# Rikorose/DeepFilterNet

Hardware: AMD Instinct MI355X
Metric: 48 kHz audio frames/sec (hop=480), DeepFilterNet3 enhance() (higher is better)
Workload: dtype f32 (storage and accumulation; GRU projections / recurrences, the fused DF-encoder convolutions and the pointwise halves of the ERB separable convolutions as fp16-split MFMAs: x = hi + lo in f16, hi*hi + hi*lo + lo*hi on v_mfma_f32_16x16x32_f16, ~2^-21 relative; see exact_fp32_ms_per_step); 1 GPU; DeepFilterNet3 (recalled shipped shape, conv_ch=64) enhance(pad=True), batch=256 clips x 10 s @48 kHz per GPU, 1002 STFT frames per clip; batch_per_gpu=256, global_batch=256, parallelism=clips sharded over 1 GPU(s); no collective, inputs_resident_in_hbm=True

## Files before the change

deepfilternet_amd/csrc/dfx_gru_sync.h:

```cpp
#pragma once

#define DFX_SYNC_SPIN_LIMIT (1 << 22)

static __device__ __forceinline__ unsigned int dfx_sync_my_word(unsigned int tag) { return tag | (unsigned int)(dfx_xcc_id() + 1); }
static __device__ __forceinline__ bool dfx_sync_is_mine(const unsigned int *word, unsigned int tag) {
    return __hip_atomic_load(word, __ATOMIC_RELAXED, __HIP_MEMORY_SCOPE_AGENT) == dfx_sync_my_word(tag);
}

struct DfxWaiter {
    int spin_limit;
    unsigned int *err;
    bool dead = false;

    template <int SLEEP>
    __device__ __forceinline__ void wait_ge(const unsigned int *flag, unsigned int want) {
        int spins = 0;
        while (!dead && (int)(__hip_atomic_load(flag, __ATOMIC_RELAXED, __HIP_MEMORY_SCOPE_AGENT) - want) < 0) {
            if (++spins > spin_limit) {
                dfx_raise(err + 2);
                dead = true;
                break;
            }
            if constexpr (SLEEP > 0) __builtin_amdgcn_s_sleep(SLEEP);
        }
    }
    template <int SLEEP>
    __device__ __forceinline__ unsigned int wait_registered(const unsigned int *word, unsigned int tag) {
        unsigned int v = 0u;
        int spins = 0;
        while (!dead && (((v = __hip_atomic_load(word, __ATOMIC_RELAXED, __HIP_MEMORY_SCOPE_AGENT)) & ~15u) != tag || (v & 15u) == 0u)) {
            if (++spins > spin_limit) {
                dfx_raise(err + 2);
                dead = true;
                break;
            }
            if constexpr (SLEEP > 0) __builtin_amdgcn_s_sleep(SLEEP);
        }
        return v;
    }
};

static __device__ __forceinline__ void dfx_sync_raise(unsigned int *flag, unsigned int value, bool light) {
    if (light) __hip_atomic_store(flag, value, __ATOMIC_RELAXED, __HIP_MEMORY_SCOPE_AGENT);
    else __hip_atomic_store(flag, value, __ATOMIC_RELEASE, __HIP_MEMORY_SCOPE_AGENT);
}
static __device__ __forceinline__ void dfx_sync_acquire(bool light) {
    if (light) DFX_L1_INV();
    else __builtin_amdgcn_fence(__ATOMIC_ACQUIRE, "agent");
}

struct DfxXcd {
    unsigned int *me = nullptr;
    const unsigned int *prod = nullptr;
    const unsigned int *cons = nullptr;
    const unsigned int *cons2 = nullptr;
    unsigned int tag = 0;
    unsigned int *stat = nullptr;
};
static __device__ __forceinline__ void dfx_xcd_register(const DfxXcd &X) {
    if (X.me && threadIdx.x == 0) __hip_atomic_store(X.me, dfx_sync_my_word(X.tag), __ATOMIC_RELAXED, __HIP_MEMORY_SCOPE_AGENT);
}
static __device__ __forceinline__ bool dfx_xcd_same(const DfxXcd &X, const unsigned int *other) { return other && dfx_sync_is_mine(other, X.tag); }
static __device__ __forceinline__ void dfx_xcd_acquire(const DfxXcd &X) { dfx_sync_acquire(dfx_xcd_same(X, X.prod)); }
static __device__ __forceinline__ void dfx_xcd_release(const DfxXcd &X, unsigned int *flag, unsigned int value) {
    const bool light = dfx_xcd_same(X, X.cons) && (!X.cons2 || dfx_xcd_same(X, X.cons2));
    dfx_sync_raise(flag, value, light);
    if (light && X.stat) __hip_atomic_fetch_add(X.stat, 1u, __ATOMIC_RELAXED, __HIP_MEMORY_SCOPE_AGENT);
}
static __device__ __forceinline__ int dfx_xcd_claim(const unsigned int *rec, unsigned int tag, int groups, unsigned int *claim, int fallback, DfxWaiter &W, int *slot) {
    if (!rec || groups > 64) return fallback;
    if (threadIdx.x == 0) {
        auto xcd_of = [&](int g) { return (int)(__hip_atomic_load(rec + g, __ATOMIC_RELAXED, __HIP_MEMORY_SCOPE_AGENT) & 15u) - 1; };
        for (int g = 0; g < groups; ++g) W.wait_registered<4>(rec + g, tag);
        int got = -1;
        const int x0 = dfx_xcc_id();
        for (int d = 0; d < 8 && got < 0 && !W.dead; ++d) {
            const int x = (x0 + d) & 7;
            int cnt = 0;
            for (int g = 0; g < groups; ++g) cnt += xcd_of(g) == x;
            if (!cnt) continue;
            const unsigned int k = __hip_atomic_fetch_add(claim + x, 1u, __ATOMIC_RELAXED, __HIP_MEMORY_SCOPE_AGENT);
            if ((int)k >= cnt) continue;
            for (int g = 0, j = 0; g < groups; ++g)
                if (xcd_of(g) == x && j++ == (int)k) got = g;
        }
        *slot = got < 0 ? fallback : got;
    }
    __syncthreads();
    const int r = *slot;
    __syncthreads();
    return r;
}

struct DfxPublish {
    unsigned int *cnt = nullptr;
    unsigned int *flag = nullptr;
    unsigned int value = 0, nblocks = 0;
};
static __device__ __forceinline__ void dfx_publish(const DfxPublish &P) {
    if (!P.cnt) return;
    DFX_VMEM_DRAIN();
    __syncthreads();
    if (threadIdx.x == 0) {
        const unsigned int old = __hip_atomic_fetch_add(P.cnt, 1u, __ATOMIC_ACQ_REL, __HIP_MEMORY_SCOPE_AGENT);
        if (old + 1u == P.nblocks) {
            __hip_atomic_store(P.cnt, 0u, __ATOMIC_RELAXED, __HIP_MEMORY_SCOPE_AGENT);
            __hip_atomic_store(P.flag, P.value, __ATOMIC_RELEASE, __HIP_MEMORY_SCOPE_AGENT);
        }
    }
}

__global__ void dfx_k_flag_set(unsigned int *flag, unsigned int value) {
    if (threadIdx.x == 0) __hip_atomic_store(flag, value, __ATOMIC_RELEASE, __HIP_MEMORY_SCOPE_AGENT);
}
__global__ void dfx_k_wait_ge(const unsigned int *flags, int n, unsigned int target, unsigned int *err, int spin_limit) {
    bool ok = false;
    int spins = 0;
    while (!ok) {
        ok = true;
        for (int i = threadIdx.x; i < n; i += blockDim.x)
            ok = ok && (int)(__hip_atomic_load(flags + i, __ATOMIC_RELAXED, __HIP_MEMORY_SCOPE_AGENT) - target) >= 0;
        ok = __all(ok);
        if (!ok) {
            if (++spins > spin_limit) {
                if (threadIdx.x == 0) dfx_raise(err + 2);
                break;
            }
            __builtin_amdgcn_s_sleep(16);
        }
    }
    __builtin_amdgcn_fence(__ATOMIC_ACQUIRE, "agent");
}

__global__ void dfx_k_probe_meet(unsigned int *cnt, unsigned int n, int spin_limit, unsigned int *fail) {
    if (threadIdx.x == 0) {
        __hip_atomic_fetch_add(cnt, 1u, __ATOMIC_RELAXED, __HIP_MEMORY_SCOPE_AGENT);
        int spins = 0;
        while (__hip_atomic_load(cnt, __ATOMIC_RELAXED, __HIP_MEMORY_SCOPE_AGENT) < n) {
            if (++spins > spin_limit) {
                dfx_raise(fail);
                break;
            }
            __builtin_amdgcn_s_sleep(16);
        }
    }
}
```

deepfilternet_amd/csrc/dfx_model.hip:

```cpp
#include "dfx_manifest.h"
#include "dfx_nn_kernels.h"

#include <cmath>
#include <functional>
#include <atomic>
#include <map>
#include <mutex>
#include <type_traits>
#include <fcntl.h>
#include <sys/file.h>
#include <sys/stat.h>
#include <unistd.h>

static int check_cfg(const dfx_model_cfg *c) {
    if (!c) DFX_FAIL(DFX_ERR_INVALID_ARG, "null model cfg");
    if (c->conv_ch != 16 && c->conv_ch != 32 && c->conv_ch != 64)
        DFX_FAIL(DFX_ERR_UNSUPPORTED, "conv_ch=%d: the HIP kernels are instantiated for 16, 32, 64", c->conv_ch);
    if (c->emb_hidden_dim != 256 || c->df_hidden_dim != 256) DFX_FAIL(DFX_ERR_UNSUPPORTED, "GRU hidden size must be 256");
    if (c->nb_erb <= 0 || c->nb_erb % 8 || c->nb_erb > 64) DFX_FAIL(DFX_ERR_UNSUPPORTED, "nb_erb must be a multiple of 8, <= 64");
    static_assert(2 * DFX_DEC10_SMEM(64, 64) <= 160 * 1024, "conv_ch <= 64, nb_erb <= 64: dfx_k_erb_dec10 must fit every accepted shape");
    if (c->nb_df <= 0 || c->nb_df % 2 || c->nb_df > c->fft_size / 2 + 1) DFX_FAIL(DFX_ERR_UNSUPPORTED, "nb_df must be even and <= F");
    if (c->df_order <= 0 || c->df_order > 16 || c->df_lookahead < 0 || c->df_lookahead >= c->df_order)
        DFX_FAIL(DFX_ERR_UNSUPPORTED, "need 0 <= df_lookahead < df_order <= 16");
    if (c->conv_lookahead < 0) DFX_FAIL(DFX_ERR_INVALID_ARG, "conv_lookahead < 0");
// ... 265 lines not shown
            acc = mode == 1 ? fmaxf(acc, v) : acc + v;
        }
        if (mode == 2) acc *= inv;
        for (int c = 0; c < ch; ++c) p[(int64_t)c * T * E] = acc;
    }
}

__global__ void dfx_k_gate_stages(const unsigned char *flags, unsigned char *stages, int64_t B) {
    const int64_t b = (int64_t)blockIdx.x * blockDim.x + threadIdx.x;
    if (b >= B) return;
    const unsigned char f = flags[b];
    stages[b] = (unsigned char)((f & DFX_GATE_DF) | ((f & (DFX_GATE_GAINS | DFX_GATE_ZEROS)) ? DFX_GATE_GAINS : 0));
}

#define DFX_GATE_MAX_ENTRIES 24
struct DfxGateTable {
    float *dst[DFX_GATE_MAX_ENTRIES];
    const float *src[DFX_GATE_MAX_ENTRIES];
    int64_t row[DFX_GATE_MAX_ENTRIES];
    unsigned char mask[DFX_GATE_MAX_ENTRIES], want[DFX_GATE_MAX_ENTRIES];
    int n;
    void add(float *dst_, const float *src_, int64_t row_, unsigned char mask_, unsigned char want_) {
        dst[n] = dst_, src[n] = src_, row[n] = row_, mask[n] = mask_, want[n] = want_;
        ++n;
    }
};
__global__ void dfx_k_gate_commit(DfxGateTable G, const unsigned char *flags, int64_t B) {
    const int64_t b = blockIdx.x;
    if (b >= B) return;
    const unsigned char f = flags[b];
    for (int e = 0; e < G.n; ++e) {
        if ((f & G.mask[e]) != G.want[e]) continue;
        const float *sp = G.src[e] + b * G.row[e];
        float *dp = G.dst[e] + b * G.row[e];
        for (int64_t i = threadIdx.x; i < G.row[e]; i += blockDim.x) dp[i] = sp[i];
    }
}

__global__ void dfx_k_gate_c0_shift(const unsigned char *flags, float *c0_win, int64_t B, int64_t T, int kt, int64_t frame) {
    const int64_t b = blockIdx.x;
    if (b >= B || !(flags[b] & DFX_GATE_DF)) return;
    float *w = c0_win + (b * T + T - kt) * frame;
    for (int64_t i = (int64_t)blockIdx.y * blockDim.x + threadIdx.x; i < frame; i += (int64_t)gridDim.y * blockDim.x)
        for (int j = 0; j + 1 < kt; ++j) w[j * frame + i] = w[(j + 1) * frame + i];
}

__global__ void dfx_k_gate_hold(const unsigned char *flags, float *win, int64_t cap, int64_t row, int64_t pos, int64_t h, int64_t B) {
    const int64_t b = blockIdx.x;
    if (b >= B || !(flags[b] & DFX_GATE_FROZEN)) return;
    float *w = win + (b * cap + pos) * row;
    for (int64_t i = (int64_t)blockIdx.y * blockDim.x + threadIdx.x; i < row; i += (int64_t)gridDim.y * blockDim.x)
        for (int64_t j = h - 1; j >= 0; --j) w[(j + 1) * row + i] = w[j * row + i];
}

__global__ void dfx_k_gate_pend_commit(const unsigned char *flags, unsigned char *par, int *cnt, int64_t B) {
    const int64_t b = (int64_t)blockIdx.x * blockDim.x + threadIdx.x;
    if (b >= B || !(flags[b] & DFX_GATE_DF)) return;
    par[b] ^= 1;
    cnt[b] += 1;
}

__global__ void dfx_k_gate_finish(const unsigned char *flags, int *skip_counter, float *y, int64_t y_stride, int hop, float *lsnr_out,
                                  int64_t lsnr_stride, int64_t B, int warm) {
    const int64_t b = blockIdx.x;
    if (b >= B) return;
    const unsigned char f = flags[b];
    if (f & DFX_GATE_FROZEN) {
        for (int i = threadIdx.x; i < hop; i += blockDim.x) y[b * y_stride + i] = 0.f;
        if (threadIdx.x == 0 && lsnr_out) lsnr_out[b * lsnr_stride] = (f & DFX_GATE_PAUSED) ? __int_as_float(0x7fc00000) : -15.f;
    } else if (threadIdx.x == 0 && !warm) {
        skip_counter[b] = (f & (DFX_GATE_GAINS | DFX_GATE_ZEROS)) ? 0 : skip_counter[b] + 1;
    }
}

enum { EV_START = 0, EV_C0, EV_C1, EV_C0P, EV_EMB, EV_COEFS, EV_FRONT, EV_DONE, EV_XA, EV_MASK, EV_FIN, EV_TICKET };

struct DfxCan {
    bool fuse_c0 = false;
    bool c0_batch_unfused = false;
    bool c0_h3 = false;
    bool c0_presplit = false;
    bool pw_h3 = false;
    bool fan = false, fan_skp = false;
    bool enc_fan = false;
    bool dfenc = false;
    bool fuse_enc = false;
    bool erb_tail = false;
    bool erb_enc4 = false;
    int df_out = DFX_PLAN_DF_OUT_GGEMM;
};

struct DfxSyncLayout {
    static constexpr size_t LG = (size_t)DFX_MAX_GRU_LAYERS * DFX_SEQ_GMAX;
    static constexpr size_t ready = 0;
    static constexpr size_t emb = 8;
    static constexpr size_t probe = 13;
    static constexpr size_t poison = 14;
    static constexpr size_t done = 16;
    static constexpr size_t pcnt = done + LG;
    static constexpr size_t yprog = pcnt + 16;
    static constexpr size_t giprog = yprog + LG;
    static constexpr size_t xtab = giprog + LG;
    static constexpr size_t xstat = xtab + 3 * LG;
    static constexpr size_t total = xstat + 64;
};

struct dfx_model {
    dfx_model_cfg cfg{};
    float *d_w = nullptr;
    size_t n_w = 0;
    size_t erb0_w = 0, erb0_b = 0;
    PwW erb1, erb2, erb3, dfc0, dfc1, ct3, ct2, ct1;
    size_t co_w = 0, co_ska = 0, co_skb = 0;
    float co_bias = 0.f;
    size_t tail_w0h3 = 0, tail_woh3 = 0;
    float tail_w0_unscale = 1.f, tail_wo_unscale = 1.f;
    GlinW fc_emb, enc_in, enc_out, dec_in, dec_out, dfg_in, df_skip, df_out, enc_skip, dec_skip;
    std::vector<GruW> enc_gru, dec_gru, df_gru;
    size_t lsnr_w = 0;
    float lsnr_b = 0.f;
    size_t fan_w = 0;
    int fan_chunks = 0;
    size_t efan_w1 = 0, efan_w2 = 0;
    int efan_groups = 0;
    size_t dfenc_fc = 0, dfenc_in = 0;
    float dfenc_fc_unscale = 1.f, dfenc_in_unscale = 1.f;
    size_t dfo_h3 = 0;
    float dfo_unscale = 1.f;
    size_t cp_w1 = 0, cp_w2 = 0, cp_b = 0;
    size_t cp_weff = 0, cp_b16 = 0;
    size_t cin_weff = 0, cin_b = 0;
    size_t c0_h3 = 0, dfc1_h3 = 0, cp_h3 = 0;
    float c0_unscale = 1.f, dfc1_unscale = 1.f, cp_unscale = 1.f;
    int cp_G = 0, cp_NO = 0;
    DfxLane *lanes = nullptr;
    struct DfxLaneSet *laneset = nullptr;
    hipEvent_t ev_fork = nullptr;
    hipEvent_t ev_pass = nullptr;
    hipEvent_t ev_gate = nullptr;
    mutable bool pass_pending = false;
    bool enqueue_ahead = false;
    bool concurrent = false;
    int max_chunks = 1;
    int tchunks = 12;
    int tchunk_min = 32;
    bool run_df = true;
    bool exact_fp32 = false;
    DfxCan can;
    unsigned int *d_sync = nullptr;
    unsigned int *d_psync = nullptr;
    mutable unsigned int seq_pbase = 0;
    mutable int64_t passes_ps = 0;
    mutable int64_t passes_pair = 0;
    mutable int64_t last_plan = 0;
    mutable int64_t passes_seq = 0, passes_ev = 0;
    mutable unsigned int seq_base = 0;
    unsigned long long *d_trace = nullptr;
    mutable int trace_dims[3] = {0, 0, 0};
    bool gru_seq = true;
    struct {
        int chunks = 0;
        bool gru_pair_far = false;
        bool gru_pair = true;
        int convp_late = -1;
        int p0_ahead = 3;
        int tail_every = 1;
        int dftail_every = 0;
        bool tail_split = true;
        int64_t convp_elems = (int64_t)1 << 29;
        bool c0_presplit = true;
        bool seq_trace = false;
        char hwq_probe_mode = 0;
        bool erb_enc_split = false;
        int ws_fill = -1;
    } sw;
    unsigned int *d_err = nullptr;
    unsigned int *h_err = nullptr;
    bool check_every_pass = false;
    int spin_limit = DFX_SYNC_SPIN_LIMIT;
    bool hwq_probe_pending = false;
    int hwq_probe = -1;
    const float *p(size_t off) const { return d_w + off; }
};

namespace {
struct Prep {
    const float *blob;
    const DfxManifest &man;
    std::vector<float> out;
    std::string err;
    bool exact_fp32 = false;
    struct Packed {
        bool pw = false, tail = false, c0 = false, fan = false, fan_skp = false, encfan = false, dfenc = false;
        int dfo_tiles = 0;
    } packed;
    const float *get(const std::string &name, const DfxTensor **tt = nullptr) {
        const DfxTensor *t = man.find(name);
        if (!t) {
            err = "tensor not in manifest: " + name;
            return nullptr;
        }
        if (tt) *tt = t;
        return blob + t->offset;
    }
    size_t alloc(size_t n) {
        size_t off = (out.size() + 3) & ~(size_t)3;
        out.resize(off + n, 0.f);
        return off;
    }
    bool bn(const std::string &p, int n, std::vector<float> &scale, std::vector<float> &shift) {
        const float *g = get(p + ".weight"), *b = get(p + ".bias"), *m = get(p + ".running_mean"), *v = get(p + ".running_var");
        if (!g || !b || !m || !v) return false;
        scale.resize(n);
        shift.resize(n);
        for (int i = 0; i < n; ++i) {
            const float s = g[i] / sqrtf(v[i] + 1e-5f);
            scale[i] = s;
            shift[i] = b[i] - m[i] * s;
        }
        return true;
    }
};

bool prep_sep(Prep &P, const std::string &name, int C, PwW &w) {
    const float *dw = P.get(name + ".0.weight"), *pw = P.get(name + ".1.weight");
    std::vector<float> sc, sh;
    if (!dw || !pw || !P.bn(name + ".2", C, sc, sh)) return false;
    w.dw = P.alloc(3 * C);
    w.wt = P.alloc((size_t)C * C);
    w.bias = P.alloc(C);
    for (int c = 0; c < C; ++c)
        for (int j = 0; j < 3; ++j) P.out[w.dw + j * C + c] = dw[c * 3 + j];
    for (int n = 0; n < C; ++n)
        for (int k = 0; k < C; ++k) P.out[w.wt + (size_t)k * C + n] = pw[(size_t)n * C + k] * sc[n];
    for (int n = 0; n < C; ++n) P.out[w.bias + n] = sh[n];
    return true;
}
bool prep_path(Prep &P, const std::string &name, int C, size_t &a_off, size_t &b_off) {
    const float *w = P.get(name + ".0.weight");
    std::vector<float> sc, sh;
    if (!w || !P.bn(name + ".1", C, sc, sh)) return false;
    a_off = P.alloc(C);
    b_off = P.alloc(C);
    for (int c = 0; c < C; ++c) {
        P.out[a_off + c] = w[c] * sc[c];
        P.out[b_off + c] = sh[c];
    }
    return true;
}
template <typename F>
size_t pack_h3(Prep &P, int nfrag, F val, float *unscale) {
    std::vector<float> v((size_t)nfrag * 64 * 8);
    float mx = 0.f;
    for (int fr = 0; fr < nfrag; ++fr)
        for (int l = 0; l < 64; ++l)
            for (int i = 0; i < 8; ++i) {
                const float w = val(fr, l, i);
                v[((size_t)fr * 64 + l) * 8 + i] = w;
                mx = fmaxf(mx, fabsf(w));
            }
    int e = 0;
    if (mx > 0.f) {
        int ex;
        frexpf(mx, &ex);
        e = 14 - ex;
        if (e > 24) e = 24;
        if (e < -14) e = -14;
    }
    const float sc = ldexpf(1.f, e);
    *unscale = ldexpf(1.f, -e);
    const size_t off = P.alloc((size_t)nfrag * 2 * 64 * 8 / 2);
    uint16_t *dst = reinterpret_cast<uint16_t *>(&P.out[off]);
    for (int fr = 0; fr < nfrag; ++fr)
        for (int l = 0; l < 64; ++l)
            for (int i = 0; i < 8; ++i) {
                const float w = v[((size_t)fr * 64 + l) * 8 + i] * sc;
                const uint16_t hb = dfx_f32_to_f16_bits(w);
                const uint16_t lb = dfx_f32_to_f16_bits(w - dfx_f16_bits_to_f32(hb));
                dst[(((size_t)fr * 2 + 0) * 64 + l) * 8 + i] = hb;
                dst[(((size_t)fr * 2 + 1) * 64 + l) * 8 + i] = lb;
            }
    return off;
}
size_t pack_x32(Prep &P, const float *w) {
    const int H = 256;
    const size_t off = P.alloc((size_t)3 * H * H);
    float *dst = &P.out[off];
    for (int ut = 0; ut < 16; ++ut)
        for (int kc = 0; kc < 8; ++kc)
            for (int gate = 0; gate < 3; ++gate)
                for (int half = 0; half < 2; ++half)
                    for (int l = 0; l < 64; ++l)
                        for (int i = 0; i < 4; ++i) {
                            const int unit = 16 * ut + (l & 15), k = 32 * kc + 8 * (l >> 4) + 4 * half + i;
                            const size_t frag = (((size_t)ut * 8 + kc) * 3 + gate) * 2 + half;
                            dst[(frag * 64 + l) * 4 + i] = w[(size_t)(gate * H + unit) * H + k];
                        }
    return off;
}
void pack_pw_h3(Prep &P, dfx_model *m) {
    const int C = m->cfg.conv_ch, KC = C / 32;
    if (C % 32 != 0) return;
    for (PwW *w : {&m->erb1, &m->erb2, &m->erb3, &m->ct3, &m->ct2, &m->ct1}) {
        w->wt_h3 = pack_h3(P, (C / 16) * KC, [&](int fr, int l, int i) {
            const int nt = fr / KC, kc = fr % KC;
            return P.out[w->wt + (size_t)((C / 4) * (l >> 4) + 8 * kc + i) * C + 16 * nt + (l & 15)];
        }, &w->unscale);
        w->has_h3 = true;
    }
    P.packed.pw = true;
}
bool prep_glin(Prep &P, const std::string &name, GlinW &g) {
    const DfxTensor *t = nullptr;
    const float *w = P.get(name, &t);
    if (!w) return false;
    g.G = (int)t->shape[0];
// ... 296 lines not shown
        const int j = l & 15, e = 8 * kc + i, ch = 16 * (e >> 2) + 4 * (l >> 4) + (e & 3);
        return j < 3 ? P.out[wo + (size_t)j * C + ch] : 0.f;
    }, &m->tail_wo_unscale);
    P.packed.tail = true;
}
bool prep_df_convp(Prep &P, dfx_model *m) {
    const dfx_model_cfg &c = m->cfg;
    const int C = c.conv_ch, kt = c.df_pathway_kernel_size_t, NO = 2 * c.df_order, G = dfx_gcd(C, NO), CG = C / G, OG = NO / G;
    const int idx = kt > 1 ? 1 : 0;
    const bool has_pw = kt > 1;
    const float *w = P.get("df_dec.df_convp." + std::to_string(idx) + ".weight");
    const float *pw = has_pw ? P.get("df_dec.df_convp." + std::to_string(idx + 1) + ".weight") : nullptr;
    std::vector<float> sc, sh;
    if (!w || (has_pw && !pw) || !P.bn("df_dec.df_convp." + std::to_string(idx + (has_pw ? 2 : 1)), NO, sc, sh)) return false;
    m->cp_G = G;
    m->cp_NO = NO;
    m->cp_w1 = P.alloc((size_t)G * kt * CG * 16);
    m->cp_w2 = P.alloc((size_t)NO * NO);
    m->cp_b = P.alloc(NO);
    for (int g = 0; g < G; ++g)
        for (int k = 0; k < kt; ++k)
            for (int ci = 0; ci < CG; ++ci)
                for (int o = 0; o < OG; ++o) {
                    float v = w[(((size_t)(g * OG + o) * CG + ci) * kt + k)];
                    if (!has_pw) v *= sc[g * OG + o];
                    P.out[m->cp_w1 + ((((size_t)g * kt + k) * CG + ci) * 16 + o)] = v;
                }
    for (int n = 0; n < NO; ++n) {
        for (int o = 0; o < NO; ++o) P.out[m->cp_w2 + (size_t)n * NO + o] = has_pw ? pw[(size_t)n * NO + o] * sc[n] : (n == o ? 1.f : 0.f);
        P.out[m->cp_b + n] = sh[n];
    }
    const bool folded = NO <= 16;
    m->cp_weff = P.alloc(folded ? (size_t)kt * C * 16 : 0);
    m->cp_b16 = P.alloc(16);
    for (int k = 0; folded && k < kt; ++k)
        for (int ch = 0; ch < C; ++ch) {
            const int g = ch / CG, ci = ch - g * CG;
            for (int n = 0; n < NO; ++n) {
                double acc = 0.0;
                for (int o = g * OG; o < (g + 1) * OG; ++o) {
                    const double p2 = has_pw ? (double)pw[(size_t)n * NO + o] : (n == o ? 1.0 : 0.0);
                    acc += p2 * (double)w[((size_t)o * CG + ci) * kt + k];
                }
                P.out[m->cp_weff + ((size_t)k * C + ch) * 16 + n] = (float)(acc * (double)sc[n]);
            }
        }
    for (int n = 0; folded && n < NO; ++n) P.out[m->cp_b16 + n] = sh[n];
    return true;
}
void pack_c0_h3(Prep &P, dfx_model *m) {
    const dfx_model_cfg &c = m->cfg;
    const int C = c.conv_ch, kt = c.df_pathway_kernel_size_t;
    if (C % 32 != 0 || 2 * c.df_order > 16) return;
    const int KC = C / 32;
    auto chan = [](int kc, int l, int i) { const int e = 8 * kc + i; return 16 * (e >> 2) + 4 * (l >> 4) + (e & 3); };
    const size_t cin = m->cin_weff, wt1 = m->dfc1.wt, cpw = m->cp_weff;
    m->c0_h3 = pack_h3(P, C / 16, [&](int nt, int l, int i) {
        const int k = 8 * (l >> 4) + i;
        return k < 18 ? P.out[cin + (size_t)k * C + 16 * nt + (l & 15)] : 0.f;
    }, &m->c0_unscale);
    m->dfc1_h3 = pack_h3(P, (C / 16) * KC, [&](int fr, int l, int i) {
        const int nt = fr / KC, kc = fr % KC;
        return P.out[wt1 + (size_t)chan(kc, l, i) * C + 16 * nt + (l & 15)];
    }, &m->dfc1_unscale);
    m->cp_h3 = pack_h3(P, kt * KC, [&](int fr, int l, int i) {
        const int k = fr / KC, kc = fr % KC;
        return P.out[cpw + ((size_t)k * C + chan(kc, l, i)) * 16 + (l & 15)];
    }, &m->cp_unscale);
    P.packed.c0 = true;
}
void pack_dfo_h3(Prep &P, dfx_model *m) {
    const GlinW a = m->df_out;
    const int NO = 2 * m->cfg.df_order, Fd = m->cfg.nb_df;
    if (!(a.Kg <= 32 && a.Kg % 8 == 0 && a.Ng % 2 == 0 && NO % 2 == 0 && Fd % 2 == 0 && (int64_t)a.G * a.Ng == (int64_t)NO * Fd &&
          DFX_DFO_SMEM(NO, Fd) <= (size_t)64 * 1024))
        return;
    const int NU = (a.Ng + 15) / 16;
    m->dfo_h3 = pack_h3(P, a.G * NU, [&](int fr, int l, int i) {
        const int g = fr / NU, u = fr % NU, o = 16 * u + (l & 15), k = 8 * (l >> 4) + i;
        return o < a.Ng && k < a.Kg ? P.out[a.w + ((size_t)g * a.Kg + k) * a.Ng + o] : 0.f;
    }, &m->dfo_unscale);
    P.packed.dfo_tiles = NU;
}
void pack_dfenc_h3(Prep &P, dfx_model *m) {
    const GlinW a = m->fc_emb, b = m->enc_in;
    const int C = m->cfg.conv_ch, Fout = m->cfg.nb_df / 2, KC = C / 32;
    if (!P.packed.c0) return;
    if (!(a.Kg % 32 == 0 && a.Ng == 16 && b.Kg == 32 && b.Ng == 16 && b.G * 2 == a.G && (int64_t)a.G * a.Kg == (int64_t)Fout * C)) return;
    m->dfenc_fc = pack_h3(P, Fout * KC, [&](int ci, int l, int i) {
        const int fo = ci / KC, kc = ci % KC, ch = 16 * ((8 * kc + i) >> 2) + 4 * (l >> 4) + (i & 3);
        const int idx = fo * C + ch, g = idx / a.Kg, kin = idx % a.Kg;
        return P.out[a.w + ((size_t)g * a.Kg + kin) * 16 + (l & 15)];
    }, &m->dfenc_fc_unscale);
    m->dfenc_in = pack_h3(P, b.G, [&](int j, int l, int i) {
        return P.out[b.w + ((size_t)j * 32 + 16 * (i >> 2) + 4 * (l >> 4) + (i & 3)) * 16 + (l & 15)];
    }, &m->dfenc_in_unscale);
    P.packed.dfenc = true;
}

bool prepare_weights(Prep &P, dfx_model *m) {
    const dfx_model_cfg &c = m->cfg;
    const int C = c.conv_ch;
    const bool skip_enc = c.emb_gru_skip_enc == DFX_SKIP_GROUPEDLINEAR, skip_dec = c.emb_gru_skip == DFX_SKIP_GROUPEDLINEAR;
    if (!prep_erb_conv0(P, m)) return false;
    if (!prep_sep(P, "enc.erb_conv1", C, m->erb1) || !prep_sep(P, "enc.erb_conv2", C, m->erb2) || !prep_sep(P, "enc.erb_conv3", C, m->erb3) ||
        !prep_sep(P, "enc.df_conv1", C, m->dfc1))
        return false;
    if (!prep_df_conv0(P, m)) return false;
    if (!prep_glin(P, "enc.df_fc_emb.0.weight", m->fc_emb) || !prep_glin(P, "enc.emb_gru.linear_in.0.weight", m->enc_in) ||
        !prep_gru(P, "enc.emb_gru.gru", 1, m->enc_gru) || !prep_glin(P, "enc.emb_gru.linear_out.0.weight", m->enc_out))
        return false;
    if (skip_enc && !prep_glin(P, "enc.emb_gru.gru_skip.weight", m->enc_skip)) return false;
    if (skip_dec && !prep_glin(P, "erb_dec.emb_gru.gru_skip.weight", m->dec_skip)) return false;
    if (!prep_lsnr(P, m)) return false;
    if (!prep_glin(P, "erb_dec.emb_gru.linear_in.0.weight", m->dec_in) || !prep_gru(P, "erb_dec.emb_gru.gru", c.emb_num_layers - 1, m->dec_gru) ||
        !prep_glin(P, "erb_dec.emb_gru.linear_out.0.weight", m->dec_out))
        return false;
    if (!prep_sep(P, "erb_dec.convt3", C, m->ct3) || !prep_path(P, "erb_dec.conv3p", C, m->ct3.sk_a, m->ct3.sk_b) ||
        !prep_sep(P, "erb_dec.convt2", C, m->ct2) || !prep_path(P, "erb_dec.conv2p", C, m->ct2.sk_a, m->ct2.sk_b) ||
        !prep_sep(P, "erb_dec.convt1", C, m->ct1) || !prep_path(P, "erb_dec.conv1p", C, m->ct1.sk_a, m->ct1.sk_b) ||
        !prep_path(P, "erb_dec.conv0p", C, m->co_ska, m->co_skb))
        return false;
    m->ct3.has_skip = m->ct2.has_skip = m->ct1.has_skip = true;
    pack_pw_h3(P, m);
    if (!prep_conv0_out(P, m)) return false;
    pack_tail_h3(P, m);
    if (!prep_df_convp(P, m)) return false;
    pack_c0_h3(P, m);
    if (!prep_glin(P, "df_dec.df_gru.linear_in.0.weight", m->dfg_in) || !prep_gru(P, "df_dec.df_gru.gru", c.df_num_layers, m->df_gru)) return false;
    if (c.df_gru_skip == DFX_SKIP_GROUPEDLINEAR && !prep_glin(P, "df_dec.df_skip.weight", m->df_skip)) return false;
    if (!prep_glin(P, "df_dec.df_out.0.weight", m->df_out)) return false;
    pack_fan(P, m);
    pack_encfan(P, m);
    pack_dfo_h3(P, m);
    pack_dfenc_h3(P, m);
    return true;
}
}

static void read_switches(dfx_model *m) {
    auto is = [](const char *name, char ch) {
        const char *v = getenv(name);
        return v && v[0] == ch;
    };
    auto at_least = [](const char *name, int least, int *out) {
        const char *v = getenv(name);
        if (v && atoi(v) >= least) *out = atoi(v);
    };
    m->exact_fp32 = is("DFX_EXACT_FP32", '1');
    m->concurrent = !is("DFX_STREAMS", '0');
    m->gru_seq = !is("DFX_GRU_SEQ", '0') && !dfx_env_is_emulator();
    if (getenv("DFX_GRU_PAIR")) m->sw.gru_pair = !is("DFX_GRU_PAIR", '0');
    m->sw.gru_pair_far = is("DFX_GRU_PAIR_FAR", '1');
    m->check_every_pass = is("DFX_CHECK_EVERY_PASS", '1');
    at_least("DFX_SYNC_SPIN_LIMIT", 1, &m->spin_limit);
    if (const char *v = getenv("DFX_CONVP_ELEMS"))
        if (atoll(v) > 0) m->sw.convp_elems = atoll(v);
    m->sw.erb_enc_split = is("DFX_ERB_ENC_SPLIT", '1');
    m->sw.c0_presplit = !is("DFX_C0_PRESPLIT", '0');
    if (const char *v = getenv("DFX_WS_FILL"))
        if (v[0] >= '0' && v[0] <= '9' && atoi(v) <= 255) m->sw.ws_fill = atoi(v);
#ifdef DFX_DEV
    if (getenv("DFX_TAIL_SPLIT")) m->sw.tail_split = !is("DFX_TAIL_SPLIT", '0');
    at_least("DFX_SEQ_P0_AHEAD", 1, &m->sw.p0_ahead);
    at_least("DFX_SEQ_DFTAIL_EVERY", 1, &m->sw.dftail_every);
    at_least("DFX_SEQ_TAIL_EVERY", 1, &m->sw.tail_every);
    at_least("DFX_SEQ_CHUNKS", 1, &m->sw.chunks);
    at_least("DFX_CONVP_LATE", 0, &m->sw.convp_late);
#endif
    m->sw.seq_trace = is("DFX_SEQ_TRACE", '1');
    int tc = 0;
    at_least("DFX_TCHUNKS", 1, &tc);
    if (tc) m->tchunks = tc < DFX_MAX_TCHUNKS ? tc : DFX_MAX_TCHUNKS;
    m->enqueue_ahead = is("DFX_ENQUEUE_AHEAD", '1');
    m->sw.hwq_probe_mode = is("DFX_HWQ_PROBE", '0') ? '0' : is("DFX_HWQ_PROBE", 'f') ? 'f' : 0;
}

static void model_capabilities(dfx_model *m, const Prep::Packed &k) {
    const dfx_model_cfg &c = m->cfg;
    const int C = c.conv_ch, E = c.nb_erb, Fd = c.nb_df, NO = 2 * c.df_order, emb = C * E / 4;
    const bool split = !m->exact_fp32;
    DfxCan &can = m->can;
    can.fuse_c0 = c.df_pathway_kernel_size_t <= 5 && NO <= 16;
    can.c0_batch_unfused = m->exact_fp32 && can.fuse_c0;
    can.c0_h3 = can.fuse_c0 && split && k.c0;
    can.c0_presplit = m->sw.c0_presplit && can.c0_h3;
    can.pw_h3 = split && k.pw;
    can.fan = k.fan && !c.enc_concat && emb == 64 * m->fan_chunks;
    can.fan_skp = can.fan && c.df_gru_skip == DFX_SKIP_GROUPEDLINEAR && k.fan_skp;
    can.enc_fan = k.encfan && !c.enc_concat && emb == 16 * m->efan_groups;
    can.dfenc = can.c0_h3 && can.enc_fan && k.dfenc;
    can.fuse_enc = E % 2 == 0 && 3 * (E + 2) <= 192 && 2 * DFX_ENC_SMEM(C, E) <= (size_t)160 * 1024;
    can.erb_tail = can.pw_h3 && k.tail && dfx_tail_ok(C, E);
    can.erb_enc4 = can.fuse_enc && can.pw_h3 && dfx_enc4_ok(C, E);
    const bool resident = k.dfo_tiles == 4 && m->df_out.G <= 16 && (int64_t)(NO / 2) * 16 * (Fd / 2) <= (int64_t)DFX_DFO_NPT * DFX_DFO_THREADS;
    can.df_out = !(split && k.dfo_tiles > 0) ? DFX_PLAN_DF_OUT_GGEMM : resident ? DFX_PLAN_DF_OUT_RESIDENT : DFX_PLAN_DF_OUT_STREAMING;
}

static int create_device_objects(dfx_model *m) {
    if (m->sw.seq_trace) (void)hipMalloc(reinterpret_cast<void **>(&m->d_trace), (size_t)DFX_MAX_GRU_LAYERS * DFX_SEQ_GMAX * DFX_GS_MAX_CHUNKS * 3 * 8);
    const size_t sync_bytes = DfxSyncLayout::total * sizeof(unsigned int);
    const size_t psync_bytes = (size_t)DFX_MAX_GRU_LAYERS * (DFX_SEQ_GMAX / 2) * 48 * sizeof(unsigned int);
    if (hipMalloc(reinterpret_cast<void **>(&m->d_psync), psync_bytes) != hipSuccess || hipMemset(m->d_psync, 0, psync_bytes) != hipSuccess ||
        hipMalloc(reinterpret_cast<void **>(&m->d_sync), sync_bytes) != hipSuccess || hipMemset(m->d_sync, 0, sync_bytes) != hipSuccess ||
        dfx_env_err_words_alloc(&m->h_err, &m->d_err, 256) != hipSuccess)
        DFX_FAIL(DFX_ERR_ALLOC, "dfx_model_create: device allocation failed");
    bool good = hipEventCreateWithFlags(&m->ev_fork, hipEventDisableTiming) == hipSuccess;
    good = good && hipEventCreateWithFlags(&m->ev_pass, hipEventDisableTiming) == hipSuccess;
    good = good && hipEventCreateWithFlags(&m->ev_gate, hipEventDisableTiming) == hipSuccess;
    good = good && dfx_create_lane(m, 0);
    for (int l = 1; l < m->max_chunks && good; ++l) good = dfx_create_lane(m, l);
    if (!good) DFX_FAIL(DFX_ERR_HIP, "dfx_model_create: could not create the auxiliary streams/events");
    return DFX_OK;
}

extern "C" int dfx_model_create(const dfx_model_cfg *cfg, const float *blob, dfx_model **out) {
    if (int rc = check_cfg(cfg)) return rc;
    if (!blob || !out) DFX_FAIL(DFX_ERR_INVALID_ARG, "dfx_model_create: null");
    if (int rc = dfx_require_device()) return rc;
    dfx_model *m = new dfx_model();
    m->cfg = *cfg;
    read_switches(m);
    const DfxManifest man = dfx_build_manifest(m->cfg);
    Prep P{blob, man};
    P.exact_fp32 = m->exact_fp32;
    if (!prepare_weights(P, m)) {
        delete m;
        DFX_FAIL(DFX_ERR_INVALID_ARG, "dfx_model_create: %s", P.err.empty() ? "weight preparation failed" : P.err.c_str());
    }
    m->n_w = P.out.size();
    if (hipMalloc(reinterpret_cast<void **>(&m->d_w), m->n_w * sizeof(float)) != hipSuccess) {
        delete m;
        DFX_FAIL(DFX_ERR_ALLOC, "dfx_model_create: device allocation of %zu bytes failed", m->n_w * sizeof(float));
    }
    if (hipMemcpy(m->d_w, P.out.data(), m->n_w * sizeof(float), hipMemcpyHostToDevice) != hipSuccess) {
        dfx_model_free(m);
        DFX_FAIL(DFX_ERR_HIP, "dfx_model_create: upload failed");
    }
    model_capabilities(m, P.packed);
    if (int rc = create_device_objects(m)) {
        dfx_model_free(m);
        return rc;
    }
    if (m->gru_seq && m->concurrent && !dfx_env_is_emulator()) {
        if (m->sw.hwq_probe_mode == 'f') {
            m->hwq_probe = 0;
            hwq_probe_fallback(m);
        } else if (m->sw.hwq_probe_mode != '0') {
            m->hwq_probe_pending = true;
        }
    }
    *out = m;
    return DFX_OK;
}

static void pass_gate_forget(const dfx_model *m);
extern "C" void dfx_model_free(dfx_model *m) {
    if (!m) return;
    pass_gate_forget(m);
    if (m->ev_fork) (void)hipEventDestroy(m->ev_fork);
    if (m->ev_pass) (void)hipEventDestroy(m->ev_pass);
    if (m->ev_gate) (void)hipEventDestroy(m->ev_gate);
    dfx_env_err_words_free(m->h_err);
    if (m->d_sync && m->d_trace) {
        unsigned int n = 0;
        if (hipMemcpy(&n, m->d_sync + DfxSyncLayout::xstat, sizeof(n), hipMemcpyDeviceToHost) == hipSuccess) fprintf(stderr, "[dfx] same-XCD (light) block hand-overs over the model's life: %u\n", n);
    }
    if (m->d_sync) (void)hipFree(m->d_sync);
    if (m->d_psync) (void)hipFree(m->d_psync);
    if (m->d_trace) (void)hipFree(m->d_trace);
    if (m->d_w) (void)hipFree(m->d_w);
    delete m;
}
extern "C" int dfx_model_set_streams(dfx_model *m, int enable) {
    if (!m) DFX_FAIL(DFX_ERR_INVALID_ARG, "null");
    m->concurrent = enable != 0;
    return DFX_OK;
}
extern "C" int dfx_model_set_run_df(dfx_model *m, int enable) {
    if (!m) DFX_FAIL(DFX_ERR_INVALID_ARG, "null");
    m->run_df = enable != 0;
    return DFX_OK;
}
extern "C" int dfx_model_set_pipeline(dfx_model *m, int time_chunks, int min_chunk_frames, int batch_chunks) {
    if (!m || time_chunks < 1 || min_chunk_frames < 1 || batch_chunks < 1) DFX_FAIL(DFX_ERR_INVALID_ARG, "dfx_model_set_pipeline: bad arguments");
    m->tchunks = time_chunks < DFX_MAX_TCHUNKS ? time_chunks : DFX_MAX_TCHUNKS;
    m->tchunk_min = min_chunk_frames;
    m->max_chunks = batch_chunks < DFX_MAX_LANES ? batch_chunks : DFX_MAX_LANES;
    for (int l = 1; l < m->max_chunks; ++l)
        if (!dfx_create_lane(m, l)) DFX_FAIL(DFX_ERR_HIP, "dfx_model_set_pipeline: could not create the streams of lane %d", l);
    return DFX_OK;
}
static int model_poll(const dfx_model *m) {
    unsigned int *h = m->h_err;
    if (!h) return DFX_OK;
    if (!(((volatile unsigned int *)h)[1] | ((volatile unsigned int *)h)[2])) return DFX_OK;
    const unsigned int e1 = __atomic_exchange_n(&h[1], 0u, __ATOMIC_ACQ_REL), e2 = __atomic_exchange_n(&h[2], 0u, __ATOMIC_ACQ_REL);
    if (!(e1 | e2)) return DFX_OK;
    if (e2)
        DFX_FAIL(DFX_ERR_HIP, "dfx: a flag wait of the persistent GRU phase timed out (bounded spin: the streams of the pass did not make progress "
                              "independently — hardware queues shared with other work, or the GPU shared with another process); the results of "
                              "the previous pass on this model are invalid.  DFX_GRU_SEQ=0 selects the event-synchronised form");
    DFX_FAIL(DFX_ERR_UNSUPPORTED, "dfx: an activation of magnitude >= 6e4 reached an fp16-split matrix kernel (GRU / DF-encoder / separable-conv "
                                  "path); the results of the previous pass on this model are invalid.  DFX_EXACT_FP32=1 selects the exact fp32 kernels");
}
extern "C" int dfx_model_poll(const dfx_model *m) {
    if (!m) DFX_FAIL(DFX_ERR_INVALID_ARG, "null");
    return model_poll(m);
}
extern "C" int dfx_model_check(const dfx_model *m) {
    if (!m) DFX_FAIL(DFX_ERR_INVALID_ARG, "null");
    DFX_HIP(hipDeviceSynchronize());
    return model_poll(m);
}
extern "C" int dfx_model_query(const dfx_model *m, int what, int64_t *value) {
    if (!m || !value) DFX_FAIL(DFX_ERR_INVALID_ARG, "dfx_model_query: null");
    switch (what) {
        case DFX_Q_GRU_PERSISTENT:
        case DFX_Q_HWQ_PROBE: {
            std::lock_guard<std::mutex> lk(dfx_enqueue_mu());
            hwq_probe_run(const_cast<dfx_model *>(m));
            *value = what == DFX_Q_HWQ_PROBE ? m->hwq_probe : (m->gru_seq && m->concurrent ? 1 : 0);
            return DFX_OK;
        }
        case DFX_Q_EXACT_FP32: *value = m->exact_fp32 ? 1 : 0; return DFX_OK;
        case DFX_Q_PASSES_PERSISTENT: *value = m->passes_seq; return DFX_OK;
        case DFX_Q_PASSES_TICKET_BUSY: *value = m->passes_ev; return DFX_OK;
        case DFX_Q_SPIN_LIMIT: *value = m->spin_limit; return DFX_OK;
        case DFX_Q_PASSES_C0_PRESPLIT: *value = m->passes_ps; return DFX_OK;
        case DFX_Q_LAST_PLAN: *value = m->last_plan; return DFX_OK;
        case DFX_Q_PASSES_PAIR: *value = m->passes_pair; return DFX_OK;
    }
    DFX_FAIL(DFX_ERR_INVALID_ARG, "dfx_model_query: unknown item %d", what);
}
extern "C" int dfx_model_seq_trace(const dfx_model *m, unsigned long long *out_host, int64_t cap, int *dims) {
    if (!m || !m->d_trace || !out_host || !dims) DFX_FAIL(DFX_ERR_INVALID_ARG, "dfx_model_seq_trace: tracing is off (DFX_SEQ_TRACE=1 at model creation)");
    const int64_t n = (int64_t)m->trace_dims[0] * m->trace_dims[1] * m->trace_dims[2] * 3;
    if (n > cap) DFX_FAIL(DFX_ERR_INVALID_ARG, "dfx_model_seq_trace: buffer too small");
    DFX_HIP(hipMemcpy(out_host, m->d_trace, (size_t)n * 8, hipMemcpyDeviceToHost));
    for (int i = 0; i < 3; ++i) dims[i] = m->trace_dims[i];
    return DFX_OK;
}
extern "C" int dfx_model_cfg_get(const dfx_model *m, dfx_model_cfg *out) {
    if (!m || !out) DFX_FAIL(DFX_ERR_INVALID_ARG, "null");
    *out = m->cfg;
    return DFX_OK;
}

static inline bool dfx_dfenc_ok(const dfx_model *m, int64_t B, int64_t T, int64_t feat_T) {
    const dfx_model_cfg &c = m->cfg;
    const int64_t emb = (int64_t)c.conv_ch * c.nb_erb / 4;
    return m->can.dfenc && B * T * emb < ((int64_t)1 << 31) && B * (feat_T > 0 ? feat_T : T) * c.nb_df < ((int64_t)1 << 29);
}
static inline bool dfx_feat_spec_unread(const dfx_model *m, int64_t B, int64_t T) { return m->can.c0_presplit && dfx_dfenc_ok(m, B, T, 0); }
static inline float *dfx_ws_base(void *workspace) { return reinterpret_cast<float *>(((uintptr_t)workspace + 255) & ~(uintptr_t)255); }

namespace {
struct Ws {
    size_t e0, e1, e2, e3, c0, c1, emb_in, emb, xa, xb, gi, xa2, xb2, gi2, demb, d3, d2, mask, c0p, xdf, coefs, lsnr, skp_e, skp_d, fps, total;
    size_t pgi[DFX_MAX_GRU_LAYERS], py[DFX_MAX_GRU_LAYERS], ph[DFX_MAX_GRU_LAYERS];
};
Ws plan_ws(const dfx_model *m, int64_t R, int64_t B) {
    const dfx_model_cfg &c = m->cfg;
    const bool c0_stored = !m->can.fuse_c0 || m->can.c0_batch_unfused, presplit = m->can.c0_presplit;
    Ws w{};
    size_t off = 0;
    auto take = [&](size_t n) {
        size_t o = off;
        off += (n + 63) & ~(size_t)63;
        return o;
    };
    const size_t C = c.conv_ch, E = c.nb_erb, Fd = c.nb_df, emb = C * E / 4, NO = 2 * c.df_order;
    w.e0 = take(R * E * C);
    w.e1 = take(R * (E / 2) * C);
    w.e2 = take(R * (E / 4) * C);
    w.e3 = take(R * (E / 4) * C);
    w.c0 = c0_stored ? take(R * Fd * C) : 0;
    w.c1 = take(R * (Fd / 2) * C);
    w.emb_in = take(R * emb * (c.enc_concat ? 2 : 1));
    w.emb = take(R * emb);
    w.xa = take(R * 256);
    w.xb = take(R * 256);
    w.gi = take(R * 768);
    w.xa2 = take(R * 256);
    w.xb2 = take(R * 256);
    w.gi2 = take(R * 768);
    w.demb = take(R * emb);
    w.d3 = take(R * (E / 4) * C);
    w.d2 = take(R * (E / 2) * C);
    w.mask = take(R * E);
    w.c0p = take(R * Fd * NO);
    w.xdf = take(R * 256);
    w.coefs = take(R * Fd * NO);
    w.lsnr = take(R);
    w.skp_e = take(c.emb_gru_skip_enc == DFX_SKIP_GROUPEDLINEAR ? R * emb : 0);
    w.skp_d = take(c.emb_gru_skip == DFX_SKIP_GROUPEDLINEAR ? R * emb : 0);
    w.fps = take(presplit ? R * Fd * 2 : 0);
    const int nlayers = 1 + (c.emb_num_layers - 1) + c.df_num_layers;
    for (int l = 0; l < DFX_MAX_GRU_LAYERS; ++l) {
        const bool used = l < nlayers;
        w.pgi[l] = take(used ? R * 768 : 0);
        w.py[l] = take(used ? R * 256 : 0);
        w.ph[l] = take(used ? (B > 0 ? B : R) * 256 : 0);
    }
    w.total = off;
    return w;
}
}

extern "C" int dfx_model_workspace_bytes(const dfx_model *m, int64_t B, int64_t T, int64_t *bytes) {
    if (!m || !bytes || B < 0 || T < 0) DFX_FAIL(DFX_ERR_INVALID_ARG, "dfx_model_workspace_bytes: bad arguments");
    *bytes = (int64_t)(plan_ws(m, B * T, B).total * sizeof(float)) + 256;
    return DFX_OK;
}

#include "dfx_model_launch.h"
#include "dfx_model_forward.h"
#include "dfx_model_stream.h"
#include "dfx_stream_move.h"
#include "dfx_model_enhance.h"
```

deepfilternet_amd/csrc/dfx_model_forward.h:

```cpp
#pragma once

#ifdef DFX_DEV
static int dfx_dev_skip() {
    static const int v = [] { const char *e = getenv("DFX_DEV_SKIP"); return e ? atoi(e) : 0; }();
    return v;
}
static bool dfx_dev_stage(int n) {
    static const int lo = [] { const char *e = getenv("DFX_DEV_STAGE_LO"); return e ? atoi(e) : 0; }();
    static const int hi = [] { const char *e = getenv("DFX_DEV_STAGE_HI"); return e ? atoi(e) : 99; }();
    return n >= lo && n <= hi;
}
#else
static constexpr int dfx_dev_skip() { return 0; }
static constexpr bool dfx_dev_stage(int) { return true; }
#endif

struct TicketGuard {
    bool armed = false;
    ~TicketGuard() {
        if (armed) dfx_ticket_release_cb(nullptr);
    }
};

template <int C>
// ... 334 lines not shown
            convp_split = use_seq && late_pct > 0 ? T - (T - t_begin) * late_pct / 100 : T;
            if (convp_split > t_begin && dfx_dev_stage(1) && (rc = convp_range(t_begin, convp_split, x2))) return rc;
            if (post_behind_convp && (rc = sc->df_post(x2))) return rc;
            if (convp_split >= T && (rc = signal(EV_C0P, x2))) return rc;
        }
        if (dfx_dev_stage(2) && (rc = erb_range(t_begin, T, Rn, rmw, s))) return rc;
        if ((rc = wait(EV_C1, s))) return rc;
        if (dfenc) {
            if (dfx_dev_stage(3) && (rc = launch_df_enc<C>(m, feat_spec, e3, c.emb_gru_skip_enc != DFX_SKIP_NONE ? emb_in : nullptr, xa, B, T, Fd, s, t_begin, Lk, T, featT, fps))) return rc;
        } else if (dfx_dev_stage(3) && (rc = emb_range(Rn, rmw, s))) return rc;
        if (signal_front && (rc = signal(EV_FRONT, s))) return rc;
        return DFX_OK;
    }

    int gru_serial() {
        int rc;
        float *hs_enc = sc ? sc->h_state : nullptr, *hs_dec = sc ? sc->h_state + (int64_t)nenc * B * 256 : nullptr;
        float *hs_df = sc ? sc->h_state + (int64_t)(nenc + ndec) * B * 256 : nullptr;
        float *hn_enc = sc && sc->h_next ? sc->h_next : nullptr, *hn_dec = hn_enc ? hn_enc + (int64_t)nenc * B * 256 : nullptr;
        float *hn_df = hn_enc ? hn_enc + (int64_t)(nenc + ndec) * B * 256 : nullptr;
        const float *y = xa;
        if (dfx_dev_stage(4) && (rc = run_gru_stack(m, m->enc_gru, xa, xa, xb, gi, B, T, &y, s, hs_enc, t_begin, rmw, hn_enc))) return rc;
        float *dec_x = y == xa ? xb : xa;
        if (fan) {
            if (dfx_dev_stage(5) && (rc = emb_fan(y, dec_x, Rn, s, rmw))) return rc;
            if ((rc = signal(EV_EMB, s)) || (rc = wait(EV_EMB, x1))) return rc;
        } else {
            if ((rc = enc_out_skip(y, Rn, s, rmw))) return rc;
            if ((rc = signal(EV_EMB, s)) || (rc = wait(EV_EMB, x1))) return rc;
            if ((rc = lsnr_all(s))) return rc;
        }
        if (gate) {
            dfx_launch(dfx_k_gate_post, dim3((unsigned)dfx_ceil_div(B, 256)), dim3(256), 0, s, (const float *)lsnr, T, gate->thr[0],
                       gate->thr[1], run_df ? gate->thr[2] : -INFINITY, gate->flags, B, gate->channels, gate->thr_rows);
            DFX_LAUNCH_CHECK();
        }
        if (run_df && dfx_dev_stage(6)) {
            const float *y2 = nullptr;
            if (!fan && (rc = launch_glin(m, m->dfg_in, embv, DFX_ACT_RELU, nullptr, xa2, Rn, x1, rmw))) return rc;
            if ((rc = run_gru_stack(m, m->df_gru, xa2, xa2, xb2, gi2, B, T, &y2, x1, hs_df, t_begin, rmw, hn_df, par))) return rc;
            if ((rc = df_tail_rows(y2, Rn, rmw, x1, true))) return rc;
            if ((rc = signal(EV_COEFS, x1))) return rc;
        }
        if (!fan && (rc = launch_glin(m, m->dec_in, embv, DFX_ACT_RELU, nullptr, dec_x, Rn, s, rmw))) return rc;
        if (dfx_dev_stage(7) && (rc = run_gru_stack(m, m->dec_gru, dec_x, xa, xb, gi, B, T, &y, s, hs_dec, t_begin, rmw, hn_dec, par && run_df))) return rc;
        if (dfx_dev_stage(8) && (rc = dec_out_skip(y, Rn, s, rmw))) return rc;
        if ((!fuse_tail || dfx_dev_stage(9)) && (rc = erb_dec_convs(Rn, rmw, s))) return rc;
        return DFX_OK;
    }

    int gru_events() {
        int rc;
        auto proj_ev = [&](const GruW &g, int l, int k, const float *xin, hipStream_t st) -> int {
            if ((dfx_dev_skip() & 4) && l > 0) return DFX_OK;
            return proj_chunk(g, l, k, xin, st);
        };
        auto gru_chunk = [&](const GruW &g, int l, int k, hipStream_t st) -> int {
            float *hl = ws + w.ph[l];
            return launch_gru_h3(m, g, ws + w.pgi[l], ws + w.py[l], k == 0 ? nullptr : hl, hl, B, T, tb(k), tb(k + 1), st, l);
        };
        if ((rc = signal(EV_XA, s))) return rc;
        for (int l = 0; l < nl; ++l) {
            if (l > 0 && (rc = wait(EV_XA, ln->gs[l]))) return rc;
            if ((rc = wait(EV_XA, ln->ps[l]))) return rc;
        }
        if ((rc = wait(EV_XA, ln->ts[0])) || (rc = wait(EV_XA, ln->ts[1]))) return rc;
        for (int k = 0; k < K; ++k) {
            if ((rc = proj_ev(m->enc_gru[0], 0, k, xa, ln->ps[0])) || (rc = esig(ln->pev[0][k], ln->ps[0]))) return rc;
        }
        for (int k = 0; k < K; ++k) {
            if ((rc = ewait(ln->pev[0][k], s)) || (rc = gru_chunk(m->enc_gru[0], 0, k, s)) || (rc = esig(ln->gev[0][k], s))) return rc;
        }
        for (int j = 0; j < ndec; ++j) {
            const int l = 1 + j;
            hipStream_t pst = ln->ps[l], gst = ln->gs[l];
            for (int k = 0; k < K; ++k) {
                if ((rc = ewait(ln->gev[l - 1][k], pst))) return rc;
                const float *xin = ws + w.py[l - 1];
                if (j == 0 && fan) {
                    if ((rc = emb_fan(ws + w.py[0], xb, Mk(k), pst, rmk(k)))) return rc;
                    if ((rc = esig(ln->eev[k], pst))) return rc;
                    xin = xb;
                } else if (j == 0) {
                    if ((rc = enc_out_skip(ws + w.py[0], Mk(k), pst, rmk(k)))) return rc;
                    if ((rc = esig(ln->eev[k], pst))) return rc;
                    if ((rc = launch_glin(m, m->dec_in, embv, DFX_ACT_RELU, nullptr, xb, Mk(k), pst, rmk(k)))) return rc;
                    xin = xb;
                }
                if ((rc = proj_ev(m->dec_gru[j], l, k, xin, pst)) || (rc = esig(ln->pev[l][k], pst))) return rc;
            }
            for (int k = 0; k < K; ++k) {
                if ((rc = ewait(ln->pev[l][k], gst)) || (rc = gru_chunk(m->dec_gru[j], l, k, gst)) || (rc = esig(ln->gev[l][k], gst))) return rc;
            }
        }
        {
            hipStream_t st = ln->ts[0];
            for (int k = 0; k < K; ++k) {
                if ((rc = ewait(ln->gev[ndec][k], st))) return rc;
                if (dfx_dev_skip() & 1) continue;
                if ((rc = dec_out_skip(ws + w.py[ndec], Mk(k), st, rmk(k))) || (rc = erb_dec_convs(Mk(k), rmk(k), st))) return rc;
            }
            if ((rc = signal(EV_MASK, st))) return rc;
        }
        for (int j = 0; j < ndf; ++j) {
            const int l = 1 + ndec + j;
            hipStream_t pst = ln->ps[l], gst = ln->gs[l];
            for (int k = 0; k < K; ++k) {
                const float *xin = ws + w.py[l - 1];
                if (j == 0) {
                    if ((rc = ewait(ln->eev[k], pst))) return rc;
                    if (!fan && (rc = launch_glin(m, m->dfg_in, embv, DFX_ACT_RELU, nullptr, xa2, Mk(k), pst, rmk(k)))) return rc;
                    xin = xa2;
                } else if ((rc = ewait(ln->gev[l - 1][k], pst))) return rc;
                if ((rc = proj_ev(m->df_gru[j], l, k, xin, pst)) || (rc = esig(ln->pev[l][k], pst))) return rc;
            }
            for (int k = 0; k < K; ++k) {
                if ((rc = ewait(ln->pev[l][k], gst)) || (rc = gru_chunk(m->df_gru[j], l, k, gst)) || (rc = esig(ln->gev[l][k], gst))) return rc;
            }
        }
        if (run_df) {
            hipStream_t st = ln->ts[1];
            const int l = ndec + ndf;
            if ((rc = wait(EV_C0P, st))) return rc;
            if (c.df_gru_skip != DFX_SKIP_IDENTITY) {
                for (int k = 0; k < K; ++k) {
                    if ((rc = ewait(ln->gev[l][k], st))) return rc;
                    if (dfx_dev_skip() & 2) continue;
                    if ((rc = df_tail_rows(ws + w.py[l], Mk(k), rmk(k), st))) return rc;
                }
            } else if ((rc = ewait(ln->gev[l][K - 1], st)) || (rc = df_tail_identity(ws + w.py[l], st))) return rc;
            if ((rc = signal(EV_COEFS, st))) return rc;
        }
        if ((rc = ewait(ln->eev[K - 1], s))) return rc;
        if (!fan && (rc = lsnr_all(s))) return rc;
        return DFX_OK;
    }

    int gru_persistent() {
        int rc;
        const unsigned int base = m->seq_base;
        m->seq_base += (unsigned int)K + 1u;
        using SL = DfxSyncLayout;
        unsigned int *ready = m->d_sync + SL::ready, *embf = m->d_sync + SL::emb, *done = m->d_sync + SL::done;
        unsigned int *pcnt = m->d_sync + SL::pcnt;
        unsigned int *yprog = m->d_sync + SL::yprog, *giprog = m->d_sync + SL::giprog;
        unsigned int *embprog = yprog + (size_t)(DFX_MAX_GRU_LAYERS - 1) * DFX_SEQ_GMAX;
        unsigned int *xtab = m->d_sync + SL::xtab, *xstat = m->d_sync + SL::xstat;
        const unsigned int xtag = (m->seq_pbase & 0x0fffffffu) << 4;
        auto xword = [&](int kind, int layer) { return xtab + ((size_t)kind * DFX_MAX_GRU_LAYERS + layer) * DFX_SEQ_GMAX; };
        const unsigned int pbase = m->seq_pbase;
        bool followed[DFX_MAX_GRU_LAYERS] = {};
        int nfollow = 0;
        const int lfirst_df = 1 + ndec;
        const bool follow_emb = fan && c.emb_gru_skip_enc != DFX_SKIP_GROUPEDLINEAR && nl < DFX_MAX_GRU_LAYERS &&
                                (nl + nl) * groups <= dfx_env_num_cus() * 3 / 4 && nl - 1 <= DFX_PF_MAX;
        for (int l = 1; l < nl; ++l) {
            const bool first = l == 1 || l == lfirst_df;
            if (!first || follow_emb) followed[l] = true, ++nfollow;
        }
        if (nfollow > DFX_PF_MAX || (nl + nfollow + 1) * groups > dfx_env_num_cus() * 3 / 4) {
            nfollow = 0;
            for (int l = 0; l < nl; ++l) followed[l] = false;
        }
        const bool use_pair = m->sw.gru_pair && !m->exact_fp32 && groups >= 2 && m->d_psync;
        m->passes_pair += use_pair ? 1 : 0;
        if (nfollow || use_pair) m->seq_pbase += (unsigned int)T + 1u;
        auto proj_pub = [&](const GruW &g, int l, int k, const float *xin, hipStream_t st) -> int {
            DfxPublish pub;
            pub.cnt = pcnt + l, pub.flag = ready + l, pub.value = base + (unsigned int)k + 1u;
            return proj_chunk(g, l, k, xin, st, &pub);
        };
        auto donep = [&](int l) { return done + (size_t)l * DFX_SEQ_GMAX; };
        auto tgt = [&](int k) { return base + (unsigned int)k + 1u; };
        hipStream_t G = ln->gs[1], Eq = ln->ts[0], Dq = ln->ts[1], Pq = ln->ps[0];
        const int ev_go = EV_XA;
        if ((rc = signal(EV_XA, s))) return rc;
        if (!m->enqueue_ahead && R >= DFX_THROTTLE_MIN_FRAMES) DFX_HIP(hipEventSynchronize(ln->ev[EV_XA]));
        if ((rc = wait(ev_go, G)) || (rc = wait(ev_go, Eq)) || (rc = wait(ev_go, Dq)) || (rc = wait(ev_go, Pq))) return rc;
        if (nfollow) DFX_HIP(hipMemsetAsync(xstat + 8, 0, (size_t)(DFX_PF_MAX + 1) * 8 * sizeof(unsigned int), G));
        {
            DfxGsArgs S;
            for (int l = 0; l < DFX_GS_MAX_LAYERS; ++l) S.gi[l] = nullptr, S.y[l] = nullptr, S.whf[l] = nullptr, S.bhn[l] = nullptr, S.unscale[l] = 1.f;
            for (int l = 0; l < nl; ++l) {
                const GruW &g = l == 0 ? m->enc_gru[0] : (l <= ndec ? m->dec_gru[l - 1] : m->df_gru[l - 1 - ndec]);
                S.gi[l] = ws + w.pgi[l];
                S.y[l] = ws + w.py[l];
                S.whf[l] = reinterpret_cast<const dfx_h8 *>(m->p(m->exact_fp32 ? g.whh_x32 : g.whh_h3));
                S.bhn[l] = m->p(g.bhn);
                S.unscale[l] = m->exact_fp32 ? 1.f : g.whh_unscale;
            }
            S.B = B, S.T = T, S.nlayers = nl, S.groups = groups, S.K = K;
            for (int i = 0; i <= K; ++i) S.tb[i] = cb[i];
            S.ready = ready, S.done = done, S.done_stride = DFX_SEQ_GMAX, S.base = base, S.err = m->d_err;
            S.trace = m->d_trace;
            S.spin_limit = m->spin_limit;
            S.pbase = pbase, S.sblk = 16;
            S.xtab = xtab, S.xstride = DFX_SEQ_GMAX, S.xstat = xstat;
            S.xtag = xtag, S.psync = m->d_psync, S.pair_far = m->sw.gru_pair_far ? 1 : 0;
            for (int l = 1; l < nl; ++l) {
                if (!followed[l]) continue;
                S.giprog[l] = giprog + (size_t)l * DFX_SEQ_GMAX;
                const bool first = l == 1 || l == lfirst_df;
                const int src = first ? 0 : l - 1;
                S.yprog[src] = yprog + (size_t)src * DFX_SEQ_GMAX;
                S.yblk[src] = first ? DFX_EF_STEPS : 16;
                S.xcons_kind[src] = first ? 2 : 1, S.xcons_layer[src] = first ? 0 : l;
            }
            m->trace_dims[0] = nl, m->trace_dims[1] = groups, m->trace_dims[2] = K;
            if (use_pair) DFX_HIP(dfx_env_set_max_dyn_smem((const void *)dfx_k_gru_seq_p2, DFX_GP_SMEM));
            else DFX_HIP(dfx_env_set_max_dyn_smem(m->exact_fp32 ? (const void *)dfx_k_gru_seq_x32 : (const void *)dfx_k_gru_seq, DFX_GH_SMEM));
            DfxKScope ks(DFX_K_GRU_REC, G);
            if (use_pair) dfx_launch(dfx_k_gru_seq_p2, dim3(dfx_gp_grid(nl * (int)((groups + 1) / 2))), dim3(DFX_GP_THREADS), DFX_GP_SMEM, G, S);
            else if (m->exact_fp32) dfx_launch(dfx_k_gru_seq_x32, dim3((unsigned)(nl * groups)), dim3(DFX_GH_THREADS), DFX_GH_SMEM, G, S);
            else dfx_launch(dfx_k_gru_seq, dim3((unsigned)(nl * groups)), dim3(DFX_GH_THREADS), DFX_GH_SMEM, G, S);
            DFX_LAUNCH_CHECK();
        }
        if (nfollow) {
            DfxPfArgs F;
            int f = 0;
            for (int l = 1; l < nl; ++l) {
                if (!followed[l]) continue;
                const GruW &g = l <= ndec ? m->dec_gru[l - 1] : m->df_gru[l - 1 - ndec];
                const bool first = l == 1 || l == lfirst_df;
                F.x[f] = first ? (l == 1 ? xb : xa2) : ws + w.py[l - 1], F.gi[f] = ws + w.pgi[l];
                F.wf[f] = reinterpret_cast<const dfx_h8 *>(m->p(m->exact_fp32 ? g.wih_t : g.wih_h3)), F.bias[f] = m->p(g.bias_i), F.unscale[f] = g.wih_unscale;
                F.yprog[f] = first ? embprog : yprog + (size_t)(l - 1) * DFX_SEQ_GMAX, F.giprog[f] = giprog + (size_t)l * DFX_SEQ_GMAX;
                F.xme[f] = xword(1, l), F.xprod[f] = first ? xword(2, 0) : xword(0, l - 1), F.xcons[f] = xword(0, l);
                ++f;
            }
            for (; f < DFX_PF_MAX; ++f) F.x[f] = nullptr, F.gi[f] = nullptr, F.wf[f] = nullptr, F.bias[f] = nullptr, F.unscale[f] = 1.f, F.yprog[f] = nullptr, F.giprog[f] = nullptr;
            F.xtag = xtag, F.xstat = xstat;
            F.xrec = xword(0, 0), F.xclaim = xstat + 8;
            F.B = B, F.T = T, F.nf = nfollow, F.groups = groups, F.pbase = pbase, F.err = m->d_err, F.spin_limit = m->spin_limit;
            int lq = -1;
            for (int l = nl - 1; l >= 2 && lq < 0; --l)
                if (followed[l]) lq = l;
            hipStream_t Fq = lq > 0 ? ln->ps[lq] : Dq;
            DFX_HIP(dfx_env_set_max_dyn_smem(m->exact_fp32 ? (const void *)dfx_k_proj_follow_x32 : (const void *)dfx_k_proj_follow, DFX_PH_SMEM));
            if ((rc = wait(ev_go, Fq))) return rc;
            DfxKScope ks(DFX_K_PROJ, Fq);
            if (m->exact_fp32) dfx_launch(dfx_k_proj_follow_x32, dim3((unsigned)(nfollow * groups)), dim3(512), DFX_PH_SMEM, Fq, F);
            else dfx_launch(dfx_k_proj_follow, dim3((unsigned)(nfollow * groups)), dim3(512), DFX_PH_SMEM, Fq, F);
            DFX_LAUNCH_CHECK();
        }
        if (followed[1]) {
            const float *res = c.emb_gru_skip_enc == DFX_SKIP_IDENTITY ? emb_in : nullptr;
            const bool need_emb = c.emb_gru_skip != DFX_SKIP_NONE || (run_df && c.df_gru_skip == DFX_SKIP_IDENTITY);
            float *dfg_x = run_df ? xa2 : nullptr, *skp = fan_skp ? xdf : nullptr;
            DfxFanArgs EA = emb_fan_args(m, ws + w.py[0], res, need_emb ? embv : nullptr, xb, dfg_x, skp, lsnr);
            DfxFollowSync EY;
            EY.x.me = xword(2, 0), EY.x.prod = xword(0, 0), EY.x.cons = xword(1, 1), EY.x.cons2 = followed[lfirst_df] ? xword(1, lfirst_df) : nullptr;
            EY.x.tag = xtag, EY.x.stat = xstat;
            EY.xclaim = xstat + 8 + 8 * DFX_PF_MAX, EY.groups = groups;
            EY.src = yprog, EY.dst = embprog, EY.pbase = pbase, EY.err = m->d_err, EY.spin_limit = m->spin_limit, EY.B = B, EY.T = T;
            hipStream_t Eq2 = ln->ps[1];
            if ((rc = wait(ev_go, Eq2))) return rc;
            {
                DfxKScope ks(DFX_K_EMB_FAN, Eq2);
                if (dfg_x && skp) dfx_launch((dfx_k_emb_follow<1, 2, 1>), dim3((unsigned)groups), dim3(512), 0, Eq2, EA, EY);
                else if (dfg_x) dfx_launch((dfx_k_emb_follow<1, 2, 0>), dim3((unsigned)groups), dim3(512), 0, Eq2, EA, EY);
                else dfx_launch((dfx_k_emb_follow<1, 0, 0>), dim3((unsigned)groups), dim3(512), 0, Eq2, EA, EY);
                DFX_LAUNCH_CHECK();
            }
            if ((rc = signal(EV_EMB, Eq2))) return rc;
        }
        const bool convp_after_p0 = nfollow > 0;
        auto convp_late = [&]() -> int {
            if (!(run_df && convp_split < T)) return DFX_OK;
            int r;
            if ((r = wait(ev_go, x2)) || (r = convp_range(convp_split, T, x2)) || (r = signal(EV_C0P, x2))) return r;
            return DFX_OK;
        };
        if (!convp_after_p0 && (rc = convp_late())) return rc;
        {
            for (int k = 0; k < K; ++k) {
                const int p0_ahead = m->sw.p0_ahead;
                if (k >= p0_ahead && (rc = launch_wait_ge(m, donep(0), groups, tgt(k - p0_ahead), Pq))) return rc;
                if ((rc = proj_pub(m->enc_gru[0], 0, k, xa, Pq))) return rc;
                if (convp_after_p0 && k == (K < p0_ahead ? K : p0_ahead) - 1 && (rc = convp_late())) return rc;
            }
        }
        for (int l = 1; l < nl; ++l)
            if ((rc = wait(ev_go, ln->ps[l]))) return rc;
        const int lf = 1 + ndec;
        auto prep_dec = [&](int j, int k) -> int {
            const int l = 1 + j;
            hipStream_t st = ln->ps[l];
            int r;
            if (followed[l]) return DFX_OK;
            if ((r = launch_wait_ge(m, donep(l - 1), groups, tgt(k), st))) return r;
            const float *xin = ws + w.py[l - 1];
            if (j == 0 && fan) {
                if (!m->exact_fp32) {
                    DfxPublish pub;
                    pub.cnt = pcnt + 8, pub.flag = embf, pub.value = tgt(k);
                    if ((r = emb_fan(ws + w.py[0], xb, Mk(k), st, rmk(k), &pub))) return r;
                } else if ((r = emb_fan(ws + w.py[0], xb, Mk(k), st, rmk(k))) || (r = launch_flag_set(embf, tgt(k), st))) return r;
                if (k == K - 1 && (r = signal(EV_EMB, st))) return r;
                xin = xb;
            } else if (j == 0) {
                if ((r = enc_out_skip(ws + w.py[0], Mk(k), st, rmk(k))) || (r = launch_flag_set(embf, tgt(k), st))) return r;
                if (k == K - 1 && (r = signal(EV_EMB, st))) return r;
                if ((r = launch_glin(m, m->dec_in, embv, DFX_ACT_RELU, nullptr, xb, Mk(k), st, rmk(k)))) return r;
                xin = xb;
            }
            if ((r = proj_pub(m->dec_gru[j], l, k, xin, st))) return r;
            return DFX_OK;
        };
        auto erb_tail = [&](int k0, int k) -> int {
            const int64_t Rk = Mk(k0, k);
            const DfxRowMap rm = rmk(k0, k);
            int r;
            hipStream_t Gq = (m->sw.tail_split && ndec >= 2 && followed[2]) ? ln->ps[2] : Eq;
            if ((r = launch_wait_ge(m, donep(ndec), groups, tgt(k), Gq))) return r;
            if (dfx_dev_skip() & 1) return DFX_OK;
            if ((r = dec_out_skip(ws + w.py[ndec], Rk, Gq, rm))) return r;
            if (Gq != Eq && ((r = esig(ln->pev[2][k], Gq)) || (r = ewait(ln->pev[2][k], Eq)))) return r;
            return erb_dec_convs(Rk, rm, Eq);
        };
        auto prep_df = [&](int j, int k) -> int {
            const int l = lf + j;
            hipStream_t st = ln->ps[l];
            int r;
            if (followed[l]) return DFX_OK;
            const float *xin = ws + w.py[l - 1];
            if (j == 0) {
                if ((r = launch_wait_ge(m, embf, 1, tgt(k), st))) return r;
                if (!fan && (r = launch_glin(m, m->dfg_in, embv, DFX_ACT_RELU, nullptr, xa2, Mk(k), st, rmk(k)))) return r;
                xin = xa2;
            } else if ((r = launch_wait_ge(m, donep(l - 1), groups, tgt(k), st))) return r;
            if ((r = proj_pub(m->df_gru[j], l, k, xin, st))) return r;
            return DFX_OK;
        };
        auto df_tail = [&](int k0, int k) -> int {
            const int l = ndec + ndf;
            const int64_t Rk = Mk(k0, k);
            const DfxRowMap rm = rmk(k0, k);
            if (int r = launch_wait_ge(m, donep(l), groups, tgt(k), Dq)) return r;
            if (dfx_dev_skip() & 2) return DFX_OK;
            if (c.df_gru_skip == DFX_SKIP_IDENTITY) {
                if (k < K - 1) return DFX_OK;
                return df_tail_identity(ws + w.py[l], Dq);
            }
            return df_tail_rows(ws + w.py[l], Rk, rm, Dq);
        };
        if (run_df && (rc = wait(EV_C0P, Dq))) return rc;
        for (int k = 0; k < K; ++k) {
            for (int j = 0; j < (ndec > ndf ? ndec : ndf); ++j) {
                if (j < ndec && (rc = prep_dec(j, k))) return rc;
                if (j < ndf && (rc = prep_df(j, k))) return rc;
            }
            const int tail_every = m->sw.tail_every;
            if ((k + 1) % tail_every == 0 || k == K - 1) {
                const int k0 = k - (k % tail_every);
                if ((rc = erb_tail(k0, k))) return rc;
            }
            const int dft_env = m->sw.dftail_every;
            const int dft_every = dft_env > 0 ? dft_env : (nfollow > 0 && convp_split < T && tail_every < 4 ? 4 : tail_every);
            if (run_df && ((k + 1) % dft_every == 0 || k == K - 1)) {
                const int k0 = k - (k % dft_every);
                if ((rc = df_tail(k0, k))) return rc;
            }
        }
        if ((rc = signal(EV_MASK, Eq))) return rc;
        if ((rc = wait(EV_EMB, s))) return rc;
        if (!fan && (rc = lsnr_all(s))) return rc;
        DFX_HIP(hipEventRecord(ln->gev[0][0], G));
        DFX_HIP(hipStreamWaitEvent(s, ln->gev[0][0], 0));
        for (int l = 0; l < nl; ++l) {
            DFX_HIP(hipEventRecord(ln->pev[l][0], ln->ps[l]));
            DFX_HIP(hipStreamWaitEvent(s, ln->pev[l][0], 0));
        }
        return DFX_OK;
    }

    int finish(float *coefs_out) {
        int rc;
        if (pipe) {
            fin_s = ln->ts[1];
            if ((rc = wait(EV_MASK, fin_s))) return rc;
        }
        if (run_df && fin_s == s && (rc = wait(EV_COEFS, s))) return rc;
        if (!run_df && coefs_out) DFX_HIP(hipMemsetAsync(coefs_out, 0, (size_t)R * Fd * NO * sizeof(float), fin_s));
        if (sc) {
            const float beta = sc->pf_beta >= 0.f ? sc->pf_beta : (c.mask_pf ? c.pf_beta : 0.f);
            if (sc->channels > 1 && sc->reduce_mask != 0) {
                dfx_launch(dfx_k_mask_reduce, dim3((unsigned)nn_grid(dfx_ceil_div(Rn * E / sc->channels, 256), 8)), dim3(256), 0, s, mask, B, T, t_begin,
                           E, sc->channels, sc->reduce_mask);
                DFX_LAUNCH_CHECK();
            }
            if (gate) {
                dfx_launch(dfx_k_gate_edit, dim3((unsigned)B), dim3(128), 0, s, (const unsigned char *)gate->flags, mask, coefs,
                           (const unsigned char *)bands->d_bin2band, B, T, E, Fd, run_df ? O : 0, O - 1 - c.df_lookahead);
                DFX_LAUNCH_CHECK();
            }
            return dfx_launch_df_apply(spec, coefs, DFX_COEF_BOTF, mask, bands, B, sc->spec_T, c.fft_size / 2 + 1, run_df ? Fd : 0, O, c.df_lookahead, beta,
                                       atten_lim, sc->out, s, t_begin, T, T, sc->out_T, sc->out_toff, sc->spec_stride, sc->spec_stride,
                                       sc->channels > 0 ? sc->channels : 1, sc->lim_rows, sc->beta_rows);
        }
        if (fin && dfx_synthesis_rows_ok(fin->st, true, O, run_df ? Fd : 0, E) && bands == fin->st->bands && sstride % 2 == 0 && sstride > 0) {
            m->last_plan |= DFX_PLAN_ROWS_FINISH;
            if ((rc = dfx_launch_synthesis_rows(fin->st, spec, sstride, run_df ? coefs : nullptr, run_df ? Fd : 0, O, c.df_lookahead, mask,
                                                c.mask_pf ? c.pf_beta : 0.f, atten_lim, B, T, fin->y, fin->out_stride, fin->out_skip, fin->out_len, fin_s, fin->out_i16, m->d_err, m->d_sync ? m->d_sync + DfxSyncLayout::poison : nullptr)))
                return rc;
        } else {
            if (dfx_dev_stage(10) && (rc = dfx_launch_df_apply(spec, coefs, DFX_COEF_BOTF, mask, bands, B, T, c.fft_size / 2 + 1, run_df ? Fd : 0, O, c.df_lookahead,
                                          c.mask_pf ? c.pf_beta : 0.f, atten_lim, spec_e, fin_s, 0, -1, -1, -1, 0, sstride, sstride)))
                return rc;
            if (fin && (rc = dfx_launch_synthesis(fin->st, spec_e, B, T, nullptr, nullptr, fin->y, fin->out_stride, fin->out_skip, fin->out_len,
                                                  fin_s, 0, -1, sstride, fin->out_i16)))
                return rc;
        }
        if (fin_s != s && ((rc = signal(EV_FIN, fin_s)) || (rc = wait(EV_FIN, s)))) return rc;
        if (use_seq && dfx_ticket().fd >= 0) {
// ... 131 lines not shown
```

deepfilternet_amd/csrc/dfx_nn_kernels.h:

```cpp
#pragma once

#include "dfx_common.h"

#include <type_traits>

#define DFX_ACT_NONE 0
#define DFX_ACT_RELU 1
#define DFX_ACT_TANH 2
#define DFX_ACT_SIGMOID 3

static __device__ __forceinline__ float dfx_sigmoid(float x) { return 1.f / (1.f + expf(-x)); }
static __device__ __forceinline__ float dfx_act(float v, int act) {
    if (act == DFX_ACT_RELU) return fmaxf(v, 0.f);
    if (act == DFX_ACT_TANH) return tanhf(v);
    if (act == DFX_ACT_SIGMOID) return dfx_sigmoid(v);
    return v;
}

static __device__ __forceinline__ float dfx_row256_scale_split(const float4 (&raw)[16], dfx_h8 (&xh)[8], dfx_h8 (&xl)[8]) {
    float mx = 0.f;
#pragma unroll
    for (int i = 0; i < 16; ++i) mx = fmaxf(mx, fmaxf(fmaxf(fabsf(raw[i].x), fabsf(raw[i].y)), fmaxf(fabsf(raw[i].z), fabsf(raw[i].w))));
    mx = fmaxf(mx, __shfl_xor(mx, 16));
    mx = fmaxf(mx, __shfl_xor(mx, 32));
// ... 2917 lines not shown
            }
        }
        __syncthreads();
        int prow = row0, pcol = col0;
        DFX_OPAQUE(prow);
        DFX_OPAQUE(pcol);
#pragma unroll
        for (int h = 0; h < 2; ++h) {
            float4 cv[DFX_DFO_NPT / 2];
            unsigned off[DFX_DFO_NPT / 2];
            int lrow[DFX_DFO_NPT / 2];
#pragma unroll
            for (int k = 0; k < DFX_DFO_NPT / 2; ++k) {
                off[k] = piece_off(prow, pcol);
                lrow[k] = (prow << 8) | pcol;
                piece_next(prow, pcol);
                cv[k] = *reinterpret_cast<const float4 *>(A.c0p + (off[k] != 0xffffffffu ? off[k] : 0u));
            }
#pragma unroll
            for (int k = 0; k < DFX_DFO_NPT / 2; ++k) {
                if (off[k] != 0xffffffffu) {
                    const float4 v = *reinterpret_cast<const float4 *>(img + (size_t)(lrow[k] >> 8) * RS + 4 * (lrow[k] & 255));
                    *reinterpret_cast<float4 *>(A.out + off[k]) = make_float4(v.x + cv[k].x, v.y + cv[k].y, v.z + cv[k].z, v.w + cv[k].w);
                }
            }
        }
        __syncthreads();
    }
    if (amax >= DFX_H3_LIMIT && A.err) dfx_raise(A.err + 1);
}

#define DFX_PJ_K 256
#define DFX_PJ_BN 128
#define DFX_PJ_LDW (DFX_PJ_BN + 16)
#define DFX_PJ_SMEM ((size_t)DFX_PJ_K * DFX_PJ_LDW * 4)
struct DfxPjArgs {
    const float *a;
    const float *w;
    const float *bias;
    float *out;
    int64_t M;
    int N, ncol, rgroups;
    DfxRowMap rm = DfxRowMap{0, 0, 0};
};

#define DFX_PJ_THREADS 512
template <int MODE>
__global__ void __launch_bounds__(DFX_PJ_THREADS, 2) dfx_k_proj256(DfxPjArgs A) {
    constexpr int K = DFX_PJ_K, BN = DFX_PJ_BN, LDW = DFX_PJ_LDW, NT = BN / 16;
    DFX_DYN_SMEM(float, wl);
    const int tid = threadIdx.x, lane = tid & 63, wave = tid >> 6, q = lane >> 4, jl = lane & 15;
    const int64_t jj = (int64_t)blockIdx.x >> 3;
    const int64_t rg = (jj / A.ncol) * 8 + (blockIdx.x & 7);
    const int ct = (int)(jj % A.ncol);
    if (rg >= A.rgroups) return;
    const int n0 = ct * BN;
    for (int i = tid; i < K * (BN / 4); i += DFX_PJ_THREADS) {
        const int k = i / (BN / 4), n4 = i - k * (BN / 4);
        const float4 v = *reinterpret_cast<const float4 *>(A.w + (size_t)k * A.N + n0 + 4 * n4);
        *reinterpret_cast<float4 *>(wl + ((k & 63) * 4 + (k >> 6)) * LDW + 4 * n4) = v;
    }
    __syncthreads();
    constexpr int NW = DFX_PJ_THREADS / 64;
    const int64_t ntiles = (A.M + 15) / 16;
    const int64_t tstride = (int64_t)A.rgroups * NW;
    const float *wfrag = wl + q * LDW + jl;
    const float4 *bias4 = reinterpret_cast<const float4 *>(A.bias + n0) + q;
    auto load_half = [&](float4 *dst, int64_t tl, int h) {
        const int64_t m = tl * 16 + jl;
        if (MODE != 1 && tl < ntiles && m < A.M) {
            const float4 *p = reinterpret_cast<const float4 *>(A.a + dfx_row(A.rm, m) * K + 64 * q) + 8 * h;
#pragma unroll
            for (int v = 0; v < 8; ++v) dst[8 * h + v] = p[v];
        } else {
#pragma unroll
            for (int v = 0; v < 8; ++v) dst[8 * h + v] = make_float4(0.f, 0.f, 0.f, 0.f);
        }
    };
    float4 xv[16];
    int64_t tile = rg * NW + wave;
    load_half(xv, tile, 0);
    load_half(xv, tile, 1);
    while (tile < ntiles) {
        const int64_t next = tile + tstride;
        f32x4 acc[NT];
#pragma unroll
        for (int nt = 0; nt < NT; ++nt) acc[nt] = f32x4{0.f, 0.f, 0.f, 0.f};
        float fa[2][NT];
#pragma unroll
        for (int nt = 0; nt < NT; ++nt) fa[0][nt] = wfrag[16 * nt];
        dfx_static_for<0, 64>([&](auto kc) {
            constexpr int ks = decltype(kc)::value;
            if constexpr (ks + 1 < 64 && MODE != 2) {
#pragma unroll
                for (int nt = 0; nt < NT; ++nt) fa[(ks + 1) & 1][nt] = wfrag[(ks + 1) * 4 * LDW + 16 * nt];
            }
            const float4 x4 = xv[ks >> 2];
            const float xk = (ks & 3) == 0 ? x4.x : (ks & 3) == 1 ? x4.y : (ks & 3) == 2 ? x4.z : x4.w;
#pragma unroll
            for (int nt = 0; nt < NT; ++nt) acc[nt] = __builtin_amdgcn_mfma_f32_16x16x4f32(fa[MODE == 2 ? 0 : (ks & 1)][nt], xk, acc[nt], 0, 0, 0);
            DFX_SCHED_BARRIER();
            if constexpr (ks == 31) load_half(xv, next, 0);
        });
        load_half(xv, next, 1);
        const int64_t m = tile * 16 + jl;
        if (m < A.M) {
            float4 *op = reinterpret_cast<float4 *>(A.out + dfx_row(A.rm, m) * A.N + n0 + 4 * q);
#pragma unroll
            for (int nt = 0; nt < NT; ++nt) {
                const float4 bz = bias4[4 * nt];
                op[4 * nt] = make_float4(acc[nt][0] + bz.x, acc[nt][1] + bz.y, acc[nt][2] + bz.z, acc[nt][3] + bz.w);
            }
        }
        tile = next;
    }
}

#define DFX_PH_THREADS 512
#define DFX_PH_BM 128
#define DFX_PH_NC 64
#define DFX_PH_CHUNK_H8 (8 * 4 * 2 * 64)
#define DFX_PH_SMEM ((size_t)2 * DFX_PH_CHUNK_H8 * 16)
#include "dfx_gru_sync.h"
struct DfxPhArgs {
    const float *a;
    const dfx_h8 *wf;
    const float *bias;
    float *out;
    int64_t M;
    int N;
    float unscale;
    DfxRowMap rm;
    int parts = 1;
    DfxPublish pub;
};

__global__ void __launch_bounds__(DFX_PH_THREADS, 2) dfx_k_proj256_h3(DfxPhArgs A) {
    DFX_DYN_SMEM(dfx_h8, ws);
    const int tid = threadIdx.x, lane = tid & 63, wave = tid >> 6, q = lane >> 4, jl = lane & 15;
    const int nparts = A.parts > 0 ? A.parts : 1;
    const int cper = A.N / DFX_PH_NC / nparts;
    const int cfirst = (int)(blockIdx.x % nparts) * cper, nchunks = cfirst + cper;
    const int64_t ml = (int64_t)(blockIdx.x / nparts) * DFX_PH_BM + 16 * wave + jl;
    const bool ok = ml < A.M;
    const int64_t m = ok ? dfx_row(A.rm, ml) : 0;
    constexpr int PER_T = DFX_PH_CHUNK_H8 / DFX_PH_THREADS;
#pragma unroll
    for (int i = 0; i < PER_T; ++i) ws[(size_t)(cfirst & 1) * DFX_PH_CHUNK_H8 + i * DFX_PH_THREADS + tid] = A.wf[(size_t)cfirst * DFX_PH_CHUNK_H8 + i * DFX_PH_THREADS + tid];
    dfx_h8 xh[8], xl[8];
    const float unscale = A.unscale * dfx_row256_split(A.a + m * 256 + 8 * q, ok, xh, xl);
    __syncthreads();
    for (int c = cfirst; c < nchunks; ++c) {
        const dfx_h8 *wc = ws + (size_t)(c & 1) * DFX_PH_CHUNK_H8;
        dfx_h8 pre[PER_T];
        if (c + 1 < nchunks) {
            const dfx_h8 *src = A.wf + (size_t)(c + 1) * DFX_PH_CHUNK_H8;
#pragma unroll
            for (int i = 0; i < PER_T; ++i) pre[i] = src[i * DFX_PH_THREADS + tid];
        }
        f32x4 acc[4];
#pragma unroll
        for (int ct = 0; ct < 4; ++ct) acc[ct] = f32x4{0.f, 0.f, 0.f, 0.f};
#pragma unroll
        for (int kc = 0; kc < 8; ++kc) {
            dfx_h8 whi[4], wlo[4];
#pragma unroll
            for (int ct = 0; ct < 4; ++ct) {
                whi[ct] = wc[((kc * 4 + ct) * 2 + 0) * 64 + lane];
                wlo[ct] = wc[((kc * 4 + ct) * 2 + 1) * 64 + lane];
            }
#pragma unroll
            for (int ct = 0; ct < 4; ++ct) acc[ct] = dfx_mfma_16x16x32_f16(wlo[ct], xh[kc], acc[ct]);
#pragma unroll
            for (int ct = 0; ct < 4; ++ct) acc[ct] = dfx_mfma_16x16x32_f16(whi[ct], xl[kc], acc[ct]);
#pragma unroll
            for (int ct = 0; ct < 4; ++ct) acc[ct] = dfx_mfma_16x16x32_f16(whi[ct], xh[kc], acc[ct]);
        }
        if (ok) {
#pragma unroll
            for (int ct = 0; ct < 4; ++ct) {
                const int n = c * DFX_PH_NC + 16 * ct + 4 * q;
                const float4 bz = *reinterpret_cast<const float4 *>(A.bias + n);
                *reinterpret_cast<float4 *>(A.out + m * A.N + n) =
                    make_float4(acc[ct][0] * unscale + bz.x, acc[ct][1] * unscale + bz.y, acc[ct][2] * unscale + bz.z, acc[ct][3] * unscale + bz.w);
            }
        }
        if (c + 1 < nchunks) {
            dfx_h8 *dst = ws + (size_t)((c + 1) & 1) * DFX_PH_CHUNK_H8;
#pragma unroll
            for (int i = 0; i < PER_T; ++i) dst[i * DFX_PH_THREADS + tid] = pre[i];
        }
        __syncthreads();
    }
    dfx_publish(A.pub);
}

struct DfxGstArgs {
    const float *x;
    const float *h_in;
    float *h_out;
    float *y;
    const dfx_h8 *wif, *whf;
    const float *bias_i;
    const float *bhn;
    float unscale_i, unscale_h;
    int64_t B;
    DfxRowMap xrm, yrm;
};
#ifndef DFX_GST_ABLATE
#define DFX_GST_ABLATE 0
#endif
template <int CT>
static __device__ __forceinline__ bool dfx_gru_step_place(int64_t B, int wave, int jl, int &u, int64_t &b) {
    constexpr int NU = 16 / CT;
    const int xcd = (int)(blockIdx.x & 7), kk = (int)(blockIdx.x >> 3);
    u = kk % NU;
    const int64_t rb = xcd + 8 * (int64_t)(kk / NU);
    b = rb * DFX_PH_BM + 16 * wave + jl;
    return rb * DFX_PH_BM < B;
}
template <int CT>
static __device__ __forceinline__ void dfx_gru_step_gates(const DfxGstArgs &A, const f32x4 (&g)[6][CT], int64_t b, int u, int q) {
    const int64_t yr = A.y ? dfx_row(A.yrm, b) : 0;
#pragma unroll
    for (int ct = 0; ct < CT; ++ct) {
        const int n0 = 16 * CT * u + 16 * ct + 4 * q;
        const float4 br = *reinterpret_cast<const float4 *>(A.bias_i + n0), bz = *reinterpret_cast<const float4 *>(A.bias_i + 256 + n0),
                     bn = *reinterpret_cast<const float4 *>(A.bias_i + 512 + n0), bh = *reinterpret_cast<const float4 *>(A.bhn + n0),
                     hp = *reinterpret_cast<const float4 *>(A.h_in + b * 256 + n0);
        const float brr[4] = {br.x, br.y, br.z, br.w}, bzz[4] = {bz.x, bz.y, bz.z, bz.w}, bnn[4] = {bn.x, bn.y, bn.z, bn.w},
                    bhh[4] = {bh.x, bh.y, bh.z, bh.w}, hpp[4] = {hp.x, hp.y, hp.z, hp.w};
        float o[4];
#pragma unroll
        for (int r = 0; r < 4; ++r) {
            if (DFX_GST_ABLATE & 8) {
                o[r] = g[0][ct][r] + g[1][ct][r] + g[2][ct][r] + g[3][ct][r] + g[4][ct][r] + g[5][ct][r] + brr[r] + bzz[r] + bnn[r] + bhh[r] + hpp[r];
                continue;
            }
            const float rg = dfx_fast_rcp(1.f + dfx_fast_exp(-((g[0][ct][r] + brr[r]) + g[3][ct][r])));
            const float zg = dfx_fast_rcp(1.f + dfx_fast_exp(-((g[1][ct][r] + bzz[r]) + g[4][ct][r])));
            const float pre = (g[2][ct][r] + bnn[r]) + rg * (g[5][ct][r] + bhh[r]);
            const float ng = 2.f * dfx_fast_rcp(1.f + dfx_fast_exp(-2.f * pre)) - 1.f;
            o[r] = (1.f - zg) * ng + zg * hpp[r];
        }
        const float4 ov = make_float4(o[0], o[1], o[2], o[3]);
        *reinterpret_cast<float4 *>(A.h_out + b * 256 + n0) = ov;
        if (A.y) *reinterpret_cast<float4 *>(A.y + yr * 256 + n0) = ov;
    }
}
template <int CT>
__global__ void __launch_bounds__(DFX_PH_THREADS, 2) dfx_k_gru_step_h3(DfxGstArgs A) {
    static_assert(CT == 2 || CT == 4, "32 or 64 hidden units per workgroup");
    constexpr int CHUNK = 8 * CT * 2 * 64;
    constexpr int PER_T = CHUNK / DFX_PH_THREADS;
    DFX_DYN_SMEM(dfx_h8, ws);
    const int tid = threadIdx.x, lane = tid & 63, wave = tid >> 6, q = lane >> 4, jl = lane & 15;
    int u;
    int64_t b;
    if (!dfx_gru_step_place<CT>(A.B, wave, jl, u, b)) return;
    const bool ok = b < A.B;
    const int ct0 = (CT * u) & 3;
    auto chunk_src = [&](int i) { return (i < 3 ? A.wif : A.whf) + (size_t)(4 * (i % 3) + (CT * u) / 4) * DFX_PH_CHUNK_H8; };
    auto src_index = [&](int e) {
        const int kc = e / (CT * 128), rem = e - kc * (CT * 128);
        return (kc * 4 + ct0) * 128 + rem;
    };
    float4 xraw[16], hraw[16];
    const int64_t bl = ok ? b : A.B - 1;
    const int64_t xr = dfx_row(A.xrm, bl);
    auto fetch_row = [&](const float *row, float4 (&raw)[16]) {
        const float4 *p = reinterpret_cast<const float4 *>(row + 8 * q);
#pragma unroll
        for (int kc = 0; kc < 8; ++kc) {
            raw[2 * kc] = !(DFX_GST_ABLATE & 4) ? p[8 * kc] : make_float4(0.f, 0.f, 0.f, 0.f);
            raw[2 * kc + 1] = !(DFX_GST_ABLATE & 4) ? p[8 * kc + 1] : make_float4(0.f, 0.f, 0.f, 0.f);
        }
    };
    fetch_row(A.x + xr * 256, xraw);
    fetch_row(A.h_in + bl * 256, hraw);
    {
        const dfx_h8 *src = chunk_src(0);
#pragma unroll
        for (int i = 0; i < PER_T; ++i) ws[i * DFX_PH_THREADS + tid] = src[src_index(i * DFX_PH_THREADS + tid)];
    }
    dfx_h8 xh[8], xl[8], hh[8], hl[8];
    const float us_x = A.unscale_i * dfx_row256_scale_split(xraw, xh, xl);
    float us_h = 0.f;
    f32x4 g[6][CT];
    __syncthreads();
    dfx_static_for<0, 6>([&](auto cc) {
        constexpr int c = decltype(cc)::value;
        const dfx_h8 *wc = ws + (size_t)(c & 1) * CHUNK;
        dfx_h8 pre[PER_T];
        if constexpr (c + 1 < 6 && !(DFX_GST_ABLATE & 2)) {
            const dfx_h8 *src = chunk_src(c + 1);
#pragma unroll
            for (int i = 0; i < PER_T; ++i) pre[i] = src[src_index(i * DFX_PH_THREADS + tid)];
            DFX_SCHED_BARRIER();
        }
        f32x4 acc[CT];
#pragma unroll
        for (int ct = 0; ct < CT; ++ct) acc[ct] = f32x4{0.f, 0.f, 0.f, 0.f};
        if constexpr (c == 1) us_h = A.unscale_h * dfx_row256_scale_split(hraw, hh, hl);
#pragma unroll
        for (int kc = 0; kc < 8; ++kc) {
            dfx_h8 whi[CT], wlo[CT];
#pragma unroll
            for (int ct = 0; ct < CT; ++ct) {
                whi[ct] = wc[((kc * CT + ct) * 2 + 0) * 64 + lane];
                wlo[ct] = wc[((kc * CT + ct) * 2 + 1) * 64 + lane];
            }
            const dfx_h8 vh = c < 3 ? xh[kc] : hh[kc], vl = c < 3 ? xl[kc] : hl[kc];
#pragma unroll
            for (int ct = 0; ct < CT; ++ct) acc[ct] = dfx_mfma_16x16x32_f16(wlo[ct], vh, acc[ct]);
            if (DFX_GST_ABLATE & 1) continue;
#pragma unroll
            for (int ct = 0; ct < CT; ++ct) acc[ct] = dfx_mfma_16x16x32_f16(whi[ct], vl, acc[ct]);
#pragma unroll
            for (int ct = 0; ct < CT; ++ct) acc[ct] = dfx_mfma_16x16x32_f16(whi[ct], vh, acc[ct]);
        }
#pragma unroll
        for (int ct = 0; ct < CT; ++ct) g[c][ct] = acc[ct] * (c < 3 ? us_x : us_h);
        if constexpr (c + 1 < 6) {
            dfx_h8 *dst = ws + (size_t)((c + 1) & 1) * CHUNK;
#pragma unroll
            for (int i = 0; i < PER_T; ++i) dst[i * DFX_PH_THREADS + tid] = pre[i];
            __syncthreads();
        }
    });
    if (ok) dfx_gru_step_gates<CT>(A, g, b, u, q);
}

template <int CT>
__global__ void __launch_bounds__(DFX_PH_THREADS, 2) dfx_k_gru_step_x32(DfxGstArgs A) {
    static_assert(CT == 2 || CT == 4, "32 or 64 hidden units per workgroup");
    constexpr int CHUNK = 8 * CT * 2 * 64;
    constexpr int PER_T = CHUNK / DFX_PH_THREADS;
    static_assert((size_t)2 * CHUNK * 16 <= DFX_PH_SMEM, "two chunks fit the projection kernel's LDS");
    DFX_DYN_SMEM(dfx_h8, ws);
    const int tid = threadIdx.x, lane = tid & 63, wave = tid >> 6, q = lane >> 4, jl = lane & 15;
    int u;
    int64_t b;
    if (!dfx_gru_step_place<CT>(A.B, wave, jl, u, b)) return;
    const bool ok = b < A.B;
    auto src_of = [&](int i, int e) -> const dfx_h8 * {
        const int kc = e / (CT * 128), rem = e - kc * (CT * 128), ct = rem >> 7;
        return (i < 3 ? A.wif : A.whf) + ((((size_t)(CT * u + ct) * 8 + kc) * 3 + (i % 3)) * 128 + (rem & 127));
    };
    f32x4 xv[16], hv[16];
    const int64_t bl = ok ? b : A.B - 1;
    const int64_t xr = dfx_row(A.xrm, bl);
    auto fetch_row = [&](const float *row, f32x4 (&v)[16]) {
        const float4 *p = reinterpret_cast<const float4 *>(row + 8 * q);
#pragma unroll
        for (int i = 0; i < 16; ++i) {
            const float4 t = !(DFX_GST_ABLATE & 4) ? p[8 * (i >> 1) + (i & 1)] : make_float4(0.f, 0.f, 0.f, 0.f);
            v[i] = f32x4{t.x, t.y, t.z, t.w};
        }
    };
    fetch_row(A.x + xr * 256, xv);
    fetch_row(A.h_in + bl * 256, hv);
#pragma unroll
    for (int i = 0; i < PER_T; ++i) ws[i * DFX_PH_THREADS + tid] = *src_of(0, i * DFX_PH_THREADS + tid);
    f32x4 g[6][CT];
    __syncthreads();
    dfx_static_for<0, 6>([&](auto cc) {
        constexpr int c = decltype(cc)::value;
        const dfx_h8 *wc = ws + (size_t)(c & 1) * CHUNK;
        dfx_h8 pre[PER_T];
        if constexpr (c + 1 < 6 && !(DFX_GST_ABLATE & 2)) {
#pragma unroll
            for (int i = 0; i < PER_T; ++i) pre[i] = *src_of(c + 1, i * DFX_PH_THREADS + tid);
            DFX_SCHED_BARRIER();
        }
        f32x4 acc[CT];
#pragma unroll
        for (int ct = 0; ct < CT; ++ct) acc[ct] = f32x4{0.f, 0.f, 0.f, 0.f};
#pragma unroll
        for (int kc = 0; kc < 8; ++kc) {
#pragma unroll
            for (int hf = 0; hf < 2; ++hf) {
                f32x4 w[CT];
#pragma unroll
                for (int ct = 0; ct < CT; ++ct) w[ct] = __builtin_bit_cast(f32x4, wc[((kc * CT + ct) * 2 + hf) * 64 + lane]);
                const f32x4 v = c < 3 ? xv[2 * kc + hf] : hv[2 * kc + hf];
#pragma unroll
                for (int j = 0; j < 4; ++j)
#pragma unroll
                    for (int ct = 0; ct < CT; ++ct) acc[ct] = __builtin_amdgcn_mfma_f32_16x16x4f32(w[ct][j], v[j], acc[ct], 0, 0, 0);
            }
        }
#pragma unroll
        for (int ct = 0; ct < CT; ++ct) g[c][ct] = acc[ct];
        if constexpr (c + 1 < 6) {
            dfx_h8 *dst = ws + (size_t)((c + 1) & 1) * CHUNK;
            if constexpr (!(DFX_GST_ABLATE & 2)) {
#pragma unroll
                for (int i = 0; i < PER_T; ++i) dst[i * DFX_PH_THREADS + tid] = pre[i];
            }
            __syncthreads();
        }
    });
    if (ok) dfx_gru_step_gates<CT>(A, g, b, u, q);
}

#ifndef DFX_PH_ABLATE
#define DFX_PH_ABLATE 0
#endif
template <int NW, int CT>
__global__ void __launch_bounds__(64 * NW, CT == 2 ? 2 : 1) dfx_k_proj256_h3x2(DfxPhArgs A) {
    constexpr int DFX_PH2_THREADS = 64 * NW, BM2 = 32 * NW;
    constexpr int CH8 = 8 * CT * 2 * 64;
    DFX_DYN_SMEM(dfx_h8, ws);
    const int tid = threadIdx.x, lane = tid & 63, wave = tid >> 6, q = lane >> 4, jl = lane & 15;
    const int nchunks = A.N / (16 * CT);
    constexpr int PER_T = CH8 / DFX_PH2_THREADS;
    auto src_of = [&](int c, int i) -> const dfx_h8 * {
        const int e = i * DFX_PH2_THREADS + tid;
        const int kc = e / (CT * 128), r = e - kc * (CT * 128);
        const int blk = (c * CT) / 4, ct0 = (c * CT) % 4;
        return A.wf + (size_t)blk * DFX_PH_CHUNK_H8 + (size_t)(kc * 4 + ct0) * 128 + r;
    };
#pragma unroll
    for (int i = 0; i < PER_T; ++i) ws[i * DFX_PH2_THREADS + tid] = *src_of(0, i);
    dfx_h8 xh[2][8], xl[2][8];
    float unscale[2];
    int64_t mrow[2];
    bool okr[2];
#pragma unroll
    for (int t = 0; t < 2; ++t) {
        const int64_t ml = (int64_t)blockIdx.x * BM2 + 32 * wave + 16 * t + jl;
        okr[t] = ml < A.M;
        mrow[t] = okr[t] ? dfx_row(A.rm, ml) : 0;
        unscale[t] = A.unscale * dfx_row256_split(A.a + mrow[t] * 256 + 8 * q, okr[t], xh[t], xl[t]);
    }
    __syncthreads();
    for (int c = 0; c < nchunks; ++c) {
        const dfx_h8 *wc = ws + (size_t)(c & 1) * CH8;
        dfx_h8 pre[PER_T];
        if (c + 1 < nchunks && !(DFX_PH_ABLATE & 8)) {
#pragma unroll
            for (int i = 0; i < PER_T; ++i) pre[i] = *src_of(c + 1, i);
        }
        f32x4 acc[2][CT];
#pragma unroll
        for (int t = 0; t < 2; ++t)
#pragma unroll
            for (int ct = 0; ct < CT; ++ct) acc[t][ct] = f32x4{0.f, 0.f, 0.f, 0.f};
#pragma unroll
        for (int kc = 0; kc < 8; ++kc) {
            dfx_h8 whi[CT], wlo[CT];
#pragma unroll
            for (int ct = 0; ct < CT; ++ct) {
                whi[ct] = wc[((kc * CT + ct) * 2 + 0) * 64 + lane];
                wlo[ct] = wc[((kc * CT + ct) * 2 + 1) * 64 + lane];
            }
#pragma unroll
            for (int ct = 0; ct < CT; ++ct)
#pragma unroll
                for (int t = 0; t < 2; ++t) acc[t][ct] = (DFX_PH_ABLATE & 4) ? acc[t][ct] + f32x4{(float)wlo[ct][0], 0.f, 0.f, (float)xh[t][kc][0]} : dfx_mfma_16x16x32_f16(wlo[ct], xh[t][kc], acc[t][ct]);
#pragma unroll
            for (int ct = 0; ct < CT; ++ct)
#pragma unroll
                for (int t = 0; t < 2; ++t) acc[t][ct] = (DFX_PH_ABLATE & 4) ? acc[t][ct] : dfx_mfma_16x16x32_f16(whi[ct], xl[t][kc], acc[t][ct]);
#pragma unroll
            for (int ct = 0; ct < CT; ++ct)
#pragma unroll
                for (int t = 0; t < 2; ++t) acc[t][ct] = (DFX_PH_ABLATE & 4) ? acc[t][ct] : dfx_mfma_16x16x32_f16(whi[ct], xh[t][kc], acc[t][ct]);
        }
#pragma unroll
        for (int ct = 0; ct < CT; ++ct) {
            const int n = c * (16 * CT) + 16 * ct + 4 * q;
            const float4 bz = *reinterpret_cast<const float4 *>(A.bias + n);
#pragma unroll
            for (int t = 0; t < 2; ++t)
                if (okr[t] && (!(DFX_PH_ABLATE & 1) || acc[t][ct][0] == 1.2345e-30f))
                    *reinterpret_cast<float4 *>(A.out + mrow[t] * A.N + n) =
                        make_float4(acc[t][ct][0] * unscale[t] + bz.x, acc[t][ct][1] * unscale[t] + bz.y, acc[t][ct][2] * unscale[t] + bz.z,
                                    acc[t][ct][3] * unscale[t] + bz.w);
        }
        if (c + 1 < nchunks && !(DFX_PH_ABLATE & 2)) {
            dfx_h8 *dst = ws + (size_t)((c + 1) & 1) * CH8;
#pragma unroll
            for (int i = 0; i < PER_T; ++i) dst[i * DFX_PH2_THREADS + tid] = pre[i];
        }
        __syncthreads();
    }
    dfx_publish(A.pub);
}

#define DFX_FAN_NC 3
#define DFX_FAN_WPJ 28
struct DfxFanArgs {
    const float *y;
    const float4 *wfrag;
    const float *res;
    float *emb_out;
    float *out[DFX_FAN_NC];
    int act[DFX_FAN_NC];
    const float *lsnr_w;
    float lsnr_b, lsnr_scale, lsnr_off;
    float *lsnr;
    int64_t R;
    int nj;
    int parts;
    DfxRowMap rm;
    DfxPublish pub;
};
template <int RT, int K0, int K1, int K2>
static __device__ __forceinline__ void dfx_emb_fan_item(const DfxFanArgs &A, int64_t tile, int J0, int J1) {
    const int lane = threadIdx.x & 63, n = lane & 15, q = lane >> 4;
    const int H = 32 * A.nj, EMB = 64 * A.nj;
    int64_t prow[RT];
    bool ok[RT];
    float ls[RT];
#pragma unroll
    for (int rt = 0; rt < RT; ++rt) {
        const int64_t lr = tile * (16 * RT) + 16 * rt + n;
        ok[rt] = lr < A.R;
        prow[rt] = ok[rt] ? dfx_row(A.rm, lr) : 0;
        ls[rt] = 0.f;
    }
    float4 w1n[4], yn[RT][2];
    auto request = [&](int J) {
#pragma unroll
        for (int i = 0; i < 4; ++i) w1n[i] = A.wfrag[((size_t)J * DFX_FAN_WPJ + i) * 64 + lane];
#pragma unroll
        for (int rt = 0; rt < RT; ++rt)
#pragma unroll
            for (int ch = 0; ch < 2; ++ch)
                yn[rt][ch] = ok[rt] ? *reinterpret_cast<const float4 *>(A.y + prow[rt] * H + 32 * J + 16 * ch + 4 * q) : make_float4(0.f, 0.f, 0.f, 0.f);
    };
    request(J0);
    for (int J = J0; J < J1; ++J) {
        float4 w1[4], yc[RT][2], wc[DFX_FAN_NC][8];
#pragma unroll
        for (int i = 0; i < 4; ++i) w1[i] = w1n[i];
#pragma unroll
        for (int rt = 0; rt < RT; ++rt) yc[rt][0] = yn[rt][0], yc[rt][1] = yn[rt][1];
        dfx_static_for<0, DFX_FAN_NC>([&](auto CI) {
            constexpr int c = decltype(CI)::value;
            constexpr int kind = c == 0 ? K0 : (c == 1 ? K1 : K2);
#pragma unroll
            for (int i = 0; i < (kind == 2 ? 8 : (kind == 1 ? 4 : 0)); ++i) wc[c][i] = A.wfrag[((size_t)J * DFX_FAN_WPJ + 4 + 8 * c + i) * 64 + lane];
        });
        if (J + 1 < J1) request(J + 1);
        float4 lw[4];
#pragma unroll
        for (int tt = 0; tt < 4; ++tt)
            lw[tt] = A.lsnr_w ? *reinterpret_cast<const float4 *>(A.lsnr_w + 64 * J + 16 * tt + 4 * q) : make_float4(0.f, 0.f, 0.f, 0.f);
#pragma unroll
        for (int rt = 0; rt < RT; ++rt) {
            float e[4][4];
#pragma unroll
            for (int ch = 0; ch < 2; ++ch) {
                const float ys[4] = {yc[rt][ch].x, yc[rt][ch].y, yc[rt][ch].z, yc[rt][ch].w};
#pragma unroll
                for (int t = 0; t < 2; ++t) {
                    const int tt = 2 * ch + t;
                    const float ws[4] = {w1[tt].x, w1[tt].y, w1[tt].z, w1[tt].w};
                    f32x4 d = f32x4{0.f, 0.f, 0.f, 0.f};
#pragma unroll
                    for (int k = 0; k < 4; ++k) d = __builtin_amdgcn_mfma_f32_16x16x4f32(ws[k], ys[k], d, 0, 0, 0);
#pragma unroll
                    for (int r = 0; r < 4; ++r) e[tt][r] = fmaxf(d[r], 0.f);
                    const int64_t eoff = prow[rt] * EMB + 64 * J + 16 * tt + 4 * q;
                    if (A.res && ok[rt]) {
                        const float4 rv = *reinterpret_cast<const float4 *>(A.res + eoff);
                        e[tt][0] += rv.x, e[tt][1] += rv.y, e[tt][2] += rv.z, e[tt][3] += rv.w;
                    }
                    if (A.emb_out && ok[rt]) *reinterpret_cast<float4 *>(A.emb_out + eoff) = make_float4(e[tt][0], e[tt][1], e[tt][2], e[tt][3]);
                    ls[rt] += e[tt][0] * lw[tt].x;
                    ls[rt] += e[tt][1] * lw[tt].y;
                    ls[rt] += e[tt][2] * lw[tt].z;
                    ls[rt] += e[tt][3] * lw[tt].w;
                }
            }
            dfx_static_for<0, DFX_FAN_NC>([&](auto CI) {
                constexpr int c = decltype(CI)::value;
                constexpr int kind = c == 0 ? K0 : (c == 1 ? K1 : K2);
                if constexpr (kind != 0) {
                    constexpr int NTT = kind == 2 ? 4 : 2;
#pragma unroll
                    for (int u = 0; u < 2; ++u) {
                        f32x4 d = f32x4{0.f, 0.f, 0.f, 0.f};
#pragma unroll
                        for (int i = 0; i < NTT; ++i) {
                            const int tt = kind == 2 ? i : 2 * u + i;
                            const float4 wv = wc[c][NTT * u + i];
                            const float ws[4] = {wv.x, wv.y, wv.z, wv.w};
#pragma unroll
                            for (int r = 0; r < 4; ++r) d = __builtin_amdgcn_mfma_f32_16x16x4f32(ws[r], e[tt][r], d, 0, 0, 0);
                        }
                        if (ok[rt])
                            *reinterpret_cast<float4 *>(A.out[c] + prow[rt] * H + 32 * J + 16 * u + 4 * q) =
                                make_float4(dfx_act(d[0], A.act[c]), dfx_act(d[1], A.act[c]), dfx_act(d[2], A.act[c]), dfx_act(d[3], A.act[c]));
                    }
                }
            });
        }
    }
    if (A.lsnr) {
#pragma unroll
        for (int rt = 0; rt < RT; ++rt) {
            float v = ls[rt];
            v += __shfl_xor(v, 16);
            v += __shfl_xor(v, 32);
            if (q == 0 && ok[rt]) A.lsnr[prow[rt]] = dfx_sigmoid(v + A.lsnr_b) * A.lsnr_scale + A.lsnr_off;
        }
    }
}
template <int RT, int K0, int K1, int K2>
__global__ void __launch_bounds__(256, 2) dfx_k_emb_fan(DfxFanArgs A) {
    const int64_t ntile = (A.R + 16 * RT - 1) / (16 * RT);
    const int jper = A.nj / A.parts;
    for (int64_t item = (int64_t)blockIdx.x * 4 + (threadIdx.x >> 6); item < ntile * A.parts; item += (int64_t)gridDim.x * 4) {
        const int64_t tile = item / A.parts;
        const int J0 = (int)(item - tile * A.parts) * jper;
        dfx_emb_fan_item<RT, K0, K1, K2>(A, tile, J0, J0 + jper);
    }
    dfx_publish(A.pub);
}
#define DFX_EF_STEPS 8
struct DfxFollowSync {
    const unsigned int *src;
    unsigned int *dst;
    unsigned int pbase;
    unsigned int *err;
    int spin_limit;
    int64_t B, T;
    DfxXcd x;
    unsigned int *xclaim = nullptr;
    int groups = 0;
};
template <int K0, int K1, int K2>
__global__ void __launch_bounds__(512, 1) dfx_k_emb_follow(DfxFanArgs A, DfxFollowSync Y) {
    __shared__ int gslot;
    DfxWaiter W{Y.spin_limit, Y.err};
    const int g = dfx_xcd_claim(Y.xclaim ? Y.x.prod : nullptr, Y.x.tag, Y.groups, Y.xclaim, (int)blockIdx.x, W, &gslot);
    const int tid = threadIdx.x, wave = tid >> 6;
    const int64_t b0 = (int64_t)g * 16;
    const int nclip = (int)(Y.B - b0 < 16 ? Y.B - b0 : 16);
    if (nclip <= 0) return;
    const int H = 32 * A.nj, EMB = 64 * A.nj;
    A.y += b0 * Y.T * H;
    if (A.res) A.res += b0 * Y.T * EMB;
    if (A.emb_out) A.emb_out += b0 * Y.T * EMB;
#pragma unroll
    for (int c = 0; c < DFX_FAN_NC; ++c)
        if (A.out[c]) A.out[c] += b0 * Y.T * H;
    if (A.lsnr) A.lsnr += b0 * Y.T;
    A.parts = 1;
    DfxXcd X = Y.x;
    if (X.me) X.me += g, X.prod = X.prod ? X.prod + g : nullptr, X.cons = X.cons ? X.cons + g : nullptr, X.cons2 = X.cons2 ? X.cons2 + g : nullptr;
    dfx_xcd_register(X);
    for (int64_t t0 = 0; t0 < Y.T; t0 += DFX_EF_STEPS) {
        const int64_t t1 = t0 + DFX_EF_STEPS < Y.T ? t0 + DFX_EF_STEPS : Y.T;
        if (tid == 0) W.wait_ge<4>(Y.src + g, Y.pbase + (unsigned int)t1);
        __syncthreads();
        dfx_xcd_acquire(X);
        A.rm = DfxRowMap{Y.T, t1 - t0, t0};
        A.R = (int64_t)nclip * (t1 - t0);
        const int ntile = (int)((A.R + 15) / 16);
        for (int tile = wave; tile < ntile; tile += 8) dfx_emb_fan_item<1, K0, K1, K2>(A, tile, 0, A.nj);
        DFX_VMEM_DRAIN();
        __syncthreads();
        if (tid == 0) dfx_sync_raise(Y.dst + g, Y.pbase + (unsigned int)t1, false);
    }
}

struct DfxEncFanArgs {
    const float *c1;
    const float4 *w1;
    const float4 *w2;
    const float *e3;
    float *emb_out;
    float *out;
    int64_t R;
    int ng;
    int parts;
    DfxRowMap rm;
};
template <int RT>
__global__ void __launch_bounds__(256, 2) dfx_k_enc_fan(DfxEncFanArgs A) {
    const int lane = threadIdx.x & 63, n = lane & 15, q = lane >> 4;
    const int K = 96 * A.ng, EMB = 16 * A.ng, H = 8 * A.ng;
    const int64_t ntile = (A.R + 16 * RT - 1) / (16 * RT);
    const int gper = A.ng / A.parts;
    for (int64_t item = (int64_t)blockIdx.x * 4 + (threadIdx.x >> 6); item < ntile * A.parts; item += (int64_t)gridDim.x * 4) {
        const int64_t tile = item / A.parts;
        const int g0 = (int)(item - tile * A.parts) * gper, g1 = g0 + gper;
        int64_t prow[RT];
        bool ok[RT];
#pragma unroll
        for (int rt = 0; rt < RT; ++rt) {
            const int64_t lr = tile * (16 * RT) + 16 * rt + n;
            ok[rt] = lr < A.R;
            prow[rt] = ok[rt] ? dfx_row(A.rm, lr) : 0;
        }
        float4 wn[6], yn[RT][6];
        auto request = [&](int g) {
#pragma unroll
            for (int i = 0; i < 6; ++i) wn[i] = A.w1[((size_t)g * 6 + i) * 64 + lane];
#pragma unroll
            for (int rt = 0; rt < RT; ++rt)
#pragma unroll
                for (int i = 0; i < 6; ++i)
                    yn[rt][i] = ok[rt] ? *reinterpret_cast<const float4 *>(A.c1 + prow[rt] * K + 96 * g + 16 * i + 4 * q) : make_float4(0.f, 0.f, 0.f, 0.f);
        };
        request(g0);
        float e[RT][2][4];
        for (int g = g0; g < g1; ++g) {
            float4 w[6], y[RT][6];
#pragma unroll
            for (int i = 0; i < 6; ++i) w[i] = wn[i];
#pragma unroll
            for (int rt = 0; rt < RT; ++rt)
#pragma unroll
                for (int i = 0; i < 6; ++i) y[rt][i] = yn[rt][i];
            const int t = g & 1;
            float4 w2[2];
            if (t) {
                w2[0] = A.w2[((size_t)(g >> 1) * 2 + 0) * 64 + lane];
                w2[1] = A.w2[((size_t)(g >> 1) * 2 + 1) * 64 + lane];
            }
            if (g + 1 < g1) request(g + 1);
#pragma unroll
            for (int rt = 0; rt < RT; ++rt) {
                f32x4 d = f32x4{0.f, 0.f, 0.f, 0.f};
#pragma unroll
                for (int i = 0; i < 6; ++i) {
                    const float ws[4] = {w[i].x, w[i].y, w[i].z, w[i].w}, ys[4] = {y[rt][i].x, y[rt][i].y, y[rt][i].z, y[rt][i].w};
#pragma unroll
                    for (int k = 0; k < 4; ++k) d = __builtin_amdgcn_mfma_f32_16x16x4f32(ws[k], ys[k], d, 0, 0, 0);
                }
                const int64_t eoff = prow[rt] * EMB + 16 * g + 4 * q;
                float4 rv = make_float4(0.f, 0.f, 0.f, 0.f);
                if (ok[rt]) rv = *reinterpret_cast<const float4 *>(A.e3 + eoff);
                float ev[4] = {fmaxf(d[0], 0.f) + rv.x, fmaxf(d[1], 0.f) + rv.y, fmaxf(d[2], 0.f) + rv.z, fmaxf(d[3], 0.f) + rv.w};
                if (A.emb_out && ok[rt]) *reinterpret_cast<float4 *>(A.emb_out + eoff) = make_float4(ev[0], ev[1], ev[2], ev[3]);
                if (t == 0) {
#pragma unroll
                    for (int r = 0; r < 4; ++r) e[rt][0][r] = ev[r];
                } else {
#pragma unroll
                    for (int r = 0; r < 4; ++r) e[rt][1][r] = ev[r];
                    f32x4 o = f32x4{0.f, 0.f, 0.f, 0.f};
#pragma unroll
                    for (int tt = 0; tt < 2; ++tt) {
                        const float ws[4] = {w2[tt].x, w2[tt].y, w2[tt].z, w2[tt].w};
#pragma unroll
                        for (int r = 0; r < 4; ++r) o = __builtin_amdgcn_mfma_f32_16x16x4f32(ws[r], e[rt][tt][r], o, 0, 0, 0);
                    }
                    if (ok[rt])
                        *reinterpret_cast<float4 *>(A.out + prow[rt] * H + 16 * (g >> 1) + 4 * q) =
                            make_float4(fmaxf(o[0], 0.f), fmaxf(o[1], 0.f), fmaxf(o[2], 0.f), fmaxf(o[3], 0.f));
                }
            }
        }
    }
}

__global__ void dfx_k_lsnr(const float *emb, const float *w, float bias, float scale, float offset, float *out, int64_t R,
                           int D) {
    const int lane = threadIdx.x & 63;
    const int64_t row = ((int64_t)blockIdx.x * blockDim.x + threadIdx.x) >> 6;
    if (row >= R) return;
    float acc = 0.f;
    const float *e = emb + row * D;
    if ((D & 255) == 0 && ((reinterpret_cast<uintptr_t>(e) | reinterpret_cast<uintptr_t>(w)) & 15) == 0) {
        for (int i = 4 * lane; i < D; i += 256) {
            const float4 ev = *reinterpret_cast<const float4 *>(e + i), wv = *reinterpret_cast<const float4 *>(w + i);
            acc += ev.x * wv.x;
            acc += ev.y * wv.y;
            acc += ev.z * wv.z;
            acc += ev.w * wv.w;
        }
    } else {
        for (int i = lane; i < D; i += 64) acc += e[i] * w[i];
    }
    for (int off = 32; off > 0; off >>= 1) acc += __shfl_xor(acc, off);
    if (lane == 0) out[row] = dfx_sigmoid(acc + bias) * scale + offset;
}

__global__ void dfx_k_lsnr_rows(const float *emb, const float *w, float bias, float scale, float offset, float *out, int64_t R, int D, DfxRowMap rm) {
    const int lane = threadIdx.x & 63;
    const int64_t lrow = ((int64_t)blockIdx.x * blockDim.x + threadIdx.x) >> 6;
    if (lrow >= R) return;
    const int64_t row = dfx_row(rm, lrow);
    float acc = 0.f;
    const float *e = emb + row * D;
    for (int i = 4 * lane; i < D; i += 256) {
        const float4 ev = *reinterpret_cast<const float4 *>(e + i), wv = *reinterpret_cast<const float4 *>(w + i);
        acc += ev.x * wv.x;
        acc += ev.y * wv.y;
        acc += ev.z * wv.z;
        acc += ev.w * wv.w;
    }
    for (int off = 32; off > 0; off >>= 1) acc += __shfl_xor(acc, off);
    if (lane == 0) out[row] = dfx_sigmoid(acc + bias) * scale + offset;
}

__global__ void dfx_k_add(const float *a, const float *b, float *out, int64_t n) {
    for (int64_t i = (int64_t)blockIdx.x * blockDim.x + threadIdx.x; i < n; i += (int64_t)gridDim.x * blockDim.x)
        out[i] = a[i] + b[i];
}

#define DFX_GRU_H 256
#define DFX_GRU_ROWS 2
#define DFX_GRU_THREADS 512
#define DFX_GRU_KR 14
#define DFX_GRU_KL 6
#define DFX_GRU_KS (32 - DFX_GRU_KR - DFX_GRU_KL)
#define DFX_GRU_SMEM ((size_t)DFX_GRU_KL * 3 * DFX_GRU_THREADS * 16 + (size_t)2 * DFX_GRU_ROWS * DFX_GRU_H * 4)

__global__ void __launch_bounds__(DFX_GRU_THREADS, 2) dfx_k_gru_rec(const float *gi, const float4 *__restrict__ whh4,
                                                                    const float *bhn, const float *h_in, float *h_out,
                                                                    float *y, int64_t B, int64_t T) {
    constexpr int H = DFX_GRU_H, MR = DFX_GRU_ROWS, KR = DFX_GRU_KR, KL = DFX_GRU_KL, KS = DFX_GRU_KS, NT = DFX_GRU_THREADS;
    static_assert(KS >= 2 && KS % 2 == 0 && MR == 2, "ring of two single-block buffers, lane pair = row pair");
// ... 353 lines not shown
                    wlo[i] = ring[SC.idx[f] % D][1];
                }
            });
            constexpr int ta = DFX_GH_POS_TILE(f0), tb_ = DFX_GH_POS_TILE(f0 + 1), tc = DFX_GH_POS_TILE(f0 + 2);
            if constexpr (X32) {
                const f32x4 b0 = __builtin_bit_cast(f32x4, bh[kc & 1]), b1 = __builtin_bit_cast(f32x4, bl[kc & 1]);
                const f32x4 a0[3] = {__builtin_bit_cast(f32x4, whi[0]), __builtin_bit_cast(f32x4, whi[1]), __builtin_bit_cast(f32x4, whi[2])};
                const f32x4 a1[3] = {__builtin_bit_cast(f32x4, wlo[0]), __builtin_bit_cast(f32x4, wlo[1]), __builtin_bit_cast(f32x4, wlo[2])};
#pragma unroll
                for (int j = 0; j < 4; ++j) {
                    acc[ta] = __builtin_amdgcn_mfma_f32_16x16x4f32(a0[0][j], b0[j], acc[ta], 0, 0, 0);
                    acc[tb_] = __builtin_amdgcn_mfma_f32_16x16x4f32(a0[1][j], b0[j], acc[tb_], 0, 0, 0);
                    acc[tc] = __builtin_amdgcn_mfma_f32_16x16x4f32(a0[2][j], b0[j], acc[tc], 0, 0, 0);
                }
#pragma unroll
                for (int j = 0; j < 4; ++j) {
                    acc[ta] = __builtin_amdgcn_mfma_f32_16x16x4f32(a1[0][j], b1[j], acc[ta], 0, 0, 0);
                    acc[tb_] = __builtin_amdgcn_mfma_f32_16x16x4f32(a1[1][j], b1[j], acc[tb_], 0, 0, 0);
                    acc[tc] = __builtin_amdgcn_mfma_f32_16x16x4f32(a1[2][j], b1[j], acc[tc], 0, 0, 0);
                }
            } else if (!(DFX_GH_ABLATE & 4)) {
                acc[ta] = dfx_mfma_16x16x32_f16(wlo[0], bh[kc & 1], acc[ta]);
                acc[tb_] = dfx_mfma_16x16x32_f16(wlo[1], bh[kc & 1], acc[tb_]);
                acc[tc] = dfx_mfma_16x16x32_f16(wlo[2], bh[kc & 1], acc[tc]);
                acc[ta] = dfx_mfma_16x16x32_f16(whi[0], bl[kc & 1], acc[ta]);
                acc[tb_] = dfx_mfma_16x16x32_f16(whi[1], bl[kc & 1], acc[tb_]);
                acc[tc] = dfx_mfma_16x16x32_f16(whi[2], bl[kc & 1], acc[tc]);
                acc[ta] = dfx_mfma_16x16x32_f16(whi[0], bh[kc & 1], acc[ta]);
                acc[tb_] = dfx_mfma_16x16x32_f16(whi[1], bh[kc & 1], acc[tb_]);
                acc[tc] = dfx_mfma_16x16x32_f16(whi[2], bh[kc & 1], acc[tc]);
            } else {
                acc[ta][0] += (float)whi[0][0] + (float)wlo[0][1] + (float)bh[kc & 1][0] + (float)bl[kc & 1][0];
                acc[tb_][0] += (float)whi[1][0] + (float)wlo[1][1] + (float)bh[kc & 1][0] + (float)bl[kc & 1][0];
                acc[tc][0] += (float)whi[2][0] + (float)wlo[2][1] + (float)bh[kc & 1][0] + (float)bl[kc & 1][0];
            }
            DFX_SCHED_BARRIER();
            dfx_static_for<0, 3>([&](auto ic) {
                constexpr int f = f0 + decltype(ic)::value;
                if constexpr (SC.cls[f] == 2 && !(DFX_GH_ABLATE & 1)) {
                    constexpr int nxt = SC.spos[(SC.idx[f] + D) % FS];
                    ring[SC.idx[f] % D][0] = wst[DFX_GH_GIDX(nxt)];
                    ring[SC.idx[f] % D][1] = wst[DFX_GH_GIDX(nxt) + 64];
                }
            });
            DFX_SCHED_BARRIER();
        });
#pragma unroll
        for (int s = 0; s < NS; ++s) {
#pragma unroll
            for (int r = 0; r < 4; ++r) gate_unit(s, r);
            gate_finish(s);
        }
        const bool ypub = SEQ && Y.yprog && (((t + 1) & (Y.yblk - 1)) == 0 || t + 1 == A.T);
        if (ypub) DFX_VMEM_DRAIN();
        __syncthreads();
        cur ^= 1;
        if (ypub && tid == 0) dfx_xcd_release(Y.x, Y.yprog, Y.pbase + (unsigned int)(t + 1));
    }
    if (SEQ) {
        __builtin_amdgcn_fence(__ATOMIC_RELEASE, "agent");
        __syncthreads();
        if (tid == 0) dfx_sync_raise(Y.done + grp, Y.base + (unsigned int)ck + 1u, false);
        if (tid == 0 && Y.trace) Y.trace[ck * 3 + 2] = wall_clock64();
    }
    }
    if (A.h_out && valid) {
#pragma unroll
        for (int s = 0; s < NS; ++s)
            *reinterpret_cast<float4 *>(A.h_out + brow * H + UW * wave + 16 * s + 4 * q) = make_float4(hp[s][0], hp[s][1], hp[s][2], hp[s][3]);
    }
}
#undef DFX_GH_GIDX

template <bool X32>
static __device__ __forceinline__ void dfx_gru_rec_body(const DfxGhArgs &A) {
    int64_t grp = blockIdx.x;
    if (A.xcd_mask) {
        const int x = dfx_xcc_id();
        if (!((A.xcd_mask >> x) & 1)) return;
        grp = (int64_t)(blockIdx.x >> 3) * __builtin_popcount(A.xcd_mask) + __builtin_popcount(A.xcd_mask & ((1 << x) - 1));
        if (grp * DFX_GH_ROWS >= A.B) return;
    }
    dfx_gru_h3_run<false, X32>(A, grp, DfxGhSync{nullptr, nullptr, 0u, 1, nullptr, nullptr, nullptr, 0});
}
__global__ void __launch_bounds__(DFX_GH_THREADS, DFX_GH_NW / 4) dfx_k_gru_rec_h3(DfxGhArgs A) { dfx_gru_rec_body<false>(A); }
__global__ void __launch_bounds__(DFX_GH_THREADS, DFX_GH_NW / 4) dfx_k_gru_rec_x32(DfxGhArgs A) { dfx_gru_rec_body<true>(A); }

struct DfxGsArgs {
    const float *gi[DFX_GS_MAX_LAYERS];
    float *y[DFX_GS_MAX_LAYERS];
    const dfx_h8 *whf[DFX_GS_MAX_LAYERS];
    const float *bhn[DFX_GS_MAX_LAYERS];
    float unscale[DFX_GS_MAX_LAYERS];
    int64_t B, T;
    int nlayers, groups, K;
    int tb[DFX_GS_MAX_CHUNKS + 1];
    unsigned int *ready;
    unsigned int *done;
    int done_stride;
    unsigned int base;
    unsigned int *err;
    unsigned long long *trace;
    int spin_limit;
    unsigned int *yprog[DFX_GS_MAX_LAYERS] = {};
    unsigned int *giprog[DFX_GS_MAX_LAYERS] = {};
    unsigned int pbase = 0;
    int sblk = 16;
    int yblk[DFX_GS_MAX_LAYERS] = {};
    unsigned int *xtab = nullptr;
    int xstride = 0;
    int xcons_kind[DFX_GS_MAX_LAYERS] = {}, xcons_layer[DFX_GS_MAX_LAYERS] = {};
    unsigned int xtag = 0;
    unsigned int *xstat = nullptr;
    int pair_far = 0;
    unsigned int *psync = nullptr;
};
template <bool X32>
static __device__ __forceinline__ void dfx_gru_seq_body(const DfxGsArgs &S) {
    const int l = (int)(blockIdx.x / (unsigned)S.groups), g = (int)(blockIdx.x % (unsigned)S.groups);
    if (l >= S.nlayers) return;
    DfxGhArgs A;
    A.gi = S.gi[l];
    A.whf = S.whf[l];
    A.bhn = S.bhn[l];
    A.h_in = nullptr;
    A.h_out = nullptr;
    A.y = S.y[l];
    A.B = S.B;
    A.T = S.T;
    A.t0 = 0;
    A.t1 = S.T;
    A.unscale = S.unscale[l];
    A.xcd_mask = 0;
    DfxGhSync Y{S.ready + l, S.done + (size_t)l * S.done_stride, S.base, S.K, S.tb, S.err,
                S.trace ? S.trace + ((size_t)l * S.groups + g) * S.K * 3 : nullptr, S.spin_limit};
    Y.yprog = S.yprog[l] ? S.yprog[l] + g : nullptr;
    Y.giprog = S.giprog[l] ? S.giprog[l] + g : nullptr;
    Y.pbase = S.pbase, Y.sblk = S.sblk, Y.yblk = S.yblk[l] > 0 ? S.yblk[l] : 16;
    if (S.xtab) {
        auto word = [&](int kind, int layer) { return S.xtab + ((size_t)kind * DFX_GS_MAX_LAYERS + layer) * S.xstride + g; };
        Y.x.me = word(0, l);
        Y.x.prod = Y.giprog ? word(1, l) : nullptr;
        Y.x.cons = Y.yprog ? word(S.xcons_kind[l], S.xcons_layer[l]) : nullptr;
        Y.x.tag = S.xtag, Y.x.stat = S.xstat;
    }
    dfx_gru_h3_run<true, X32>(A, g, Y);
}
__global__ void __launch_bounds__(DFX_GH_THREADS, DFX_GH_NW / 4) dfx_k_gru_seq(DfxGsArgs S) { dfx_gru_seq_body<false>(S); }
__global__ void __launch_bounds__(DFX_GH_THREADS, DFX_GH_NW / 4) dfx_k_gru_seq_x32(DfxGsArgs S) { dfx_gru_seq_body<true>(S); }

#include "dfx_gru_pair.h"

#define DFX_PF_MAX 4
struct DfxPfArgs {
    const float *x[DFX_PF_MAX];
    float *gi[DFX_PF_MAX];
    const dfx_h8 *wf[DFX_PF_MAX];
    const float *bias[DFX_PF_MAX];
    float unscale[DFX_PF_MAX];
    const unsigned int *yprog[DFX_PF_MAX];
    unsigned int *giprog[DFX_PF_MAX];
    int64_t B, T;
    int nf, groups;
    unsigned int pbase;
    unsigned int *err;
    int spin_limit;
    const unsigned int *xprod[DFX_PF_MAX] = {};
    unsigned int *xme[DFX_PF_MAX] = {};
    const unsigned int *xcons[DFX_PF_MAX] = {};
    unsigned int xtag = 0;
    unsigned int *xstat = nullptr;
    const unsigned int *xrec = nullptr;
    unsigned int *xclaim = nullptr;
};
static __device__ __forceinline__ DfxXcd dfx_pf_xcd(const DfxPfArgs &A, int f, int g) {
    DfxXcd X;
    if (A.xme[f]) X.me = A.xme[f] + g, X.prod = A.xprod[f] ? A.xprod[f] + g : nullptr, X.cons = A.xcons[f] ? A.xcons[f] + g : nullptr, X.tag = A.xtag, X.stat = A.xstat;
    return X;
}
static __device__ __forceinline__ bool dfx_pf_begin(const DfxPfArgs &A, DfxWaiter &W, int *slot, int &f, int &g) {
    f = (int)(blockIdx.x / (unsigned)A.groups);
    if (f >= A.nf) return false;
    g = dfx_xcd_claim(A.xrec ? (A.xcons[f] ? A.xcons[f] : A.xrec) : nullptr, A.xtag, A.groups,
                      A.xclaim ? A.xclaim + 8 * f : nullptr, (int)(blockIdx.x % (unsigned)A.groups), W, slot);
    dfx_xcd_register(dfx_pf_xcd(A, f, g));
    return true;
}
static __device__ __forceinline__ void dfx_pf_wait_block(const DfxPfArgs &A, DfxWaiter &W, int f, int g, int t1) {
    if (threadIdx.x == 0) W.wait_ge<4>(A.yprog[f] + g, A.pbase + (unsigned int)t1);
    __syncthreads();
    dfx_xcd_acquire(dfx_pf_xcd(A, f, g));
}
static __device__ __forceinline__ void dfx_pf_raise_block(const DfxPfArgs &A, int f, int g, int t1) {
    if (threadIdx.x == 0) dfx_xcd_release(dfx_pf_xcd(A, f, g), A.giprog[f] + g, A.pbase + (unsigned int)t1);
}
__global__ void __launch_bounds__(512, 1) dfx_k_proj_follow(DfxPfArgs A) {
    constexpr int NW = 8, CT = 4, NTH = 64 * NW, SB = 2 * NW, N = 768;
    constexpr int CH8 = 8 * CT * 2 * 64;
    constexpr int PER_T = CH8 / NTH;
    DFX_DYN_SMEM(dfx_h8, ws);
    DfxWaiter W{A.spin_limit, A.err};
    int f, g;
    if (!dfx_pf_begin(A, W, reinterpret_cast<int *>(ws), f, g)) return;
    const int tid = threadIdx.x, lane = tid & 63, wave = tid >> 6, q = lane >> 4, jl = lane & 15;
    constexpr int nchunks = N / (16 * CT);
    const int T = (int)A.T;
    for (int t0 = 0; t0 < T; t0 += SB) {
        const int t1 = t0 + SB < T ? t0 + SB : T;
        int zoff = 0, jz = jl;
        DFX_OPAQUE(zoff);
        DFX_OPAQUE(jz);
        const dfx_h8 *wf = A.wf[f] + zoff;
        const float *bias = A.bias[f] + zoff;
        const int64_t clip = (int64_t)g * 16 + jz;
        const bool okc = clip < A.B;
        const float *xrow = A.x[f] + (okc ? clip : 0) * A.T * 256 + 8 * q;
        float *orow = A.gi[f] + (okc ? clip : 0) * A.T * N;
#pragma unroll
        for (int i = 0; i < PER_T; ++i) ws[i * NTH + tid] = wf[i * NTH + tid];
        dfx_pf_wait_block(A, W, f, g, t1);
        dfx_h8 xh[2][8], xl[2][8];
        float unscale[2];
        int trow[2];
        bool okr[2];
#pragma unroll
        for (int t = 0; t < 2; ++t) {
            trow[t] = t0 + 2 * wave + t;
            okr[t] = okc && trow[t] < t1;
            if (!okr[t]) trow[t] = t0;
            unscale[t] = A.unscale[f] * dfx_row256_split(xrow + trow[t] * 256, okr[t], xh[t], xl[t]);
        }
        for (int c = 0; c < nchunks; ++c) {
            const dfx_h8 *wc = ws + (size_t)(c & 1) * CH8;
            constexpr int HP = PER_T / 2;
            dfx_h8 pre[HP];
            const dfx_h8 *src = wf + (size_t)(c + 1) * CH8;
            dfx_h8 *dst = ws + (size_t)((c + 1) & 1) * CH8;
            if (c + 1 < nchunks) {
#pragma unroll
                for (int i = 0; i < HP; ++i) pre[i] = src[i * NTH + tid];
            }
            f32x4 acc[2][CT];
#pragma unroll
            for (int t = 0; t < 2; ++t)
#pragma unroll
                for (int ct = 0; ct < CT; ++ct) acc[t][ct] = f32x4{0.f, 0.f, 0.f, 0.f};
#pragma unroll
            for (int kc = 0; kc < 8; ++kc) {
                dfx_h8 whi[CT], wlo[CT];
#pragma unroll
                for (int ct = 0; ct < CT; ++ct) {
                    whi[ct] = wc[((kc * CT + ct) * 2 + 0) * 64 + lane];
                    wlo[ct] = wc[((kc * CT + ct) * 2 + 1) * 64 + lane];
                }
#pragma unroll
                for (int ct = 0; ct < CT; ++ct)
#pragma unroll
                    for (int t = 0; t < 2; ++t) acc[t][ct] = dfx_mfma_16x16x32_f16(wlo[ct], xh[t][kc], acc[t][ct]);
#pragma unroll
                for (int ct = 0; ct < CT; ++ct)
#pragma unroll
                    for (int t = 0; t < 2; ++t) acc[t][ct] = dfx_mfma_16x16x32_f16(whi[ct], xl[t][kc], acc[t][ct]);
#pragma unroll
                for (int ct = 0; ct < CT; ++ct)
#pragma unroll
                    for (int t = 0; t < 2; ++t) acc[t][ct] = dfx_mfma_16x16x32_f16(whi[ct], xh[t][kc], acc[t][ct]);
                if (kc == 3 && c + 1 < nchunks) {
#pragma unroll
                    for (int i = 0; i < HP; ++i) dst[i * NTH + tid] = pre[i];
#pragma unroll
                    for (int i = 0; i < HP; ++i) pre[i] = src[(HP + i) * NTH + tid];
                }
            }
#pragma unroll
            for (int ct = 0; ct < CT; ++ct) {
                const int n = c * (16 * CT) + 16 * ct + 4 * q;
                const float4 bz = *reinterpret_cast<const float4 *>(bias + n);
#pragma unroll
                for (int t = 0; t < 2; ++t)
                    if (okr[t])
                        *reinterpret_cast<float4 *>(orow + trow[t] * N + n) =
                            make_float4(acc[t][ct][0] * unscale[t] + bz.x, acc[t][ct][1] * unscale[t] + bz.y, acc[t][ct][2] * unscale[t] + bz.z,
                                        acc[t][ct][3] * unscale[t] + bz.w);
            }
            if (c + 1 < nchunks) {
#pragma unroll
                for (int i = 0; i < HP; ++i) dst[(HP + i) * NTH + tid] = pre[i];
            } else {
                DFX_VMEM_DRAIN();
            }
            __syncthreads();
        }
        dfx_pf_raise_block(A, f, g, t1);
    }
}

__global__ void __launch_bounds__(512, 1) dfx_k_proj_follow_x32(DfxPfArgs A) {
    constexpr int NW = 8, CT = 4, NTH = 64 * NW, SB = 2 * NW, N = 768, K = 256;
    constexpr int CHF = K * 16 * CT;
    constexpr int PER_T = CHF / 4 / NTH;
    constexpr int HP = PER_T / 2;
    DFX_DYN_SMEM(float, wsf);
    DfxWaiter W{A.spin_limit, A.err};
    int f, g;
    if (!dfx_pf_begin(A, W, reinterpret_cast<int *>(wsf), f, g)) return;
    const int tid = threadIdx.x, lane = tid & 63, wave = tid >> 6, q = lane >> 4, jl = lane & 15;
    constexpr int nchunks = N / (16 * CT);
    const int T = (int)A.T;
    const int kt = tid >> 4, n4 = tid & 15;
    const int src_off = kt * N + 4 * n4;
    const int dst_off0 = 4 * kt * 64 + 4 * n4, dst_off1 = 4 * kt * 64 + ((4 * n4) ^ 16);
    auto piece_src = [&](const float *w, int c, int i) -> const f32x4 * {
        return reinterpret_cast<const f32x4 *>(w + src_off + 32 * i * N + 64 * c);
    };
    auto piece_dst = [&](float *buf, int i) -> f32x4 * {
        return reinterpret_cast<f32x4 *>(buf + (((i >> 1) & 1) ? dst_off1 : dst_off0) + (128 * (i & 1) + (i >> 1)) * 64);
    };
    for (int t0 = 0; t0 < T; t0 += SB) {
        const int t1 = t0 + SB < T ? t0 + SB : T;
        int zoff = 0, jz = jl;
        DFX_OPAQUE(zoff);
        DFX_OPAQUE(jz);
        const float *w = reinterpret_cast<const float *>(A.wf[f]) + zoff;
        const float *bias = A.bias[f] + zoff;
        const int64_t clip = (int64_t)g * 16 + jz;
        const bool okc = clip < A.B;
        const float *xrow = A.x[f] + (okc ? clip : 0) * A.T * K + 64 * q;
        float *orow = A.gi[f] + (okc ? clip : 0) * A.T * N;
#pragma unroll
        for (int i = 0; i < PER_T; ++i) *piece_dst(wsf, i) = *piece_src(w, 0, i);
        dfx_pf_wait_block(A, W, f, g, t1);
        float4 xv[2][16];
        int trow[2];
        bool okr[2];
#pragma unroll
        for (int t = 0; t < 2; ++t) {
            trow[t] = t0 + 2 * wave + t;
            okr[t] = okc && trow[t] < t1;
            if (!okr[t]) trow[t] = t0;
            const float4 *p = reinterpret_cast<const float4 *>(xrow + trow[t] * K);
#pragma unroll
            for (int v = 0; v < 16; ++v) xv[t][v] = okr[t] ? p[v] : make_float4(0.f, 0.f, 0.f, 0.f);
        }
        for (int c = 0; c < nchunks; ++c) {
            const float *wc = wsf + (size_t)(c & 1) * CHF + q * 64 + jl;
            float *dstb = wsf + (size_t)((c + 1) & 1) * CHF;
            f32x4 pre[HP];
            if (c + 1 < nchunks) {
#pragma unroll
                for (int i = 0; i < HP; ++i) pre[i] = *piece_src(w, c + 1, i);
            }
            f32x4 acc[2][CT];
#pragma unroll
            for (int t = 0; t < 2; ++t)
#pragma unroll
                for (int ct = 0; ct < CT; ++ct) acc[t][ct] = f32x4{0.f, 0.f, 0.f, 0.f};
            float fa[2][CT];
#pragma unroll
            for (int ct = 0; ct < CT; ++ct) fa[0][ct] = wc[16 * (ct ^ (q & 1))];
            auto ksteps = [&](auto kc) {
                constexpr int ks = decltype(kc)::value;
                if constexpr (ks + 1 < 64) {
#pragma unroll
                    for (int ct = 0; ct < CT; ++ct) fa[(ks + 1) & 1][ct] = wc[(ks + 1) * 256 + 16 * (ct ^ (q & 1))];
                }
#pragma unroll
                for (int t = 0; t < 2; ++t) {
                    const float4 x4 = xv[t][ks >> 2];
                    const float xk = (ks & 3) == 0 ? x4.x : (ks & 3) == 1 ? x4.y : (ks & 3) == 2 ? x4.z : x4.w;
#pragma unroll
                    for (int ct = 0; ct < CT; ++ct) acc[t][ct] = __builtin_amdgcn_mfma_f32_16x16x4f32(fa[ks & 1][ct], xk, acc[t][ct], 0, 0, 0);
                }
                DFX_SCHED_BARRIER();
            };
            dfx_static_for<0, 32>(ksteps);
            if (c + 1 < nchunks) {
#pragma unroll
                for (int i = 0; i < HP; ++i) *piece_dst(dstb, i) = pre[i];
#pragma unroll
                for (int i = 0; i < HP; ++i) pre[i] = *piece_src(w, c + 1, HP + i);
            }
            dfx_static_for<32, 64>(ksteps);
            DFX_MFMA_GUARD();
#pragma unroll
            for (int ct = 0; ct < CT; ++ct) {
                const int n = c * (16 * CT) + 16 * ct + 4 * q;
                const float4 bz = *reinterpret_cast<const float4 *>(bias + n);
#pragma unroll
                for (int t = 0; t < 2; ++t)
                    if (okr[t])
                        *reinterpret_cast<float4 *>(orow + trow[t] * N + n) =
                            make_float4(acc[t][ct][0] + bz.x, acc[t][ct][1] + bz.y, acc[t][ct][2] + bz.z, acc[t][ct][3] + bz.w);
            }
            if (c + 1 < nchunks) {
#pragma unroll
                for (int i = 0; i < HP; ++i) *piece_dst(dstb, HP + i) = pre[i];
            } else {
                DFX_VMEM_DRAIN();
            }
            __syncthreads();
        }
        dfx_pf_raise_block(A, f, g, t1);
    }
}
```

deepfilternet_amd/model.py:

```python
from __future__ import annotations

import ctypes as C
import glob
import os
import re
from typing import Dict, Optional, Tuple

import numpy as np
import torch

from . import _lib
from .config import ModelParams
from .libdf import DF

def make_cfg(p: ModelParams) -> _lib.ModelCfg:
    p.check_supported()
    return p.to_cfg()


def tensor_manifest(cfg: _lib.ModelCfg):
    L = _lib.lib()
    n = C.c_int()
    _lib.check(L.dfx_model_tensor_count(C.byref(cfg), C.byref(n)))
    out = []
    name = C.create_string_buffer(256)
    shape = (C.c_int64 * 4)()
    nd, off = C.c_int(), C.c_int64()
    for i in range(n.value):
        _lib.check(L.dfx_model_tensor_info(C.byref(cfg), i, name, 256, shape, C.byref(nd), C.byref(off)))
        out.append((name.value.decode(), tuple(int(shape[k]) for k in range(nd.value)), int(off.value)))
    return out


def pack_state_dict(cfg: _lib.ModelCfg, sd: Dict[str, "np.ndarray | torch.Tensor"], strict: bool = True,
                    warn=None) -> np.ndarray:
    import warnings

    warn = warn or (lambda msg: warnings.warn(msg, stacklevel=3))
    total = C.c_int64()
    _lib.check(_lib.lib().dfx_model_blob_floats(C.byref(cfg), C.byref(total)))
    blob = np.zeros(total.value, dtype=np.float32)
    for name, shape, off in tensor_manifest(cfg):
        v = sd.get(name)
        if v is not None:
            v = v.detach().cpu().numpy() if isinstance(v, torch.Tensor) else np.asarray(v)
            if tuple(v.shape) != shape:
                if strict:
                    raise ValueError(f"size mismatch for {name}: checkpoint {tuple(v.shape)}, model {shape}")
                warn(f"size mismatch for {name}: copying a param with shape {tuple(v.shape)} from checkpoint, the shape in current "
                     f"model is {shape}. (dropped)")
                v = None
        elif strict:
            raise KeyError(f"state dict is missing '{name}'")
        else:
            warn(f"Missing key: '{name}'")
        n = int(np.prod(shape)) if shape else 1
        if v is None:
            leaf = name.rsplit(".", 1)[-1]
            is_bn = len(shape) == 1 and ".gru." not in name and "lsnr_fc" not in name
            fill = 1.0 if is_bn and leaf in ("weight", "running_var") else 0.0
            blob[off:off + n] = fill
        else:
            blob[off:off + n] = v.astype(np.float32, copy=False).ravel()
    return blob


class DfNet:

    def __init__(self, p: ModelParams, state_dict: Dict[str, "np.ndarray | torch.Tensor"], df_state: Optional[DF] = None,
                 run_df: bool = True, strict: bool = True):
        self.p = p
        self.cfg = make_cfg(p)
        blob = pack_state_dict(self.cfg, state_dict, strict=strict)
        h = C.c_void_p()
        _lib.check(_lib.lib().dfx_model_create(C.byref(self.cfg), blob.ctypes.data_as(C.POINTER(C.c_float)), C.byref(h)))
        self._h = h
        self.run_df = bool(run_df)
        if not self.run_df:
            _lib.check(_lib.lib().dfx_model_set_run_df(self._h, 0))
        self.df_state = df_state or DF(p.sr, p.fft_size, p.hop_size, p.nb_erb, p.min_nb_freqs)
        self.nb_df = p.nb_df
        self.df_order = p.df_order
        self.df_lookahead = p.df_lookahead
        self.freq_bins = p.freq_bins
        self.erb_bins = p.nb_erb
        self.post_filter = p.mask_pf
        self._ws: Optional[torch.Tensor] = None

    def __del__(self):
        h, self._h = getattr(self, "_h", None), None
        try:
            if h:
                _lib.lib().dfx_model_free(h)
        except Exception:
            pass

    @property
    def handle(self) -> C.c_void_p:
        return self._h

    def set_streams(self, enable: bool) -> None:
        _lib.check(_lib.lib().dfx_model_set_streams(self._h, int(bool(enable))))

    def set_pipeline(self, time_chunks: int = 6, min_chunk_frames: int = 32, batch_chunks: int = 1) -> None:
        _lib.check(_lib.lib().dfx_model_set_pipeline(self._h, int(time_chunks), int(min_chunk_frames), int(batch_chunks)))

    def check(self) -> None:
        _lib.check(_lib.lib().dfx_model_check(self._h))

    def poll(self) -> None:
        _lib.check(_lib.lib().dfx_model_poll(self._h))

    Q_GRU_PERSISTENT, Q_HWQ_PROBE, Q_EXACT_FP32, Q_SPIN_LIMIT, Q_PASSES_PERSISTENT, Q_PASSES_TICKET_BUSY = 1, 2, 3, 4, 5, 6
    Q_PASSES_C0_PRESPLIT = 7
    Q_LAST_PLAN = 8
    Q_PASSES_PAIR = 9
    PLAN_BITS = {"fan": 1 << 0, "fan_skp": 1 << 1, "fuse_h3": 1 << 2, "presplit": 1 << 3, "fuse_tail": 1 << 4, "fuse_enc": 1 << 5,
                 "fuse_enc4": 1 << 6, "enc_fan": 1 << 7, "dfenc": 1 << 8, "c0_fused": 1 << 9, "pipe": 1 << 10, "use_seq": 1 << 11,
                 "rows_finish": 1 << 14, "fuse_dec": 1 << 15}
    PLAN_DF_OUT_SHIFT, PLAN_DF_OUT_FORMS = 12, {0: "none", 1: "resident", 2: "streaming", 3: "ggemm"}

    def last_plan(self) -> Dict[str, object]:
        v = self.query(self.Q_LAST_PLAN)
        d: Dict[str, object] = {k: bool(v & b) for k, b in self.PLAN_BITS.items()}
        d["df_out"] = self.PLAN_DF_OUT_FORMS[(v >> self.PLAN_DF_OUT_SHIFT) & 3]
        return d

    def query(self, what: int) -> int:
        v = C.c_int64()
        _lib.check(_lib.lib().dfx_model_query(self._h, int(what), C.byref(v)))
        return int(v.value)

    def eval(self):
        return self

    def to(self, *a, **k):
        return self

    def workspace(self, nbytes: int) -> torch.Tensor:
        if self._ws is None or self._ws.numel() < nbytes or not _lib.on_device(self._ws):
            self._ws = None
            self._ws = torch.empty(int(nbytes), dtype=torch.uint8, device=_lib.device())
        return self._ws

    @torch.no_grad()
    def __call__(self, spec: torch.Tensor, feat_erb: torch.Tensor, feat_spec: torch.Tensor, atten_lim: float = 0.0
                 ) -> Tuple[torch.Tensor, torch.Tensor, torch.Tensor, torch.Tensor]:
        p = self.p
        dev = _lib.device()
        B, _, T, F, _ = spec.shape
        spec_d = spec.to(dev, torch.float32).contiguous()
        fe = feat_erb.to(dev, torch.float32).contiguous()
        fs = feat_spec.to(dev, torch.float32).contiguous()
        assert F == p.freq_bins and fe.shape == (B, 1, T, p.nb_erb) and fs.shape == (B, 1, T, p.nb_df, 2)
        spec_e = torch.empty_like(spec_d)
        m = torch.empty((B, 1, T, p.nb_erb), dtype=torch.float32, device=dev)
        lsnr = torch.empty((B, T, 1), dtype=torch.float32, device=dev)
        coefs = torch.empty((B, p.df_order, T, p.nb_df, 2), dtype=torch.float32, device=dev)
        nbytes = C.c_int64()
        L = _lib.lib()
        _lib.check(L.dfx_model_workspace_bytes(self._h, B, T, C.byref(nbytes)))
        ws = self.workspace(nbytes.value)
        _lib.check(L.dfx_model_forward(self._h, self.df_state.bands_handle, _lib.ptr(spec_d), _lib.ptr(fe), _lib.ptr(fs),
                                       B, T, float(atten_lim), _lib.ptr(spec_e), _lib.ptr(m), _lib.ptr(lsnr),
                                       _lib.ptr(coefs), _lib.ptr(ws), ws.numel(), _lib.stream()))
        if not self.run_df:
            coefs = torch.zeros((), device=dev)
        self.poll()
        return spec_e, m, lsnr, coefs

    forward = __call__


def _find_checkpoint(dirname: str, epoch) -> Tuple[Optional[str], int]:
    if not dirname or not os.path.isdir(dirname):
        return None, 0
    cps = glob.glob(os.path.join(dirname, "model_*.ckpt*"))
    if not cps:
        return None, 0

    def ep(path):
        mm = re.search(r"model_(\d+)\.ckpt", os.path.basename(path))
        return int(mm.group(1)) if mm else -1

    if isinstance(epoch, int) or (isinstance(epoch, str) and epoch.isdigit()):
        want = int(epoch)
        for c in cps:
            if ep(c) == want:
                return c, want
        return None, 0
    if epoch == "best":
        best = [c for c in cps if c.endswith(".best")]
        if best:
            c = max(best, key=ep)
            return c, ep(c)
    c = max(cps, key=ep)
    return c, ep(c)


def read_cp(dirname: str, epoch="best") -> Tuple[Optional[Dict[str, torch.Tensor]], int]:
    path, ep = _find_checkpoint(dirname, epoch)
    if path is None:
        return None, 0
    sd = torch.load(path, map_location="cpu")
    if isinstance(sd, dict) and "model" in sd and isinstance(sd["model"], dict):
        sd = sd["model"]
    out = {}
    for k, v in sd.items():
        out[k.replace("clc", "df")] = v
    return out, ep


def read_onnx_targz(path: str) -> Tuple[ModelParams, Dict[str, np.ndarray]]:
    L = _lib.lib()
    cfg = _lib.ModelCfg()
    n = C.c_int64()
    _lib.check(L.dfx_onnx_targz_read(os.fsencode(path), C.byref(cfg), None, 0, C.byref(n)))
    blob = np.empty(n.value, dtype=np.float32)
    _lib.check(L.dfx_onnx_targz_read(os.fsencode(path), C.byref(cfg), blob.ctypes.data_as(C.POINTER(C.c_float)), n.value, C.byref(n)))
    return _from_cfg_blob(cfg, blob)


def read_dfx(path: str) -> Tuple[ModelParams, Dict[str, np.ndarray]]:
    import struct

    with open(path, "rb") as f:
        data = f.read()
    if data[:4] != b"DFXM" or len(data) < 12:
        raise ValueError(f"{path}: not a .dfx model file")
    ver, csz = struct.unpack_from("<II", data, 4)
    if ver not in (1, 2) or csz > C.sizeof(_lib.ModelCfg) or len(data) < 20 + csz:
        raise ValueError(f"{path}: .dfx model file of version {ver} / configuration size {csz}: re-export it with export_dfx")
    cfg = _lib.ModelCfg()
    C.memmove(C.addressof(cfg), data[12:12 + csz], csz)
    (n,) = struct.unpack_from("<q", data, 12 + csz)
    if n < 0 or len(data) < 20 + csz + 4 * n:
        raise ValueError(f"{path}: truncated .dfx model file")
    return _from_cfg_blob(cfg, np.frombuffer(data, dtype="<f4", count=n, offset=20 + csz))


def _from_cfg_blob(cfg: _lib.ModelCfg, blob: np.ndarray) -> Tuple[ModelParams, Dict[str, np.ndarray]]:
    skip = {0: "none", 1: "identity", 2: "groupedlinear"}
    p = ModelParams(sr=cfg.sr, fft_size=cfg.fft_size, hop_size=cfg.hop_size, nb_erb=cfg.nb_erb, nb_df=cfg.nb_df,
                    min_nb_freqs=cfg.min_nb_freqs, df_order=cfg.df_order, df_lookahead=cfg.df_lookahead, lsnr_min=cfg.lsnr_min,
                    lsnr_max=cfg.lsnr_max, conv_lookahead=cfg.conv_lookahead, conv_ch=cfg.conv_ch, emb_hidden_dim=cfg.emb_hidden_dim,
                    emb_num_layers=cfg.emb_num_layers, df_hidden_dim=cfg.df_hidden_dim, df_num_layers=cfg.df_num_layers,
                    df_gru_skip=skip[cfg.df_gru_skip], df_pathway_kernel_size_t=cfg.df_pathway_kernel_size_t, lin_groups=cfg.lin_groups,
                    enc_lin_groups=cfg.enc_lin_groups, mask_pf=bool(cfg.mask_pf), pf_beta=cfg.pf_beta,
                    emb_gru_skip_enc=skip[cfg.emb_gru_skip_enc], emb_gru_skip=skip[cfg.emb_gru_skip], enc_concat=bool(cfg.enc_concat),
                    norm_alpha_value=float(cfg.norm_alpha))
    sd = {}
    for name, shape, off in tensor_manifest(cfg):
        k = int(np.prod(shape)) if shape else 1
        sd[name] = blob[off:off + k].reshape(shape).copy()
    return p, sd


def export_dfx(path: str, model_base_dir: Optional[str] = None, epoch="best", *, params: Optional[ModelParams] = None,
               state_dict: Optional[Dict[str, "np.ndarray | torch.Tensor"]] = None) -> str:
    if params is None:
        if model_base_dir is None:
            raise ValueError("export_dfx needs a model directory or params= + state_dict=")
        params = ModelParams.from_ini(os.path.join(model_base_dir, "config.ini"), must_exist=True)
    if state_dict is None:
        if model_base_dir is None:
            raise ValueError("export_dfx needs a model directory or params= + state_dict=")
        state_dict, _ = read_cp(os.path.join(model_base_dir, "checkpoints"), epoch)
        if state_dict is None:
            raise FileNotFoundError("Could not find a checkpoint")
# ... 5 lines not shown
```

include/dfx.h:

```cpp
#ifndef DFX_H
#define DFX_H

#include <stddef.h>
#include <stdint.h>

#ifdef __cplusplus
extern "C" {
#endif

#define DFX_OK 0
#define DFX_ERR_INVALID_ARG 1
#define DFX_ERR_UNSUPPORTED 2
#define DFX_ERR_HIP 3
#define DFX_ERR_NO_DEVICE 4
#define DFX_ERR_ALLOC 5

#define DFX_VERSION 200

#define DFX_G711_ULAW 1
#define DFX_G711_ALAW 2
#define DFX_FMT_F32 0
#define DFX_FMT_PCM16 1
#define DFX_FMT_ULAW 2
#define DFX_FMT_ALAW 3

int dfx_version(void);
const char *dfx_status_string(int status);
const char *dfx_last_error(void);
int dfx_device_count(void);
int dfx_is_emulator(void);

typedef struct dfx_bands dfx_bands;
int dfx_bands_create(const uint64_t *widths_host, int nb_bands, dfx_bands **out);
void dfx_bands_free(dfx_bands *b);
int dfx_bands_nb(const dfx_bands *b);
int dfx_bands_nfreqs(const dfx_bands *b);

typedef struct dfx_state dfx_state;
int dfx_state_create(int sr, int fft_size, int hop_size, int nb_bands, int min_nb_erb_freqs, dfx_state **out);
void dfx_state_free(dfx_state *st);
int dfx_state_sr(const dfx_state *st);
int dfx_state_fft_size(const dfx_state *st);
int dfx_state_hop_size(const dfx_state *st);
int dfx_state_nb_erb(const dfx_state *st);
float dfx_state_wnorm(const dfx_state *st);
const dfx_bands *dfx_state_bands(const dfx_state *st);
int dfx_state_erb_widths(const dfx_state *st, uint64_t *out_host );
int dfx_state_fft_window(const dfx_state *st, float *out_host );
int dfx_erb_fb(int sr, int fft_size, int nb_bands, int min_nb_freqs, uint64_t *out_host);

int dfx_analysis(const dfx_state *st, const float *x, int64_t B, int64_t T, int64_t x_stride, const float *mem_in,
                 float *mem_out, float *spec, void *stream);

int dfx_synthesis(const dfx_state *st, const float *spec, int64_t B, int64_t Tf, const float *mem_in, float *mem_out,
                  float *out, int64_t out_stride, void *stream);

int dfx_erb(const dfx_bands *bands, const float *spec, int64_t rows, int db, float *out, void *stream);
int dfx_erb_inv(const dfx_bands *bands, const float *gains, int64_t rows, float *out, void *stream);
int dfx_erb_norm(float *x, int64_t C, int64_t T, int E, float alpha, float *state, void *stream);
int dfx_unit_norm(const float *x, int64_t x_frame_stride, float *out, int64_t C, int64_t T, int F, float alpha,
                  float *state, void *stream);
int dfx_unit_norm_init(int n, float *out_host);

int dfx_features(const dfx_state *st, const float *x, int64_t B, int64_t T, int64_t x_stride, int nb_df, float alpha,
                 float *spec, float *erb_feat, float *spec_feat, void *stream);

#define DFX_COEF_BOTF 0
#define DFX_COEF_BTFO 1
#define DFX_COEF_BTOF 2
int dfx_df_apply(const float *spec, const float *coefs, int coef_layout, const float *gains, const dfx_bands *bands,
                 int64_t B, int64_t T, int F, int nb_df, int order, int lookahead, float pf_beta, float atten_lim,
                 float *out, void *stream);
int dfx_df_apply_strided(const float *spec, int64_t spec_stride, const float *coefs, int coef_layout, const float *gains,
                         const dfx_bands *bands, int64_t B, int64_t T, int F, int nb_df, int order, int lookahead, float pf_beta,
                         float atten_lim, float *out, int64_t out_stride, void *stream);

#define DFX_SKIP_NONE 0
#define DFX_SKIP_IDENTITY 1
#define DFX_SKIP_GROUPEDLINEAR 2

typedef struct dfx_model_cfg {
    int32_t sr, fft_size, hop_size, nb_erb, nb_df, min_nb_freqs, df_order, df_lookahead;
    int32_t lsnr_min, lsnr_max;
    int32_t conv_lookahead, conv_ch, emb_hidden_dim, emb_num_layers, df_hidden_dim, df_num_layers;
    int32_t df_gru_skip;
    int32_t df_pathway_kernel_size_t, lin_groups, enc_lin_groups;
    int32_t mask_pf;
    float pf_beta;
    float norm_alpha;
    int32_t emb_gru_skip_enc, emb_gru_skip, enc_concat;
} dfx_model_cfg;

int dfx_model_tensor_count(const dfx_model_cfg *cfg, int *count);
int dfx_model_tensor_info(const dfx_model_cfg *cfg, int index, char *name_out, int name_cap, int64_t shape_out[4],
                          int *ndim_out, int64_t *offset_out );
int dfx_model_blob_floats(const dfx_model_cfg *cfg, int64_t *n);

typedef struct dfx_model dfx_model;
int dfx_model_create(const dfx_model_cfg *cfg, const float *blob_host, dfx_model **out);
void dfx_model_free(dfx_model *m);
int dfx_model_save_file(const dfx_model_cfg *cfg, const float *blob_host, const char *path);
int dfx_model_load_file(const char *path, dfx_model **out);
int dfx_onnx_targz_read(const char *path, dfx_model_cfg *cfg_out, float *blob_out, int64_t blob_cap, int64_t *blob_floats);
int dfx_model_cfg_get(const dfx_model *m, dfx_model_cfg *out);
int dfx_model_set_streams(dfx_model *m, int enable);
int dfx_model_set_run_df(dfx_model *m, int enable);
int dfx_model_set_pipeline(dfx_model *m, int time_chunks, int min_chunk_frames, int batch_chunks);
int dfx_model_poll(const dfx_model *m);
int dfx_model_check(const dfx_model *m);
#define DFX_Q_GRU_PERSISTENT 1
#define DFX_Q_HWQ_PROBE 2
#define DFX_Q_EXACT_FP32 3
#define DFX_Q_SPIN_LIMIT 4
#define DFX_Q_PASSES_PERSISTENT 5
#define DFX_Q_PASSES_TICKET_BUSY 6
#define DFX_Q_PASSES_C0_PRESPLIT 7
#define DFX_Q_PASSES_PAIR 9
#define DFX_Q_LAST_PLAN 8
#define DFX_PLAN_FAN (1 << 0)
#define DFX_PLAN_FAN_SKP (1 << 1)
#define DFX_PLAN_FUSE_H3 (1 << 2)
#define DFX_PLAN_PRESPLIT (1 << 3)
#define DFX_PLAN_FUSE_TAIL (1 << 4)
#define DFX_PLAN_FUSE_ENC (1 << 5)
#define DFX_PLAN_FUSE_ENC4 (1 << 6)
#define DFX_PLAN_ENC_FAN (1 << 7)
#define DFX_PLAN_DFENC (1 << 8)
#define DFX_PLAN_C0_FUSED (1 << 9)
#define DFX_PLAN_PIPE (1 << 10)
#define DFX_PLAN_USE_SEQ (1 << 11)
#define DFX_PLAN_DF_OUT_SHIFT 12
#define DFX_PLAN_DF_OUT_MASK (3 << DFX_PLAN_DF_OUT_SHIFT)
#define DFX_PLAN_DF_OUT_RESIDENT 1
#define DFX_PLAN_DF_OUT_STREAMING 2
#define DFX_PLAN_DF_OUT_GGEMM 3
#define DFX_PLAN_ROWS_FINISH (1 << 14)
#define DFX_PLAN_FUSE_DEC (1 << 15)
int dfx_model_query(const dfx_model *m, int what, int64_t *value);

int dfx_model_workspace_bytes(const dfx_model *m, int64_t B, int64_t T, int64_t *bytes);

int dfx_model_forward(const dfx_model *m, const dfx_bands *bands, const float *spec, const float *feat_erb,
                      const float *feat_spec, int64_t B, int64_t T, float atten_lim, float *spec_e, float *mask,
                      float *lsnr, float *df_coefs, void *workspace, int64_t workspace_bytes, void *stream);

int dfx_enhance_workspace_bytes(const dfx_model *m, const dfx_state *st, int64_t B, int64_t T, int pad, int64_t *bytes);
int dfx_enhance(const dfx_model *m, const dfx_state *st, const float *x, int64_t B, int64_t T, int pad,
                float atten_lim_db, float *y, void *workspace, int64_t workspace_bytes, void *stream);
int dfx_enhance_pcm16(const dfx_model *m, const dfx_state *st, const int16_t *x, int64_t B, int64_t T, int pad,
                      float atten_lim_db, int16_t *y, void *workspace, int64_t workspace_bytes, void *stream);
int dfx_enhance_varlen_workspace_bytes(const dfx_model *m, const dfx_state *st, int64_t B, const int64_t *lengths, int pad, int64_t *bytes);
int dfx_enhance_varlen(const dfx_model *m, const dfx_state *st, const float *x, int64_t B, int64_t x_stride, const int64_t *lengths,
                       int pad, float atten_lim_db, float *y, int64_t y_stride, void *workspace, int64_t workspace_bytes, void *stream);
int dfx_enhance_varlen_pcm16(const dfx_model *m, const dfx_state *st, const int16_t *x, int64_t B, int64_t x_stride, const int64_t *lengths,
                             int pad, float atten_lim_db, int16_t *y, int64_t y_stride, void *workspace, int64_t workspace_bytes, void *stream);

typedef struct dfx_stream_state dfx_stream_state;
int dfx_stream_create(const dfx_model *m, const dfx_state *st, int64_t streams, int max_frames, dfx_stream_state **out);
void dfx_stream_free(dfx_stream_state *s);
int dfx_stream_reset(dfx_stream_state *s, void *stream);
int dfx_stream_reset_streams(dfx_stream_state *s, const int64_t *ids, int64_t count, void *stream);
int dfx_stream_frames(const dfx_stream_state *s, int64_t *frames_out);
int dfx_stream_frame_length(const dfx_stream_state *s);
int dfx_stream_delay_frames(const dfx_stream_state *s);
int dfx_stream_set_atten_lim(dfx_stream_state *s, float lim_db);
int dfx_stream_set_atten_lim_enhance(dfx_stream_state *s, float atten_lim_db);
int dfx_stream_set_post_filter_beta(dfx_stream_state *s, float beta);
int dfx_stream_set_channels(dfx_stream_state *s, int channels, int reduce_mask);
int dfx_stream_set_gating(dfx_stream_state *s, int enable);
int dfx_stream_set_thresholds(dfx_stream_state *s, float min_db_thresh, float max_db_erb_thresh,
                              float max_db_df_thresh);
int dfx_stream_set_atten_lim_streams(dfx_stream_state *s, const int64_t *ids, int64_t count, const float *lim_db ,
                                     void *stream);
int dfx_stream_set_post_filter_beta_streams(dfx_stream_state *s, const int64_t *ids, int64_t count, const float *beta ,
                                            void *stream);
int dfx_stream_set_thresholds_streams(dfx_stream_state *s, const int64_t *ids, int64_t count, const float *thr ,
                                      void *stream);
int dfx_stream_get_settings(const dfx_stream_state *s, float *out_host);
int dfx_stream_process(dfx_stream_state *s, const float *x, int64_t n_frames, float *y, float *lsnr, void *stream);
int dfx_stream_set_pausable(dfx_stream_state *s, int enable);
int dfx_stream_process_active(dfx_stream_state *s, const float *x, int64_t n_frames, float *y, float *lsnr,
                              const unsigned char *active, void *stream);
int dfx_stream_process_raw(dfx_stream_state *s, const float *spec, float *gains, float *coefs, unsigned char *stages, float *lsnr,
                           void *stream);
int dfx_stream_set_sample_rate(dfx_stream_state *s, int sr, int lowpass_filter_width, double rolloff, int method, double beta);
int dfx_stream_sample_rate(const dfx_stream_state *s);
int64_t dfx_stream_resample_delay(const dfx_stream_state *s);
int dfx_stream_process_pcm16(dfx_stream_state *s, const int16_t *x, int64_t n_frames, int16_t *y, float *lsnr, const unsigned char *active,
                             void *stream);
int dfx_stream_process_g711(dfx_stream_state *s, const uint8_t *x, int law, int64_t n_frames, uint8_t *y, float *lsnr,
                            const unsigned char *active, void *stream);
int dfx_stream_process_ends(dfx_stream_state *s, const void *x, int x_format, int64_t n_frames, void *y, float *lsnr,
                            const int64_t *valid_hops, void *stream);
int dfx_stream_memory_bytes(const dfx_model *m, const dfx_state *st, int64_t streams, int max_frames, int64_t *bytes);
#define DFX_STREAM_META_MAGIC 0x53584644u
#define DFX_STREAM_META_VERSION 1u
typedef struct dfx_stream_meta {
    uint32_t magic, version;
    uint64_t fingerprint;
    int64_t age;
    float settings[5];
    int32_t pending_current;
} dfx_stream_meta;
int dfx_stream_snapshot_bytes(const dfx_stream_state *s, int64_t *bytes_per_stream);
int dfx_stream_export_streams(dfx_stream_state *s, const int64_t *ids, int64_t count, void *payload_dev ,
                              dfx_stream_meta *meta_host , void *stream);
int dfx_stream_import_streams(dfx_stream_state *s, const int64_t *ids, int64_t count, const void *payload_dev,
                              const dfx_stream_meta *meta_host, int with_settings, void *stream);

int dfx_mf_filter(const float *spec, const float *ifc, const float *mat, int op, int frame_size, int lookahead, int cholesky_decomp,
                  int inverse, int enforce_constraints, float eps, float dload, int64_t B, int64_t T, int F, int nb, float *out,
                  void *stream);

int dfx_pcm16_to_f32(const int16_t *pcm, int64_t n, float *out, void *stream);
int dfx_f32_to_pcm16(const float *x, int64_t n, int16_t *out, void *stream);
int dfx_g711_decode(const uint8_t *codes, int law, int64_t n, void *out, int out_is_pcm16, void *stream);
int dfx_g711_encode(const void *x, int x_is_pcm16, int law, int64_t n, uint8_t *out, void *stream);
typedef struct dfx_flac_info {
    int32_t sample_rate, channels, bits_per_sample, min_block, max_block;
    int32_t first_frame;
    int64_t total_samples;
    uint8_t md5[16];
} dfx_flac_info;
int dfx_flac_probe(const uint8_t *head, int64_t n, dfx_flac_info *out);
int dfx_flac_workspace_bytes(int64_t n_streams, const int64_t *lengths, const dfx_flac_info *infos, int64_t *bytes);
int dfx_flac_decode(const uint8_t *blob, int64_t blob_bytes, int64_t n_streams, const int64_t *offsets, const int64_t *lengths,
                    const dfx_flac_info *infos, const int64_t *out_offsets, void *out, int64_t out_bytes, int64_t *status, void *workspace,
                    int64_t workspace_bytes, void *stream);
typedef struct dfx_resampler dfx_resampler;
int dfx_resampler_create(int orig_sr, int new_sr, int lowpass_filter_width, double rolloff, int method, double beta,
                         dfx_resampler **out);
void dfx_resampler_free(dfx_resampler *r);
int64_t dfx_resampler_out_len(const dfx_resampler *r, int64_t in_len);
int dfx_resampler_kernel(int orig_sr, int new_sr, int lowpass_filter_width, double rolloff, int method, double beta, int *phases,
                         int *taps, int *width, float *w_host , int64_t cap_floats);
int dfx_resample(const dfx_resampler *r, const float *x, int64_t B, int64_t T, int64_t x_stride, float *y, int64_t y_stride,
                 void *stream);
typedef struct dfx_stream_resampler dfx_stream_resampler;
int dfx_stream_resampler_create(const dfx_resampler *r, int64_t rows, int64_t max_in_samples, dfx_stream_resampler **out);
void dfx_stream_resampler_free(dfx_stream_resampler *h);
int dfx_stream_resampler_reset(dfx_stream_resampler *h, const int64_t *rows , int64_t count, void *stream);
int dfx_stream_resampler_delay(const dfx_stream_resampler *h, int64_t *in_samples, int64_t *out_samples);
int dfx_stream_resampler_process(dfx_stream_resampler *h, const void *x, int x_format, int64_t in_len, int64_t x_stride, void *y,
                                 int y_format, int64_t y_stride, const unsigned char *active_host , void *stream);

int dfx_si_sdr_workspace_bytes(int64_t B, const int64_t *lengths_host, int64_t *bytes);
int dfx_si_sdr(const float *ref, const float *est, int64_t B, int64_t stride, const int64_t *lengths_host, float *out, void *workspace,
               int64_t workspace_bytes, void *stream);
int dfx_stoi_workspace_bytes(int fs_source, int64_t B, const int64_t *lengths_host, int64_t *bytes);
int dfx_stoi(const dfx_resampler *r, const float *clean, const float *degraded, int64_t B, int64_t stride, const int64_t *lengths_host,
             float *out, int32_t *info, void *workspace, int64_t workspace_bytes, void *stream);

int dfx_sepm_workspace_bytes(int fs_source, int64_t B, const int64_t *lengths_host, int64_t *bytes);
int dfx_sepm(const dfx_resampler *r, const float *clean, const float *processed, int64_t B, int64_t stride, const int64_t *lengths_host,
             double *out , int32_t *info , void *workspace, int64_t workspace_bytes,
             void *stream);

int dfx_prof_kernel_count(void);
const char *dfx_prof_kernel_name(int kernel_id);
int dfx_prof_enable(uint32_t kernel_mask);
int dfx_prof_reset(void);
int dfx_prof_read(int kernel_id, double *total_ms, int64_t *launches);

#ifdef __cplusplus
}
#endif
#endif
```

Baseline: 24.52 million frames/s.

## Let follow kernels serve two clip groups per workgroup; hoist bias loads

Adds an opt-in mode (DFX_FOLLOW_PAIRS, default off) where the projection-follow and embedding-follow kernels each handle two 16-clip groups per workgroup. This cuts their workgroup count so the follow chain fits the CU budget alongside paired GRU recurrences. The CU-budget check now counts recurrence, projection and embedding workgroups separately. Separately, the GRU projection kernels load bias before the MFMA loop, or stage it once in shared memory, and write the next weight chunk to shared memory before the output stores. This shortens the store epilogue but increases follow-kernel shared memory.

```diff
diff --git a/deepfilternet_amd/csrc/dfx_gru_sync.h b/deepfilternet_amd/csrc/dfx_gru_sync.h
--- a/deepfilternet_amd/csrc/dfx_gru_sync.h
+++ b/deepfilternet_amd/csrc/dfx_gru_sync.h
@@ -67,11 +67,12 @@
     dfx_sync_raise(flag, value, light);
     if (light && X.stat) __hip_atomic_fetch_add(X.stat, 1u, __ATOMIC_RELAXED, __HIP_MEMORY_SCOPE_AGENT);
 }
-static __device__ __forceinline__ int dfx_xcd_claim(const unsigned int *rec, unsigned int tag, int groups, unsigned int *claim, int fallback, DfxWaiter &W, int *slot) {
+static __device__ __forceinline__ int dfx_xcd_claim(const unsigned int *rec, unsigned int tag, int groups, unsigned int *claim, int fallback, DfxWaiter &W, int *slot,
+                                                    int stride = 1) {
     if (!rec || groups > 64) return fallback;
     if (threadIdx.x == 0) {
-        auto xcd_of = [&](int g) { return (int)(__hip_atomic_load(rec + g, __ATOMIC_RELAXED, __HIP_MEMORY_SCOPE_AGENT) & 15u) - 1; };
-        for (int g = 0; g < groups; ++g) W.wait_registered<4>(rec + g, tag);
+        auto xcd_of = [&](int g) { return (int)(__hip_atomic_load(rec + g * stride, __ATOMIC_RELAXED, __HIP_MEMORY_SCOPE_AGENT) & 15u) - 1; };
+        for (int g = 0; g < groups; ++g) W.wait_registered<4>(rec + g * stride, tag);
         int got = -1;
         const int x0 = dfx_xcc_id();
         for (int d = 0; d < 8 && got < 0 && !W.dead; ++d) {
diff --git a/deepfilternet_amd/csrc/dfx_model.hip b/deepfilternet_amd/csrc/dfx_model.hip
--- a/deepfilternet_amd/csrc/dfx_model.hip
+++ b/deepfilternet_amd/csrc/dfx_model.hip
@@ -441,6 +441,7 @@
     mutable unsigned int seq_pbase = 0;
     mutable int64_t passes_ps = 0;
     mutable int64_t passes_pair = 0;
+    mutable int64_t passes_follow_pairs = 0;
     mutable int64_t last_plan = 0;
     mutable int64_t passes_seq = 0, passes_ev = 0;
     mutable unsigned int seq_base = 0;
@@ -451,6 +452,7 @@
         int chunks = 0;
         bool gru_pair_far = false;
         bool gru_pair = true;
+        int follow_pairs = 0;
         int convp_late = -1;
         int p0_ahead = 3;
         int tail_every = 1;
@@ -1053,6 +1055,8 @@
     m->gru_seq = !is("DFX_GRU_SEQ", '0') && !dfx_env_is_emulator();
     if (getenv("DFX_GRU_PAIR")) m->sw.gru_pair = !is("DFX_GRU_PAIR", '0');
     m->sw.gru_pair_far = is("DFX_GRU_PAIR_FAR", '1');
+    if (const char *v = getenv("DFX_FOLLOW_PAIRS"))
+        if (v[0] >= '0' && v[0] <= '3' && !v[1]) m->sw.follow_pairs = v[0] - '0';
     m->check_every_pass = is("DFX_CHECK_EVERY_PASS", '1');
     at_least("DFX_SYNC_SPIN_LIMIT", 1, &m->spin_limit);
     if (const char *v = getenv("DFX_CONVP_ELEMS"))
@@ -1231,6 +1235,7 @@
         case DFX_Q_PASSES_C0_PRESPLIT: *value = m->passes_ps; return DFX_OK;
         case DFX_Q_LAST_PLAN: *value = m->last_plan; return DFX_OK;
         case DFX_Q_PASSES_PAIR: *value = m->passes_pair; return DFX_OK;
+        case DFX_Q_PASSES_FOLLOW_PAIRS: *value = m->passes_follow_pairs; return DFX_OK;
     }
     DFX_FAIL(DFX_ERR_INVALID_ARG, "dfx_model_query: unknown item %d", what);
 }
diff --git a/deepfilternet_amd/csrc/dfx_model_forward.h b/deepfilternet_amd/csrc/dfx_model_forward.h
--- a/deepfilternet_amd/csrc/dfx_model_forward.h
+++ b/deepfilternet_amd/csrc/dfx_model_forward.h
@@ -510,18 +510,24 @@
         bool followed[DFX_MAX_GRU_LAYERS] = {};
         int nfollow = 0;
         const int lfirst_df = 1 + ndec;
+        const bool use_pair = m->sw.gru_pair && !m->exact_fp32 && groups >= 2 && m->d_psync;
+        int follow_pairs = use_pair ? m->sw.follow_pairs : 0;
+        const int64_t npairs = (groups + 1) / 2;
+        const int64_t wg_rec = use_pair ? 2 * npairs : groups, wg_proj = (follow_pairs & 1) ? npairs : groups, wg_emb = (follow_pairs & 2) ? npairs : groups;
         const bool follow_emb = fan && c.emb_gru_skip_enc != DFX_SKIP_GROUPEDLINEAR && nl < DFX_MAX_GRU_LAYERS &&
-                                (nl + nl) * groups <= dfx_env_num_cus() * 3 / 4 && nl - 1 <= DFX_PF_MAX;
+                                nl * wg_rec + (nl - 1) * wg_proj + wg_emb <= dfx_env_num_cus() * 3 / 4 && nl - 1 <= DFX_PF_MAX;
         for (int l = 1; l < nl; ++l) {
             const bool first = l == 1 || l == lfirst_df;
             if (!first || follow_emb) followed[l] = true, ++nfollow;
         }
-        if (nfollow > DFX_PF_MAX || (nl + nfollow + 1) * groups > dfx_env_num_cus() * 3 / 4) {
+        if (nfollow > DFX_PF_MAX || nl * wg_rec + nfollow * wg_proj + wg_emb > dfx_env_num_cus() * 3 / 4) {
             nfollow = 0;
             for (int l = 0; l < nl; ++l) followed[l] = false;
         }
-        const bool use_pair = m->sw.gru_pair && !m->exact_fp32 && groups >= 2 && m->d_psync;
+        if (!followed[1]) follow_pairs &= ~2;
+        if (!nfollow) follow_pairs = 0;
         m->passes_pair += use_pair ? 1 : 0;
+        m->passes_follow_pairs += follow_pairs ? 1 : 0;
         if (nfollow || use_pair) m->seq_pbase += (unsigned int)T + 1u;
         auto proj_pub = [&](const GruW &g, int l, int k, const float *xin, hipStream_t st) -> int {
             DfxPublish pub;
@@ -590,15 +596,16 @@
             F.xtag = xtag, F.xstat = xstat;
             F.xrec = xword(0, 0), F.xclaim = xstat + 8;
             F.B = B, F.T = T, F.nf = nfollow, F.groups = groups, F.pbase = pbase, F.err = m->d_err, F.spin_limit = m->spin_limit;
+            F.per_pair = follow_pairs & 1;
             int lq = -1;
             for (int l = nl - 1; l >= 2 && lq < 0; --l)
                 if (followed[l]) lq = l;
             hipStream_t Fq = lq > 0 ? ln->ps[lq] : Dq;
-            DFX_HIP(dfx_env_set_max_dyn_smem(m->exact_fp32 ? (const void *)dfx_k_proj_follow_x32 : (const void *)dfx_k_proj_follow, DFX_PH_SMEM));
+            DFX_HIP(dfx_env_set_max_dyn_smem(m->exact_fp32 ? (const void *)dfx_k_proj_follow_x32 : (const void *)dfx_k_proj_follow, DFX_PF_SMEM));
             if ((rc = wait(ev_go, Fq))) return rc;
             DfxKScope ks(DFX_K_PROJ, Fq);
-            if (m->exact_fp32) dfx_launch(dfx_k_proj_follow_x32, dim3((unsigned)(nfollow * groups)), dim3(512), DFX_PH_SMEM, Fq, F);
-            else dfx_launch(dfx_k_proj_follow, dim3((unsigned)(nfollow * groups)), dim3(512), DFX_PH_SMEM, Fq, F);
+            if (m->exact_fp32) dfx_launch(dfx_k_proj_follow_x32, dim3((unsigned)(nfollow * wg_proj)), dim3(512), DFX_PF_SMEM, Fq, F);
+            else dfx_launch(dfx_k_proj_follow, dim3((unsigned)(nfollow * wg_proj)), dim3(512), DFX_PF_SMEM, Fq, F);
             DFX_LAUNCH_CHECK();
         }
         if (followed[1]) {
@@ -609,15 +616,16 @@
             DfxFollowSync EY;
             EY.x.me = xword(2, 0), EY.x.prod = xword(0, 0), EY.x.cons = xword(1, 1), EY.x.cons2 = followed[lfirst_df] ? xword(1, lfirst_df) : nullptr;
             EY.x.tag = xtag, EY.x.stat = xstat;
-            EY.xclaim = xstat + 8 + 8 * DFX_PF_MAX, EY.groups = groups;
+            EY.xclaim = xstat + 8 + 8 * DFX_PF_MAX, EY.groups = groups, EY.per_pair = (follow_pairs & 2) ? 1 : 0;
+            const unsigned int egrid = (unsigned int)((follow_pairs & 2) ? npairs : groups);
             EY.src = yprog, EY.dst = embprog, EY.pbase = pbase, EY.err = m->d_err, EY.spin_limit = m->spin_limit, EY.B = B, EY.T = T;
             hipStream_t Eq2 = ln->ps[1];
             if ((rc = wait(ev_go, Eq2))) return rc;
             {
                 DfxKScope ks(DFX_K_EMB_FAN, Eq2);
-                if (dfg_x && skp) dfx_launch((dfx_k_emb_follow<1, 2, 1>), dim3((unsigned)groups), dim3(512), 0, Eq2, EA, EY);
-                else if (dfg_x) dfx_launch((dfx_k_emb_follow<1, 2, 0>), dim3((unsigned)groups), dim3(512), 0, Eq2, EA, EY);
-                else dfx_launch((dfx_k_emb_follow<1, 0, 0>), dim3((unsigned)groups), dim3(512), 0, Eq2, EA, EY);
+                if (dfg_x && skp) dfx_launch((dfx_k_emb_follow<1, 2, 1>), dim3(egrid), dim3(512), 0, Eq2, EA, EY);
+                else if (dfg_x) dfx_launch((dfx_k_emb_follow<1, 2, 0>), dim3(egrid), dim3(512), 0, Eq2, EA, EY);
+                else dfx_launch((dfx_k_emb_follow<1, 0, 0>), dim3(egrid), dim3(512), 0, Eq2, EA, EY);
                 DFX_LAUNCH_CHECK();
             }
             if ((rc = signal(EV_EMB, Eq2))) return rc;
diff --git a/deepfilternet_amd/csrc/dfx_nn_kernels.h b/deepfilternet_amd/csrc/dfx_nn_kernels.h
--- a/deepfilternet_amd/csrc/dfx_nn_kernels.h
+++ b/deepfilternet_amd/csrc/dfx_nn_kernels.h
@@ -3093,6 +3093,9 @@
     __syncthreads();
     for (int c = cfirst; c < nchunks; ++c) {
         const dfx_h8 *wc = ws + (size_t)(c & 1) * DFX_PH_CHUNK_H8;
+        float4 bz[4];
+#pragma unroll
+        for (int ct = 0; ct < 4; ++ct) bz[ct] = *reinterpret_cast<const float4 *>(A.bias + c * DFX_PH_NC + 16 * ct + 4 * q);
         dfx_h8 pre[PER_T];
         if (c + 1 < nchunks) {
             const dfx_h8 *src = A.wf + (size_t)(c + 1) * DFX_PH_CHUNK_H8;
@@ -3117,19 +3120,18 @@
 #pragma unroll
             for (int ct = 0; ct < 4; ++ct) acc[ct] = dfx_mfma_16x16x32_f16(whi[ct], xh[kc], acc[ct]);
         }
+        if (c + 1 < nchunks) {
+            dfx_h8 *dst = ws + (size_t)((c + 1) & 1) * DFX_PH_CHUNK_H8;
+#pragma unroll
+            for (int i = 0; i < PER_T; ++i) dst[i * DFX_PH_THREADS + tid] = pre[i];
+        }
         if (ok) {
 #pragma unroll
             for (int ct = 0; ct < 4; ++ct) {
                 const int n = c * DFX_PH_NC + 16 * ct + 4 * q;
-                const float4 bz = *reinterpret_cast<const float4 *>(A.bias + n);
-                *reinterpret_cast<float4 *>(A.out + m * A.N + n) =
-                    make_float4(acc[ct][0] * unscale + bz.x, acc[ct][1] * unscale + bz.y, acc[ct][2] * unscale + bz.z, acc[ct][3] * unscale + bz.w);
-            }
-        }
-        if (c + 1 < nchunks) {
-            dfx_h8 *dst = ws + (size_t)((c + 1) & 1) * DFX_PH_CHUNK_H8;
-#pragma unroll
-            for (int i = 0; i < PER_T; ++i) dst[i * DFX_PH_THREADS + tid] = pre[i];
+                *reinterpret_cast<float4 *>(A.out + m * A.N + n) = make_float4(acc[ct][0] * unscale + bz[ct].x, acc[ct][1] * unscale + bz[ct].y,
+                                                                               acc[ct][2] * unscale + bz[ct].z, acc[ct][3] * unscale + bz[ct].w);
+            }
         }
         __syncthreads();
     }
@@ -3378,6 +3380,9 @@
     __syncthreads();
     for (int c = 0; c < nchunks; ++c) {
         const dfx_h8 *wc = ws + (size_t)(c & 1) * CH8;
+        float4 bz[CT];
+#pragma unroll
+        for (int ct = 0; ct < CT; ++ct) bz[ct] = *reinterpret_cast<const float4 *>(A.bias + c * (16 * CT) + 16 * ct + 4 * q);
         dfx_h8 pre[PER_T];
         if (c + 1 < nchunks && !(DFX_PH_ABLATE & 8)) {
 #pragma unroll
@@ -3409,21 +3414,27 @@
 #pragma unroll
                 for (int t = 0; t < 2; ++t) acc[t][ct] = (DFX_PH_ABLATE & 4) ? acc[t][ct] : dfx_mfma_16x16x32_f16(whi[ct], xh[t][kc], acc[t][ct]);
         }
+        if (c + 1 < nchunks && !(DFX_PH_ABLATE & 2)) {
+            dfx_h8 *dst = ws + (size_t)((c + 1) & 1) * CH8;
+#pragma unroll
+            for (int i = 0; i < PER_T; ++i) dst[i * DFX_PH2_THREADS + tid] = pre[i];
+        }
+#pragma unroll
+        for (int ct = 0; ct < CT; ++ct) {
+            DFX_OPAQUE(bz[ct].x);
+            DFX_OPAQUE(bz[ct].y);
+            DFX_OPAQUE(bz[ct].z);
+            DFX_OPAQUE(bz[ct].w);
+        }
 #pragma unroll
         for (int ct = 0; ct < CT; ++ct) {
             const int n = c * (16 * CT) + 16 * ct + 4 * q;
-            const float4 bz = *reinterpret_cast<const float4 *>(A.bias + n);
 #pragma unroll
             for (int t = 0; t < 2; ++t)
                 if (okr[t] && (!(DFX_PH_ABLATE & 1) || acc[t][ct][0] == 1.2345e-30f))
                     *reinterpret_cast<float4 *>(A.out + mrow[t] * A.N + n) =
-                        make_float4(acc[t][ct][0] * unscale[t] + bz.x, acc[t][ct][1] * unscale[t] + bz.y, acc[t][ct][2] * unscale[t] + bz.z,
-                                    acc[t][ct][3] * unscale[t] + bz.w);
-        }
-        if (c + 1 < nchunks && !(DFX_PH_ABLATE & 2)) {
-            dfx_h8 *dst = ws + (size_t)((c + 1) & 1) * CH8;
-#pragma unroll
-            for (int i = 0; i < PER_T; ++i) dst[i * DFX_PH2_THREADS + tid] = pre[i];
+                        make_float4(acc[t][ct][0] * unscale[t] + bz[ct].x, acc[t][ct][1] * unscale[t] + bz[ct].y, acc[t][ct][2] * unscale[t] + bz[ct].z,
+                                    acc[t][ct][3] * unscale[t] + bz[ct].w);
         }
         __syncthreads();
     }
@@ -3573,15 +3584,18 @@
     DfxXcd x;
     unsigned int *xclaim = nullptr;
     int groups = 0;
+    int per_pair = 0;
 };
 template <int K0, int K1, int K2>
 __global__ void __launch_bounds__(512, 1) dfx_k_emb_follow(DfxFanArgs A, DfxFollowSync Y) {
     __shared__ int gslot;
     DfxWaiter W{Y.spin_limit, Y.err};
-    const int g = dfx_xcd_claim(Y.xclaim ? Y.x.prod : nullptr, Y.x.tag, Y.groups, Y.xclaim, (int)blockIdx.x, W, &gslot);
+    const int gper = Y.per_pair ? 2 : 1, units = (Y.groups + gper - 1) / gper;
+    const int g = gper * dfx_xcd_claim(Y.xclaim ? Y.x.prod : nullptr, Y.x.tag, units, Y.xclaim, (int)blockIdx.x, W, &gslot, gper);
+    const int ng = g + gper <= Y.groups ? gper : 1;
     const int tid = threadIdx.x, wave = tid >> 6;
     const int64_t b0 = (int64_t)g * 16;
-    const int nclip = (int)(Y.B - b0 < 16 ? Y.B - b0 : 16);
+    const int nclip = (int)(Y.B - b0 < 16 * ng ? Y.B - b0 : 16 * ng);
     if (nclip <= 0) return;
     const int H = 32 * A.nj, EMB = 64 * A.nj;
     A.y += b0 * Y.T * H;
@@ -3592,21 +3606,27 @@
         if (A.out[c]) A.out[c] += b0 * Y.T * H;
     if (A.lsnr) A.lsnr += b0 * Y.T;
     A.parts = 1;
-    DfxXcd X = Y.x;
+    DfxXcd X = Y.x, X1 = Y.x;
     if (X.me) X.me += g, X.prod = X.prod ? X.prod + g : nullptr, X.cons = X.cons ? X.cons + g : nullptr, X.cons2 = X.cons2 ? X.cons2 + g : nullptr;
     dfx_xcd_register(X);
+    if (ng == 2) {
+        if (X1.me) X1.me += g + 1, X1.prod = X1.prod ? X1.prod + g + 1 : nullptr;
+        dfx_xcd_register(X1);
+    }
     for (int64_t t0 = 0; t0 < Y.T; t0 += DFX_EF_STEPS) {
         const int64_t t1 = t0 + DFX_EF_STEPS < Y.T ? t0 + DFX_EF_STEPS : Y.T;
-        if (tid == 0) W.wait_ge<4>(Y.src + g, Y.pbase + (unsigned int)t1);
+        if (tid == 0)
+            for (int i = 0; i < ng; ++i) W.wait_ge<4>(Y.src + g + i, Y.pbase + (unsigned int)t1);
         __syncthreads();
-        dfx_xcd_acquire(X);
+        dfx_sync_acquire(dfx_xcd_same(X, X.prod) && (ng == 1 || dfx_xcd_same(X1, X1.prod)));
         A.rm = DfxRowMap{Y.T, t1 - t0, t0};
         A.R = (int64_t)nclip * (t1 - t0);
         const int ntile = (int)((A.R + 15) / 16);
         for (int tile = wave; tile < ntile; tile += 8) dfx_emb_fan_item<1, K0, K1, K2>(A, tile, 0, A.nj);
         DFX_VMEM_DRAIN();
         __syncthreads();
-        if (tid == 0) dfx_sync_raise(Y.dst + g, Y.pbase + (unsigned int)t1, false);
+        if (tid == 0)
+            for (int i = 0; i < ng; ++i) dfx_sync_raise(Y.dst + g + i, Y.pbase + (unsigned int)t1, false);
     }
 }
 
@@ -4266,6 +4286,7 @@
 #include "dfx_gru_pair.h"
 
 #define DFX_PF_MAX 4
+#define DFX_PF_SMEM (DFX_PH_SMEM + (size_t)768 * 4)
 struct DfxPfArgs {
     const float *x[DFX_PF_MAX];
     float *gi[DFX_PF_MAX];
@@ -4286,18 +4307,21 @@
     unsigned int *xstat = nullptr;
     const unsigned int *xrec = nullptr;
     unsigned int *xclaim = nullptr;
+    int per_pair = 0;
 };
 static __device__ __forceinline__ DfxXcd dfx_pf_xcd(const DfxPfArgs &A, int f, int g) {
     DfxXcd X;
     if (A.xme[f]) X.me = A.xme[f] + g, X.prod = A.xprod[f] ? A.xprod[f] + g : nullptr, X.cons = A.xcons[f] ? A.xcons[f] + g : nullptr, X.tag = A.xtag, X.stat = A.xstat;
     return X;
 }
-static __device__ __forceinline__ bool dfx_pf_begin(const DfxPfArgs &A, DfxWaiter &W, int *slot, int &f, int &g) {
-    f = (int)(blockIdx.x / (unsigned)A.groups);
+static __device__ __forceinline__ bool dfx_pf_begin(const DfxPfArgs &A, DfxWaiter &W, int *slot, int &f, int &g, int &ng) {
+    const int gper = A.per_pair ? 2 : 1, units = (A.groups + gper - 1) / gper;
+    f = (int)(blockIdx.x / (unsigned)units);
     if (f >= A.nf) return false;
-    g = dfx_xcd_claim(A.xrec ? (A.xcons[f] ? A.xcons[f] : A.xrec) : nullptr, A.xtag, A.groups,
-                      A.xclaim ? A.xclaim + 8 * f : nullptr, (int)(blockIdx.x % (unsigned)A.groups), W, slot);
-    dfx_xcd_register(dfx_pf_xcd(A, f, g));
+    g = gper * dfx_xcd_claim(A.xrec ? (A.xcons[f] ? A.xcons[f] : A.xrec) : nullptr, A.xtag, units,
+                             A.xclaim ? A.xclaim + 8 * f : nullptr, (int)(blockIdx.x % (unsigned)units), W, slot, gper);
+    ng = g + gper <= A.groups ? gper : 1;
+    for (int i = 0; i < ng; ++i) dfx_xcd_register(dfx_pf_xcd(A, f, g + i));
     return true;
 }
 static __device__ __forceinline__ void dfx_pf_wait_block(const DfxPfArgs &A, DfxWaiter &W, int f, int g, int t1) {
@@ -4314,18 +4338,21 @@
     constexpr int PER_T = CH8 / NTH;
     DFX_DYN_SMEM(dfx_h8, ws);
     DfxWaiter W{A.spin_limit, A.err};
-    int f, g;
-    if (!dfx_pf_begin(A, W, reinterpret_cast<int *>(ws), f, g)) return;
-    const int tid = threadIdx.x, lane = tid & 63, wave = tid >> 6, q = lane >> 4, jl = lane & 15;
+    int f, g0, ng;
+    if (!dfx_pf_begin(A, W, reinterpret_cast<int *>(ws), f, g0, ng)) return;
+    const int tid = threadIdx.x, lane = tid & 63, q = lane >> 4, jl = lane & 15;
+    const int wave = dfx_wave_uniform(tid >> 6);
     constexpr int nchunks = N / (16 * CT);
     const int T = (int)A.T;
-    for (int t0 = 0; t0 < T; t0 += SB) {
+    float4 *bl = reinterpret_cast<float4 *>(ws + 2 * CH8);
+    if (tid < N / 4) bl[tid] = reinterpret_cast<const float4 *>(A.bias[f])[tid];
+    for (int t0 = 0; t0 < T; t0 += SB)
+    for (int g = g0; g < g0 + ng; ++g) {
         const int t1 = t0 + SB < T ? t0 + SB : T;
         int zoff = 0, jz = jl;
         DFX_OPAQUE(zoff);
         DFX_OPAQUE(jz);
         const dfx_h8 *wf = A.wf[f] + zoff;
-        const float *bias = A.bias[f] + zoff;
         const int64_t clip = (int64_t)g * 16 + jz;
         const bool okc = clip < A.B;
         const float *xrow = A.x[f] + (okc ? clip : 0) * A.T * 256 + 8 * q;
@@ -4386,10 +4413,16 @@
                     for (int i = 0; i < HP; ++i) pre[i] = src[(HP + i) * NTH + tid];
                 }
             }
+            if (c + 1 < nchunks) {
+#pragma unroll
+                for (int i = 0; i < HP; ++i) dst[(HP + i) * NTH + tid] = pre[i];
+            }
+            int bo = c * (4 * CT) + q;
+            DFX_OPAQUE(bo);
 #pragma unroll
             for (int ct = 0; ct < CT; ++ct) {
                 const int n = c * (16 * CT) + 16 * ct + 4 * q;
-                const float4 bz = *reinterpret_cast<const float4 *>(bias + n);
+                const float4 bz = bl[bo + 4 * ct];
 #pragma unroll
                 for (int t = 0; t < 2; ++t)
                     if (okr[t])
@@ -4397,12 +4430,7 @@
                             make_float4(acc[t][ct][0] * unscale[t] + bz.x, acc[t][ct][1] * unscale[t] + bz.y, acc[t][ct][2] * unscale[t] + bz.z,
                                         acc[t][ct][3] * unscale[t] + bz.w);
             }
-            if (c + 1 < nchunks) {
-#pragma unroll
-                for (int i = 0; i < HP; ++i) dst[(HP + i) * NTH + tid] = pre[i];
-            } else {
-                DFX_VMEM_DRAIN();
-            }
+            if (c + 1 == nchunks) DFX_VMEM_DRAIN();
             __syncthreads();
         }
         dfx_pf_raise_block(A, f, g, t1);
@@ -4416,8 +4444,8 @@
     constexpr int HP = PER_T / 2;
     DFX_DYN_SMEM(float, wsf);
     DfxWaiter W{A.spin_limit, A.err};
-    int f, g;
-    if (!dfx_pf_begin(A, W, reinterpret_cast<int *>(wsf), f, g)) return;
+    int f, g0, ng;
+    if (!dfx_pf_begin(A, W, reinterpret_cast<int *>(wsf), f, g0, ng)) return;
     const int tid = threadIdx.x, lane = tid & 63, wave = tid >> 6, q = lane >> 4, jl = lane & 15;
     constexpr int nchunks = N / (16 * CT);
     const int T = (int)A.T;
@@ -4430,13 +4458,15 @@
     auto piece_dst = [&](float *buf, int i) -> f32x4 * {
         return reinterpret_cast<f32x4 *>(buf + (((i >> 1) & 1) ? dst_off1 : dst_off0) + (128 * (i & 1) + (i >> 1)) * 64);
     };
-    for (int t0 = 0; t0 < T; t0 += SB) {
+    float4 *bl = reinterpret_cast<float4 *>(wsf + 2 * CHF);
+    if (tid < N / 4) bl[tid] = reinterpret_cast<const float4 *>(A.bias[f])[tid];
+    for (int t0 = 0; t0 < T; t0 += SB)
+    for (int g = g0; g < g0 + ng; ++g) {
         const int t1 = t0 + SB < T ? t0 + SB : T;
         int zoff = 0, jz = jl;
         DFX_OPAQUE(zoff);
         DFX_OPAQUE(jz);
         const float *w = reinterpret_cast<const float *>(A.wf[f]) + zoff;
-        const float *bias = A.bias[f] + zoff;
         const int64_t clip = (int64_t)g * 16 + jz;
         const bool okc = clip < A.B;
         const float *xrow = A.x[f] + (okc ? clip : 0) * A.T * K + 64 * q;
@@ -4496,22 +4526,21 @@
             }
             dfx_static_for<32, 64>(ksteps);
             DFX_MFMA_GUARD();
+            if (c + 1 < nchunks) {
+#pragma unroll
+                for (int i = 0; i < HP; ++i) *piece_dst(dstb, HP + i) = pre[i];
+            }
 #pragma unroll
             for (int ct = 0; ct < CT; ++ct) {
                 const int n = c * (16 * CT) + 16 * ct + 4 * q;
-                const float4 bz = *reinterpret_cast<const float4 *>(bias + n);
+                const float4 bz = bl[n >> 2];
 #pragma unroll
                 for (int t = 0; t < 2; ++t)
                     if (okr[t])
                         *reinterpret_cast<float4 *>(orow + trow[t] * N + n) =
                             make_float4(acc[t][ct][0] + bz.x, acc[t][ct][1] + bz.y, acc[t][ct][2] + bz.z, acc[t][ct][3] + bz.w);
             }
-            if (c + 1 < nchunks) {
-#pragma unroll
-                for (int i = 0; i < HP; ++i) *piece_dst(dstb, HP + i) = pre[i];
-            } else {
-                DFX_VMEM_DRAIN();
-            }
+            if (c + 1 == nchunks) DFX_VMEM_DRAIN();
             __syncthreads();
         }
         dfx_pf_raise_block(A, f, g, t1);
diff --git a/deepfilternet_amd/model.py b/deepfilternet_amd/model.py
--- a/deepfilternet_amd/model.py
+++ b/deepfilternet_amd/model.py
@@ -115,6 +115,7 @@
     Q_PASSES_C0_PRESPLIT = 7
     Q_LAST_PLAN = 8
     Q_PASSES_PAIR = 9
+    Q_PASSES_FOLLOW_PAIRS = 10
     PLAN_BITS = {"fan": 1 << 0, "fan_skp": 1 << 1, "fuse_h3": 1 << 2, "presplit": 1 << 3, "fuse_tail": 1 << 4, "fuse_enc": 1 << 5,
                  "fuse_enc4": 1 << 6, "enc_fan": 1 << 7, "dfenc": 1 << 8, "c0_fused": 1 << 9, "pipe": 1 << 10, "use_seq": 1 << 11,
                  "rows_finish": 1 << 14, "fuse_dec": 1 << 15}
diff --git a/include/dfx.h b/include/dfx.h
--- a/include/dfx.h
+++ b/include/dfx.h
@@ -116,6 +116,7 @@
 #define DFX_Q_PASSES_TICKET_BUSY 6
 #define DFX_Q_PASSES_C0_PRESPLIT 7
 #define DFX_Q_PASSES_PAIR 9
+#define DFX_Q_PASSES_FOLLOW_PAIRS 10
 #define DFX_Q_LAST_PLAN 8
 #define DFX_PLAN_FAN (1 << 0)
 #define DFX_PLAN_FAN_SKP (1 << 1)
```

Measured after the change: 24.85 million frames/s (median of 5 runs). About the same (+1.4%).
